# Stability-AI/stable-audio-tools

Hardware: AMD Instinct MI355X
Metric: train-step samples/sec (47s@44.1kHz) (higher is better)
Workload: dtype f32(bf16x3)

## Files before the change

### include/sat_amd.h

```cpp
#ifndef SAT_AMD_H
#define SAT_AMD_H

#ifdef __cplusplus
extern "C" {
#endif

int sat_abi_version(void);
int sat_is_simulator(void);
const char* sat_last_error(void);


int sat_conv1d(const float* x, const float* w_packed, const float* bias, const float* alpha, const float* beta,
               const float* res, float* y, const float* x2, const float* alpha2, const float* beta2,
               float* part_da, float* part_db, int B, int Cin, int Cout, int Tin, int Tout, int K, int stride,
               int dil, int pad, int tanh_out, void* stream);
int sat_conv1d_partial_rows(int B, int Tout);

int sat_conv1d_bf16x3(const float* x, const short* w_hi, const short* w_lo, const float* bias, const float* snake_a,
                      const float* snake_ib, const float* res, float* y, const float* x2, const float* alpha2,
                      const float* beta2, float* part_da, float* part_db, int B, int Cin, int Cout, int Tin, int Tout,
                      int K, int stride, int dil, int pad, int tanh_out, void* stream);
int sat_conv1d_bf16x3_emit(const float* x, const short* w_hi, const short* w_lo, const float* bias, const float* snake_a,
                      const float* snake_ib, const float* res, float* y, const float* x2, const float* alpha2,
                      const float* beta2, float* part_da, float* part_db, int B, int Cin, int Cout, int Tin, int Tout,
                      int K, int stride, int dil, int pad, int tanh_out, void* em_hi, void* em_lo,
                           const float* em_a, const float* em_ib, int em_rows, void* stream);
int sat_residual_unit_fwd(const short* xp_hi, const short* xp_lo, int rows, const short* w7_hi, const short* w7_lo,
                          const float* bias1, const float* a2, const float* ib2, const short* w1_hi, const short* w1_lo,
                          const float* bias2, const float* x, float* h, float* y, int B, int C, int T, int K, int dil, int pad,
                          void* em_hi, void* em_lo, const float* em_a, const float* em_ib, int em_rows, void* stream);
int sat_convtr1d_bf16x3(const float* x, const short* w_hi, const short* w_lo, const float* bias, const float* snake_a,
                        const float* snake_ib, const float* res, float* y, const float* x2, const float* alpha2,
                        const float* beta2, float* part_da, float* part_db, int B, int Cin, int Cout, int Tin, int Tout,
                        int K, int stride, int pad, int tanh_out, void* stream);
int sat_conv1d_bf16x3_partial_rows(int B, int Tout, int K, int stride);

int sat_rows_pack(const float* x, float* buf, int B, int C, int T, int W, int kh, int dil_t, int pad_t, int pad_w, int pitch, int lead,
                  void* stream);
int sat_rows_pack_bwd(const float* dbuf, float* dx, int B, int C, int T, int W, int kh, int dil_t, int pad_t, int pad_w, int pitch,
                      int lead, void* stream);
int sat_rows_unpack(const float* y, float* out, int B, int C, int T, int W, int pad_w, int pitch, float slope, void* stream);
int sat_rows_unpack_bwd(const float* dout, const float* out, float* dy, int B, int C, int T, int W, int pad_w, int pitch, float slope,
                        void* stream);

int sat_disc_geom(int frames, int W, int* P, int* L, int* lead, int* rows);
int sat_disc_planes(const float* src, const float* out, const signed char* fm_sign, const float* fm_coef, float* dst, void* hi, void* lo, int B,
                    int C, int frames, int W, int pitched, float slope, void* stream);
int sat_disc_l1_blocks(void);
int sat_disc_l1_sum(const float* a, const float* b, float* partial, signed char* sign, long long n, void* stream);
long long sat_disc_pack_size(int Cout, int Cin, int kh, int kw, int mode);
int sat_disc_pack_weights(const float* w, short* wq, int Cout, int Cin, int kh, int kw, int mode, void* stream);
int sat_disc_conv(const void* xp_hi, const void* xp_lo, const void* wq, const float* bias, float* y, void* em_hi,
                  void* em_lo, int B, int Cin, int Cout, int frames, int W, int kh, int kw, int dil_t, float slope, const float* lk_src,
                  float lk_slope, void* stream);
int sat_disc_wgrad_nsplit(int B, int M, int Cin, int kh, int frames, int W);
int sat_disc_wgrad(const float* dy, const float* x, float* partial, int B, int M, int Cin, int frames, int W, int kh, int kw, int dil_t,
                   void* stream);

int sat_conv1d_k7_plane_rows(int Tin, int Tout, int pad);
int sat_conv1d_k7_planes(const float* x, const float* snake_a, const float* snake_ib, short* xp_hi, short* xp_lo, int B, int Cin, int Tin,
                         int rows, void* stream);
long long sat_pack_weights_k7q_size(int D0, int D1, int K, int mode);
int sat_pack_weights_k7q(const float* w, short* hi, short* lo, int D0, int D1, int K, int mode, void* stream);
int sat_conv1d_bf16x3_planesq(const short* xp_hi, const short* xp_lo, int rows, const short* w_hi, const short* w_lo, const float* bias,
                             const float* res, float* y, const float* x2, const float* alpha2, const float* beta2, float* part_da,
                             float* part_db, int B, int Cin, int Cout, int Tin, int Tout, int K, int dil, int pad, int tanh_out,
                             int flags, void* stream);
int sat_convtr1d_bf16x3_partial_rows(int B, int Tout, int stride, int pad);
int sat_pack_weights_bf16x3(const float* w, short* hi, short* lo, int D0, int D1, int K, int stride, int mode, void* stream);
long long sat_pack_weights_bf16x3_size(int D0, int D1, int K, int stride, int mode);
int sat_snake_consts(const float* alpha, const float* beta, float* a, float* ib, int C, void* stream);

int sat_convtr1d(const float* x, const float* w_packed, const float* bias, const float* alpha, const float* beta,
                 const float* res, float* y, const float* x2, const float* alpha2, const float* beta2,
                 float* part_da, float* part_db, int B, int Cin, int Cout, int Tin, int Tout, int K, int stride,
                 int pad, int tanh_out, void* stream);
int sat_convtr1d_partial_rows(int B, int Tout, int stride, int pad);

int sat_conv_wgrad(const float* lo, const float* hi, const float* alpha, const float* beta, int snake_on,
                   float* partial, long long so_m, long long so_n, long long so_k, int B, int M, int N, int Tlo,
                   int Thi, int K, int stride, int dil, int pad, void* stream);
int sat_conv_wgrad_nsplit(int B, int M, int N, int Tlo, int K, int stride, int dil);

int sat_conv_wgrad7_bf16x3(const float* dy, const float* x, const float* alpha, const float* beta, float* partial,
                           long long so_m, long long so_n, long long so_k, int B, int M, int N, int T, int dil, int pad,
                           float* dy_rowsum, void* stream);
int sat_conv_wgrad7_bf16x3_nsplit(int B, int M, int N, int T);
int sat_conv_wgrad7_bf16x3_fuses_rowsum(int B, int M, int N, int T);

int sat_conv_wgrad_bf16x3(const float* lo, const float* hi, const float* alpha, const float* beta, int snake_on,
                          float* partial, long long so_m, long long so_n, long long so_k, int B, int M, int N, int Tlo,
                          int Thi, int K, int stride, int pad, float* lo_rowsum, void* stream);
int sat_conv_wgrad_bf16x3_nsplit(int B, int M, int N, int Tlo, int K, int stride);

int sat_ru_k1_bwd_nsplit(int B, int C, int T);
int sat_ru_k1_pack(const float* w, short* hi, short* lo, int C, void* stream);
int sat_ru_k1_bwd(const float* dy, const float* h, const short* wt_hi, const short* wt_lo, const float* alpha2, const float* beta2,
                  float* dh, short* em_hi, short* em_lo, int em_rows, float* dw_partial, float* part, int B, int C, int T,
                  void* stream);

int sat_reduce_splits(const float* partial, float* out, long long count, int nsplit, float scale, int accumulate,
                      void* stream);
int sat_rowsum(const float* x, float* partial, int B, int C, int T, void* stream);
int sat_rowsum_nsplit(int T);

int sat_wn_fold(const float* v, const float* g, float* w, float* norm, int D0, int R, void* stream);
int sat_wn_grad(const float* v, const float* g, const float* norm, const float* dw, float* dv, float* dg, int D0,
                int R, void* stream);
int sat_wn_grad_splits(const float* partial, int nsplit, long long count, long long so_m, long long so_n, long long so_k,
                       const float* v, const float* g, const float* norm, float* dv, float* dg, int D0, int N, int K,
                       const float* bias_partial, int bias_cols, float* dbias, void* stream);
int sat_edge_conv_ok(int cin, int cout, int k, int stride, int dil, int pad);
int sat_edge_conv_partial_rows(int B, int T);
int sat_edge_conv(const float* x, const float* w, const float* bias, const float* alpha, const float* beta, float* y, const float* x2,
                  const float* alpha2, const float* beta2, float* part_da, float* part_db, short* em_hi, short* em_lo,
                  const float* em_alpha, const float* em_beta, int em_rows, int B, int Cin, int Cout, int T, int K, int pad, int mode,
                  int tanh_out, void* stream);
int sat_edge_conv_wgrad_nsplit(int B, int M, int N, int T);
int sat_edge_conv_wgrad(const float* dy, const float* x, const float* alpha, const float* beta, float* partial, float* rowsum, int B,
                        int M, int N, int T, int K, int pad, void* stream);
int sat_pack_weights(const float* w, float* out, int D0, int D1, int K, int S, int mode, void* stream);

int sat_vae_nblocks(long long n);
int sat_vae_sample_fwd(const float* pre, const float* noise, float* z, float* kl_partial, int B, int C, int T,
                       void* stream);
int sat_vae_sample_bwd(const float* pre, const float* noise, const float* dz, const float* dkl, float* dpre, int B,
                       int C, int T, void* stream);

int sat_fir(const float* x, const float* taps, float* y, int N, int T, int ntaps, int adjoint, void* stream);
int sat_stft_tiles(int n_fft, int hop, int T);
int sat_stft_fwd(const float* x, const float* y, const float* views, float* partial, int NI, int C, int T, int NV,
                 int n_fft, int hop, void* stream);
int sat_stft_bwd(const float* x, const float* y, const float* views, const float* coef, float* dy, int NI, int C,
                 int T, int NV, int n_fft, int hop, int wrt_x, void* stream);

int sat_adamw_step(float* p, const float* g, float* m, float* v, long long n, float lr, float beta1, float beta2,
                   float eps, float weight_decay, int step, float grad_scale, float* ema, float ema_decay,
                   void* stream);
int sat_adamw_step_dev(float* p, const float* g, float* m, float* v, long long n, const float* hyper, float beta1, float beta2,
                       float eps, float weight_decay, float* ema, void* stream);

int sat_multi_copy(const void* entries, int nent, void* stream);

int sat_allreduce_available(void);
int sat_allreduce_unique_id(void* id128);
int sat_allreduce_init(const void* id128, int world, int rank, void** comm);
int sat_allreduce_bucket(void* comm, void* buf, long long count, int dtype, int mode, void* stream);
int sat_allreduce_finalize(void* comm);

int sat_attn_prepare(const void* src, long long sb, long long sh, long long sn, short* rm_hi, short* rm_lo,
                     short* tr_hi, short* tr_lo, int B, int H, int N, int Np, int dtype, void* stream);
int sat_attention_fwd(const short* q_hi, const short* q_lo, const short* k_hi, const short* k_lo, const short* vt_hi,
                      const short* vt_lo, void* o, float* lse, int B, int H, int Hkv, int Nq, int Nk, int Nqp, int Nkp,
                      int head_dim, float scale, int dtype, void* stream);
int sat_attention_rowdot(const void* dout, const void* out, float* dsum, int B, int H, int Nq, int dtype, void* stream);
int sat_attention_bwd(const short* const* planes, const float* lse, const float* dsum, void* dq, void* dk, void* dv,
                      int B, int H, int Hkv, int Nq, int Nk, int Nqp, int Nkp, int head_dim, float scale, int dtype,
                      void* stream);
int sat_attention_cross_ok(int H, int Hkv, int Nk, int head_dim, int dtype);
int sat_attention_cross_fwd(const short* q_rm, const short* k_rm, const short* v_tr, void* o, float* lse, int B, int H, int Hkv,
                            int Nq, int Nk, int Nqp, int Nkp, int head_dim, float scale, void* stream);
long long sat_attention_cross_bwd_ws(int B, int H, int Hkv, int Nq, int Nk);
int sat_attention_cross_bwd(const short* const* planes, const float* lse, const float* dsum, void* dq, void* dk, void* dv,
                            void* ws, long long ws_bytes, int B, int H, int Hkv, int Nq, int Nk, int Nqp, int Nkp, int head_dim,
                            float scale, void* stream);

int sat_layernorm_fwd(const void* x, const float* gamma, const float* beta, const void* scale, const void* shift,
                      long long mod_stride, void* y, float* mean, float* rstd, int rows, int D, int rows_per_batch,
                      float eps, int dtype, void* stream);
int sat_layernorm_fwd_fp8(const void* x, const float* gamma, const float* beta, const void* scale, const void* shift,
                          long long mod_stride, void* q, float* qscale, int rows, int D, int rows_per_batch, float eps,
                          int dtype, void* stream);
int sat_layernorm_bwd_nblocks(int rows, int rows_per_batch);
int sat_layernorm_bwd(const void* dy, const void* x, const float* gamma, const float* beta, const void* scale,
                      long long mod_stride, const float* mean, const float* rstd, void* dx, float* part, int rows, int D,
                      int rows_per_batch, int dtype, void* stream);
int sat_layernorm_bwd_res(const void* dy, const void* x, const float* gamma, const float* beta, const void* scale,
                          long long mod_stride, const float* mean, const float* rstd, const void* dres, void* dx, float* part,
                          int rows, int D, int rows_per_batch, int dtype, void* stream);

int sat_rope_tables(const float* inv_freq, float* cs, int N, int half, float pos_scale, void* stream);
int sat_rope_apply(void* t, const float* cs, long long sb, long long sn, long long sh, int B, int N, int H, int half,
                   int tab_off, int transpose, int dtype, void* stream);

int sat_swiglu(const void* xin, const void* dout, void* out, long long rows, int F, int backward, int dtype,
               void* stream);
int sat_gate_residual(const void* x, const void* gate, long long gstride, const void* res, void* y, int B, int N, int D,
                      int dtype, void* stream);
int sat_gate_residual_bwd_nchunks(int N);
int sat_gate_residual_bwd(const void* dy, const void* x, const void* gate, long long gstride, void* dx, float* part,
                          int B, int N, int D, int dtype, void* stream);

int sat_cfg_step(const void* out2, const void* x, void* y0, void* y1, int B, int C, int T, int ncond, float scale,
                 float phi, float c0x, float c0v, float c1x, float c1v, int dtype, void* stream);
int sat_sampler_step(const void* out2, const void* x, const void* prev, void* y0, void* y1, int B, int C, int T, int ncond,
                     float scale, float phi, const float* coef, int dtype, void* stream);
int sat_sampler_step_dev(const void* out2, const void* x, const void* prev, void* y0, void* y1, int B, int C, int T, int ncond,
                         float scale, float phi, const float* coef, int dtype, void* stream);
int sat_spec_frames(int n_fft, int hop, int T);
int sat_spec_fwd(const float* x, float* z, int NI, int C, int T, int n_fft, int hop, void* stream);
int sat_spec_bwd(const float* dz, float* dx, int NI, int C, int T, int n_fft, int hop, void* stream);


int sat_gemm_bf16(const void* A, long long lda, const void* B, long long ldb, void* C, long long ldc, const float* bias,
                  const void* res, long long ldr, const void* gate, long long ldg, int rows_per_gate, void* pre,
                  long long ldp, const void* zeros, int M, int N, int K, int epilogue, int out_f32, int splits, int tile,
                  void* stream);

int sat_gemm_qkv_bf16(const void* A, long long lda, const void* B, long long ldb, const float* rope_cs, int rope_off,
                      void* q_rm, void* k_rm, void* v_tr, const void* zeros, int nb, int ntok, int npad, int heads,
                      int K, int sec0, int nsec, int tile, void* stream);

int sat_splitk_epilogue(const float* slabs, int S, const float* bias, const void* res, long long ldr, void* out, long long ldo,
                        int M, int N, int out_f32, void* stream);

int sat_gemm_fp8(const void* A, long long lda, const void* B, long long ldb, void* C, long long ldc, const float* bias,
                 const void* res, long long ldr, const void* gate, long long ldg, int rows_per_gate, void* pre,
                 long long ldp, const void* zeros, const float* alpha, const float* row_alpha, const float* col_alpha, int M, int N,
                 int K, int epilogue, int out_f32, int tile, void* stream);
int sat_gemm_qkv_fp8(const void* A, long long lda, const void* B, long long ldb, const float* rope_cs, int rope_off,
                     void* q_rm, void* k_rm, void* v_tr, const void* zeros, const float* alpha, const float* row_alpha,
                     const float* col_alpha, int nb, int ntok, int npad, int heads, int K, int sec0, int nsec, int tile, void* stream);
int sat_absmax_scale_blocks(int R, int C);
int sat_absmax_scale(const void* src, long long lds, float* work, float* scales, int R, int C, int src_f32, void* stream);
int sat_quant_fp8(const void* src, long long lds, void* dst, long long ldd, const float* qscale, int R, int C, int src_f32,
                  void* stream);
int sat_quant_fp8_rows(const void* src, long long lds, void* dst, long long ldd, float* scale, int R, int C, int src_f32,
                       void* stream);

int sat_cast_bf16(const void* src, long long lds, void* dst, long long ldd, int R, int C, int Rpad, int src_f32,
                  int transpose, void* stream);
int sat_cast_bf16_tpair(const void* src_a, long long lds_a, void* dst_a, long long ldd_a, int Ra, int Ca, int Rpad_a, int a_f32,
                        const void* src_b, long long lds_b, void* dst_b, long long ldd_b, int Rb, int Cb, int Rpad_b, int b_f32,
                        void* stream);
int sat_cast_bf16_dual(const void* src, long long lds, void* dst, long long ldd, void* dst_t, long long ldd_t, int R, int C, int Rpad,
                       int src_f32, void* stream);

int sat_split_bf16x3(const float* src, long long lds, void* dst, long long ldd, int R, int C, int side, void* stream);

#ifdef __cplusplus
}
#endif
#endif
```

### stable_audio_tools_amd/_lib.py

```python
import ctypes
import os

_P = ctypes.c_void_p
_I = ctypes.c_int
_L = ctypes.c_longlong
_F = ctypes.c_float

SIGNATURES = {
    "sat_abi_version": (_I, []),
    "sat_is_simulator": (_I, []),
    "sat_last_error": (ctypes.c_char_p, []),
    "sat_conv1d": (_I, [_P] * 12 + [_I] * 10 + [_P]),
    "sat_conv1d_partial_rows": (_I, [_I, _I]),
    "sat_conv1d_bf16x3": (_I, [_P] * 13 + [_I] * 10 + [_P]),
    "sat_conv1d_bf16x3_emit": (_I, [_P] * 13 + [_I] * 10 + [_P] * 4 + [_I, _P]),
    "sat_convtr1d_bf16x3": (_I, [_P] * 13 + [_I] * 9 + [_P]),
    "sat_conv1d_bf16x3_partial_rows": (_I, [_I] * 4),
    "sat_rows_pack": (_I, [_P, _P] + [_I] * 10 + [_P]),
    "sat_rows_pack_bwd": (_I, [_P, _P] + [_I] * 10 + [_P]),
    "sat_rows_unpack": (_I, [_P, _P] + [_I] * 6 + [_F, _P]),
    "sat_rows_unpack_bwd": (_I, [_P, _P, _P] + [_I] * 6 + [_F, _P]),
    "sat_disc_geom": (_I, [_I, _I, _P, _P, _P, _P]),
    "sat_disc_planes": (_I, [_P] * 7 + [_I] * 5 + [_F, _P]),
    "sat_disc_l1_blocks": (_I, []),
    "sat_disc_l1_sum": (_I, [_P, _P, _P, _P, _L, _P]),
    "sat_disc_pack_size": (_L, [_I] * 5),
    "sat_disc_pack_weights": (_I, [_P] * 2 + [_I] * 5 + [_P]),
    "sat_disc_conv": (_I, [_P] * 7 + [_I] * 8 + [_F, _P, _F, _P]),
    "sat_disc_wgrad_nsplit": (_I, [_I] * 6),
    "sat_disc_wgrad": (_I, [_P] * 3 + [_I] * 8 + [_P]),
    "sat_conv1d_k7_plane_rows": (_I, [_I] * 3),
    "sat_conv1d_k7_planes": (_I, [_P] * 5 + [_I] * 4 + [_P]),
    "sat_conv1d_bf16x3_planesq": (_I, [_P, _P, _I] + [_P] * 10 + [_I] * 10 + [_P]),
    "sat_pack_weights_k7q": (_I, [_P, _P, _P, _I, _I, _I, _I, _P]),
    "sat_residual_unit_fwd": (_I, [_P, _P, _I] + [_P] * 11 + [_I] * 6 + [_P] * 4 + [_I, _P]),
    "sat_pack_weights_k7q_size": (_L, [_I, _I, _I, _I]),
    "sat_convtr1d_bf16x3_partial_rows": (_I, [_I] * 4),
    "sat_pack_weights_bf16x3": (_I, [_P, _P, _P, _I, _I, _I, _I, _I, _P]),
    "sat_pack_weights_bf16x3_size": (_L, [_I, _I, _I, _I, _I]),
    "sat_snake_consts": (_I, [_P, _P, _P, _P, _I, _P]),
    "sat_conv_wgrad7_bf16x3": (_I, [_P] * 5 + [_L] * 3 + [_I] * 6 + [_P, _P]),
    "sat_conv_wgrad7_bf16x3_nsplit": (_I, [_I] * 4),
    "sat_conv_wgrad7_bf16x3_fuses_rowsum": (_I, [_I] * 4),
    "sat_conv_wgrad_bf16x3": (_I, [_P] * 4 + [_I, _P] + [_L] * 3 + [_I] * 8 + [_P, _P]),
    "sat_conv_wgrad_bf16x3_nsplit": (_I, [_I] * 6),
    "sat_convtr1d": (_I, [_P] * 12 + [_I] * 9 + [_P]),
    "sat_convtr1d_partial_rows": (_I, [_I, _I, _I, _I]),
    "sat_conv_wgrad": (_I, [_P, _P, _P, _P, _I, _P, _L, _L, _L] + [_I] * 9 + [_P]),
    "sat_conv_wgrad_nsplit": (_I, [_I] * 7),
    "sat_reduce_splits": (_I, [_P, _P, _L, _I, _F, _I, _P]),
    "sat_ru_k1_bwd_nsplit": (_I, [_I] * 3),
    "sat_ru_k1_pack": (_I, [_P, _P, _P, _I, _P]),
    "sat_ru_k1_bwd": (_I, [_P] * 9 + [_I, _P, _P, _I, _I, _I, _P]),
    "sat_rowsum": (_I, [_P, _P, _I, _I, _I, _P]),
    "sat_rowsum_nsplit": (_I, [_I]),
    "sat_wn_fold": (_I, [_P, _P, _P, _P, _I, _I, _P]),
    "sat_wn_grad": (_I, [_P, _P, _P, _P, _P, _P, _I, _I, _P]),
    "sat_wn_grad_splits": (_I, [_P, _I, _L, _L, _L, _L, _P, _P, _P, _P, _P, _I, _I, _I, _P, _I, _P, _P]),
    "sat_pack_weights": (_I, [_P, _P, _I, _I, _I, _I, _I, _P]),
    "sat_vae_nblocks": (_I, [_L]),
    "sat_vae_sample_fwd": (_I, [_P, _P, _P, _P, _I, _I, _I, _P]),
    "sat_vae_sample_bwd": (_I, [_P, _P, _P, _P, _P, _I, _I, _I, _P]),
    "sat_multi_copy": (_I, [_P, _I, _P]),
    "sat_adamw_step": (_I, [_P, _P, _P, _P, _L, _F, _F, _F, _F, _F, _I, _F, _P, _F, _P]),
    "sat_adamw_step_dev": (_I, [_P, _P, _P, _P, _L, _P, _F, _F, _F, _F, _P, _P]),
    "sat_allreduce_available": (_I, []),
    "sat_allreduce_unique_id": (_I, [_P]),
    "sat_allreduce_init": (_I, [_P, _I, _I, _P]),
    "sat_allreduce_bucket": (_I, [_P, _P, _L, _I, _I, _P]),
    "sat_allreduce_finalize": (_I, [_P]),
    "sat_fir": (_I, [_P, _P, _P, _I, _I, _I, _I, _P]),
    "sat_stft_tiles": (_I, [_I, _I, _I]),
    "sat_stft_fwd": (_I, [_P, _P, _P, _P, _I, _I, _I, _I, _I, _I, _P]),
    "sat_stft_bwd": (_I, [_P, _P, _P, _P, _P, _I, _I, _I, _I, _I, _I, _I, _P]),
    "sat_spec_frames": (_I, [_I, _I, _I]),
    "sat_spec_fwd": (_I, [_P, _P, _I, _I, _I, _I, _I, _P]),
    "sat_spec_bwd": (_I, [_P, _P, _I, _I, _I, _I, _I, _P]),
    "sat_attn_prepare": (_I, [_P, _L, _L, _L, _P, _P, _P, _P, _I, _I, _I, _I, _I, _P]),
    "sat_attention_fwd": (_I, [_P] * 8 + [_I] * 8 + [_F, _I, _P]),
    "sat_attention_rowdot": (_I, [_P, _P, _P, _I, _I, _I, _I, _P]),
    "sat_attention_bwd": (_I, [_P] * 6 + [_I] * 8 + [_F, _I, _P]),
    "sat_edge_conv_ok": (_I, [_I] * 6),
    "sat_edge_conv_partial_rows": (_I, [_I] * 2),
    "sat_edge_conv": (_I, [_P] * 15 + [_I] * 9 + [_P]),
    "sat_edge_conv_wgrad_nsplit": (_I, [_I] * 4),
    "sat_edge_conv_wgrad": (_I, [_P] * 6 + [_I] * 6 + [_P]),
    "sat_attention_cross_ok": (_I, [_I] * 5),
    "sat_attention_cross_fwd": (_I, [_P] * 5 + [_I] * 8 + [_F, _P]),
    "sat_attention_cross_bwd_ws": (_L, [_I] * 5),
    "sat_attention_cross_bwd": (_I, [_P] * 7 + [_L] + [_I] * 8 + [_F, _P]),
    "sat_gemm_bf16": (_I, [_P, _L, _P, _L, _P, _L, _P, _P, _L, _P, _L, _I, _P, _L, _P] + [_I] * 7 + [_P]),
    "sat_gemm_qkv_bf16": (_I, [_P, _L, _P, _L, _P, _I, _P, _P, _P, _P] + [_I] * 8 + [_P]),
    "sat_gemm_fp8": (_I, [_P, _L, _P, _L, _P, _L, _P, _P, _L, _P, _L, _I, _P, _L, _P, _P, _P, _P] + [_I] * 6 + [_P]),
    "sat_gemm_qkv_fp8": (_I, [_P, _L, _P, _L, _P, _I, _P, _P, _P, _P, _P, _P, _P] + [_I] * 8 + [_P]),
    "sat_quant_fp8": (_I, [_P, _L, _P, _L, _P, _I, _I, _I, _P]),
    "sat_quant_fp8_rows": (_I, [_P, _L, _P, _L, _P, _I, _I, _I, _P]),
    "sat_absmax_scale": (_I, [_P, _L, _P, _P, _I, _I, _I, _P]),
    "sat_absmax_scale_blocks": (_I, [_I, _I]),
    "sat_splitk_epilogue": (_I, [_P, _I, _P, _P, _L, _P, _L, _I, _I, _I, _P]),
    "sat_cast_bf16": (_I, [_P, _L, _P, _L, _I, _I, _I, _I, _I, _P]),
    "sat_cast_bf16_tpair": (_I, [_P, _L, _P, _L, _I, _I, _I, _I, _P, _L, _P, _L, _I, _I, _I, _I, _P]),
    "sat_cast_bf16_dual": (_I, [_P, _L, _P, _L, _P, _L, _I, _I, _I, _I, _P]),
    "sat_split_bf16x3": (_I, [_P, _L, _P, _L, _I, _I, _I, _P]),
    "sat_layernorm_fwd": (_I, [_P] * 5 + [_L] + [_P] * 3 + [_I] * 3 + [_F, _I, _P]),
    "sat_layernorm_fwd_fp8": (_I, [_P] * 5 + [_L] + [_P] * 2 + [_I] * 3 + [_F, _I, _P]),
    "sat_layernorm_bwd_nblocks": (_I, [_I, _I]),
    "sat_layernorm_bwd": (_I, [_P] * 5 + [_L] + [_P] * 4 + [_I] * 4 + [_P]),
    "sat_layernorm_bwd_res": (_I, [_P] * 5 + [_L] + [_P] * 5 + [_I] * 4 + [_P]),
    "sat_rope_tables": (_I, [_P, _P, _I, _I, _F, _P]),
    "sat_rope_apply": (_I, [_P, _P, _L, _L, _L] + [_I] * 7 + [_P]),
    "sat_swiglu": (_I, [_P, _P, _P, _L, _I, _I, _I, _P]),
    "sat_gate_residual": (_I, [_P, _P, _L, _P, _P, _I, _I, _I, _I, _P]),
    "sat_gate_residual_bwd_nchunks": (_I, [_I]),
    "sat_cfg_step": (_I, [_P, _P, _P, _P, _I, _I, _I, _I, _F, _F, _F, _F, _F, _F, _I, _P]),
    "sat_sampler_step": (_I, [_P, _P, _P, _P, _P, _I, _I, _I, _I, _F, _F, _P, _I, _P]),
    "sat_sampler_step_dev": (_I, [_P, _P, _P, _P, _P, _I, _I, _I, _I, _F, _F, _P, _I, _P]),
    "sat_gate_residual_bwd": (_I, [_P, _P, _P, _L, _P, _P, _I, _I, _I, _I, _P]),
}

LIB_PATH = os.path.join(os.path.dirname(os.path.abspath(__file__)), "csrc", "libsat_amd.so")


def bind(cdll):
    for name, (res, args) in SIGNATURES.items():
        fn = getattr(cdll, name)
        fn.restype = res
        fn.argtypes = args
    return cdll


_lib = None


def load():
    global _lib
    if _lib is not None:
        return _lib
    if not os.path.exists(LIB_PATH):
        raise RuntimeError(
            f"stable_audio_tools_amd: HIP library not built: {LIB_PATH} is missing. "
            "Run `python -c 'import __graft_entry__ as g; g.build()'` (hipcc --offload-arch=gfx950). "
            "There is no CPU fallback.")
    try:
        cdll = ctypes.CDLL(LIB_PATH)
    except OSError as e:
        raise RuntimeError(f"stable_audio_tools_amd: cannot load {LIB_PATH}: {e}. There is no CPU fallback.") from e
    bind(cdll)
    if cdll.sat_is_simulator():
        raise RuntimeError("stable_audio_tools_amd: refusing to use a simulator build as the product library")
    _lib = cdll
    return _lib
```

### stable_audio_tools_amd/csrc/conv_wgrad_bf16x3.hip

```cpp
#include "conv_common.h"
#include <type_traits>

#define SAT_WB_TT 64
#define SAT_WB_LOROW (SAT_WB_TT + 8)
#define SAT_WB_HIROW 136

struct SatWgBfParams {
    const float* dy;
    const float* x;
    const float* alpha;
    const float* beta;
    float* out;
    long long so_split, so_m, so_n, so_k;
    int B, M, N, T, pad;
    int chunks_per_split, nchunks, nT;
    float* rowsum;
    int nsplit;
};

SAT_DEVICE unsigned sat_umulhi(unsigned a, unsigned b) { return (unsigned)(((unsigned long long)a * b) >> 32); }
SAT_DEVICE float sat_row16_sum(float4 q) {
    float s = (q.x + q.y) + (q.z + q.w);
#pragma unroll
    for (int m = 1; m <= 8; m <<= 1) s += __shfl_xor(s, m);
    return s;
}

#if defined(SAT_HIPEMU)
static inline unsigned sat_alignbit(unsigned hi, unsigned lo, unsigned s) {
    return (unsigned)((((unsigned long long)hi << 32) | lo) >> s);
}
#else
SAT_DEVICE unsigned sat_alignbit(unsigned hi, unsigned lo, unsigned s) { return __builtin_amdgcn_alignbit(hi, lo, s); }
#endif


template <int DIL>
__global__ void __launch_bounds__(256)
#if !defined(SAT_HIPEMU)
__attribute__((amdgpu_waves_per_eu(2, 2)))
#endif
sat_wgrad7_bf16x3_kernel(SatWgBfParams p) {
    constexpr int NCH = (6 * DIL + 7) / 8 + 1;
    __shared__ __attribute__((aligned(16))) short lo_lds[2][SAT_CO_T][SAT_WB_LOROW];
    __shared__ __attribute__((aligned(16))) short hi_lds[2][32][SAT_WB_HIROW];
    __shared__ float sn_a[32], sn_ib[32];

    const int tid = threadIdx.x, lane = tid & 63, wave = tid >> 6;
    const int l31 = lane & 31, hi = lane >> 5;
    int mn_tile, split;
    sat_xcd_tile(blockIdx.x + gridDim.x * (blockIdx.y + gridDim.y * blockIdx.z), gridDim.x * gridDim.y, gridDim.z, &mn_tile, &split);
    const int m0 = (mn_tile % (int)gridDim.x) * SAT_CO_T, n0 = (mn_tile / (int)gridDim.x) * 32;
    const int m_w = wave * 32;
    const bool wave_on = (m0 + m_w) < p.M;

    f32x16 acc[7];
#pragma unroll
    for (int k = 0; k < 7; ++k)
#pragma unroll
        for (int r = 0; r < 16; ++r) acc[k][r] = 0.0f;

    const bool want_rs = p.rowsum != nullptr && n0 == 0;
    float rs[8] = {0.f, 0.f, 0.f, 0.f, 0.f, 0.f, 0.f, 0.f};

    if (tid < 32) {
        const int c = n0 + tid;
        float sa = 1.f, sib = 0.f;
        if (p.alpha && c < p.N) {
            sa = expf(p.alpha[c]);
            sib = 1.0f / (expf(p.beta[c]) + 1e-9f);
        }
        sn_a[tid] = sa;
        sn_ib[tid] = sib;
    }
    for (int i = tid; i < 2 * 32 * SAT_WB_HIROW; i += 256) (&hi_lds[0][0][0])[i] = 0;
    __syncthreads();

    const int c_begin = split * p.chunks_per_split;
    int c_end = c_begin + p.chunks_per_split;
    if (c_end > p.nchunks) c_end = p.nchunks;
    constexpr int HSPAN = SAT_WB_TT + 6 * DIL;

    for (int ch = c_begin; ch < c_end; ++ch) {
        const int b = ch / p.nT;
        const int tt0 = (ch - b * p.nT) * SAT_WB_TT;
        {
            const float* src = p.dy + (size_t)b * p.M * p.T;
            for (int half = 0; half < 2; ++half) {
            float4 v[4];
#pragma unroll
            for (int u = 0; u < 4; ++u) {
                const int idx = tid + (half * 4 + u) * 256;
                const int row = idx >> 4, c4 = (idx & 15) * 4;
                const int m = m0 + row, t = tt0 + c4;
                float4 q = make_float4(0.f, 0.f, 0.f, 0.f);
                if (m < p.M) {
                    const float* s = src + (size_t)m * p.T + t;
                    if (t + 3 < p.T && ((p.T & 3) == 0)) {
                        q = *reinterpret_cast<const float4*>(s);
                    } else {
                        if (t + 0 < p.T) q.x = s[0];
                        if (t + 1 < p.T) q.y = s[1];
                        if (t + 2 < p.T) q.z = s[2];
                        if (t + 3 < p.T) q.w = s[3];
                    }
                }
                v[u] = q;
            }
#pragma unroll
            for (int u = 0; u < 4; ++u) {
                const int idx = tid + (half * 4 + u) * 256;
                const int row = idx >> 4, c4 = (idx & 15) * 4;
                if (want_rs) rs[half * 4 + u] += sat_row16_sum(v[u]);
                uint32_t h0, h1, l0, l1;
                sat_split2_pk(v[u].x, v[u].y, &h0, &l0);
                sat_split2_pk(v[u].z, v[u].w, &h1, &l1);
                typedef uint32_t u2 __attribute__((ext_vector_type(2)));
                *reinterpret_cast<u2*>(&lo_lds[0][row][c4]) = u2{h0, h1};
                *reinterpret_cast<u2*>(&lo_lds[1][row][c4]) = u2{l0, l1};
            }
            }
        }
        {
            const float* src = p.x + (size_t)b * p.N * p.T;
            const int th0 = tt0 - p.pad;
            constexpr int HP = HSPAN / 2;
            constexpr int TOTAL = 32 * HP;
            for (int base = tid; base < TOTAL; base += 8 * 256) {
                float v[8][2];
#pragma unroll
                for (int u = 0; u < 8; ++u) {
                    const int idx = base + u * 256;
                    const int row = idx / HP, col = (idx - row * HP) * 2;
                    const int n = n0 + row, t = th0 + col;
                    const bool ok = idx < TOTAL && n < p.N;
                    const float* s = src + (size_t)(ok ? n : 0) * p.T;
                    v[u][0] = (ok && t >= 0 && t < p.T) ? s[t] : 0.0f;
                    v[u][1] = (ok && t + 1 >= 0 && t + 1 < p.T) ? s[t + 1] : 0.0f;
                }
#pragma unroll
                for (int u = 0; u < 8; ++u) {
                    const int idx = base + u * 256;
                    if (idx < TOTAL) {
                        const int row = idx / HP, col = (idx - row * HP) * 2;
                        float o0 = v[u][0], o1 = v[u][1];
                        if (p.alpha) {
                            const float sa = sn_a[row], sib = sn_ib[row];
                            o0 = sat_snake(o0, sa, sib);
                            o1 = sat_snake(o1, sa, sib);
                        }
                        uint32_t h, l;
                        sat_split2_pk(o0, o1, &h, &l);
                        *reinterpret_cast<uint32_t*>(&hi_lds[0][row][col]) = h;
                        *reinterpret_cast<uint32_t*>(&hi_lds[1][row][col]) = l;
                    }
                }
            }
        }
        __syncthreads();
        if (wave_on) {
#pragma unroll
            for (int ks = 0; ks < SAT_WB_TT / 16; ++ks) {
                const int tb = 16 * ks + 8 * hi;
                bf16x8 af[2];
                af[0] = *reinterpret_cast<const bf16x8*>(&lo_lds[0][m_w + l31][tb]);
                af[1] = *reinterpret_cast<const bf16x8*>(&lo_lds[1][m_w + l31][tb]);
#pragma unroll
                for (int pl = 0; pl < 2; ++pl) {
                    u32x4 cw[NCH];
#if !defined(SAT_HIPEMU)
                    asm volatile("" ::: "memory");
#endif
#pragma unroll
                    for (int j = 0; j < NCH; ++j) cw[j] = *reinterpret_cast<const u32x4*>(&hi_lds[pl][l31][tb + 8 * j]);
#pragma unroll
                    for (int k = 0; k < 7; ++k) {
                        const int off = k * DIL;
                        const int wbase = (off >> 3) * 4 + ((off & 7) >> 1);
                        const bool odd = (off & 1) != 0;
                        u32x4 r;
#pragma unroll
                        for (int i = 0; i < 4; ++i) {
                            const int w0 = wbase + i, w1 = wbase + i + 1;
                            const unsigned a0 = cw[w0 >> 2][w0 & 3];
                            if (odd) {
                                const unsigned a1 = cw[w1 >> 2][w1 & 3];
                                r[i] = sat_alignbit(a1, a0, 16);
                            } else {
                                r[i] = a0;
                            }
                        }
                        const bf16x8 bf = __builtin_bit_cast(bf16x8, r);
                        acc[k] = sat_mfma_32x32x16_bf16(af[0], bf, acc[k]);
                        if (pl == 0) acc[k] = sat_mfma_32x32x16_bf16(af[1], bf, acc[k]);
                    }
                }
            }
        }
        __syncthreads();
    }

    if (want_rs && (tid & 15) == 0) {
#pragma unroll
        for (int i = 0; i < 8; ++i) {
            const int m = m0 + (tid >> 4) + 16 * i;
            if (m < p.M) p.rowsum[(size_t)m * p.nsplit + split] = rs[i];
        }
    }
    if (wave_on) {
        float* ob = p.out + (size_t)split * p.so_split;
        const int n = n0 + l31;
#pragma unroll
        for (int k = 0; k < 7; ++k)
#pragma unroll
            for (int r = 0; r < 16; ++r) {
                const int m = m0 + m_w + (r & 3) + 8 * (r >> 2) + 4 * hi;
                if (m < p.M && n < p.N) ob[(size_t)m * p.so_m + (size_t)n * p.so_n + (size_t)k * p.so_k] = acc[k][r];
            }
    }
}

#include "conv_wgrad7_bf16x3_pipe.h"

struct SatWgBfPlan { int nsplit, cps, nchunks, nT; bool pipe; };
static void sat_wgbf_plan(int B, int M, int N, int T, SatWgBfPlan* pl) {
    pl->nT = sat_cdiv(T, SAT_WB_TT);
    pl->nchunks = B * pl->nT;
    pl->pipe = N >= SAT_WP_NI && (T & 3) == 0;
    const int tiles = sat_cdiv(M, SAT_CO_T) * sat_cdiv(N, pl->pipe ? SAT_WP_NI : 32);
    int want = 512 / tiles;
    if (want > pl->nchunks) want = pl->nchunks;
    if (want < 1) want = 1;
    if (want > 512) want = 512;
    pl->cps = sat_cdiv(pl->nchunks, want);
    pl->nsplit = sat_cdiv(pl->nchunks, pl->cps);
}
extern "C" int sat_conv_wgrad7_bf16x3_nsplit(int B, int M, int N, int T) {
    SatWgBfPlan pl;
    sat_wgbf_plan(B, M, N, T, &pl);
    return pl.nsplit;
}
extern "C" int sat_conv_wgrad7_bf16x3_fuses_rowsum(int B, int M, int N, int T) {
    SatWgBfPlan pl;
    sat_wgbf_plan(B, M, N, T, &pl);
    return pl.pipe ? 0 : 1;
}
extern "C" int sat_conv_wgrad7_bf16x3(const float* dy, const float* x, const float* alpha, const float* beta, float* partial,
                                      long long so_m, long long so_n, long long so_k, int B, int M, int N, int T, int dil,
                                      int pad, float* dy_rowsum, void* stream) {
    if (B <= 0 || M <= 0 || N <= 0 || T <= 0) { sat_set_error("sat_conv_wgrad7_bf16x3: empty shape"); return 1; }
    if (dil != 1 && dil != 3 && dil != 9) { sat_set_error("sat_conv_wgrad7_bf16x3: dilation must be 1, 3 or 9 (the Oobleck ResidualUnits)"); return 1; }
    if ((alpha == nullptr) != (beta == nullptr)) { sat_set_error("sat_conv_wgrad7_bf16x3: alpha/beta must both be given"); return 1; }
    SatWgBfPlan pl;
    sat_wgbf_plan(B, M, N, T, &pl);
    SatWgBfParams p{dy, x, alpha, beta, partial, (long long)M * N * 7, so_m, so_n, so_k, B, M, N, T, pad, pl.cps, pl.nchunks, pl.nT,
                    dy_rowsum, pl.nsplit};
    if (pl.pipe) {
        dim3 grid(sat_cdiv(M, SAT_CO_T), sat_cdiv(N, SAT_WP_NI), pl.nsplit);
        if (dy_rowsum) { sat_set_error("sat_conv_wgrad7_bf16x3: this shape's kernel does not fuse the row sums (sat_conv_wgrad7_bf16x3_fuses_rowsum)"); return 1; }
        if (dil == 1) SAT_LAUNCH((sat_wgrad7_bf16x3_pipe_kernel<1>), grid, dim3(SAT_WP_NT), stream, p);
        else if (dil == 3) SAT_LAUNCH((sat_wgrad7_bf16x3_pipe_kernel<3>), grid, dim3(SAT_WP_NT), stream, p);
        else SAT_LAUNCH((sat_wgrad7_bf16x3_pipe_kernel<9>), grid, dim3(SAT_WP_NT), stream, p);
        return sat_check_launch("sat_conv_wgrad7_bf16x3");
    }
    dim3 grid(sat_cdiv(M, SAT_CO_T), sat_cdiv(N, 32), pl.nsplit);
    if (dil == 1) SAT_LAUNCH(sat_wgrad7_bf16x3_kernel<1>, grid, dim3(256), stream, p);
    else if (dil == 3) SAT_LAUNCH(sat_wgrad7_bf16x3_kernel<3>, grid, dim3(256), stream, p);
    else SAT_LAUNCH(sat_wgrad7_bf16x3_kernel<9>, grid, dim3(256), stream, p);
    return sat_check_launch("sat_conv_wgrad7_bf16x3");
}

#define SAT_WS_TT 64
#define SAT_WS_LOROW (SAT_WS_TT + 8)
#define SAT_WS_HIROW (SAT_WS_TT + 8)

struct SatWgSmallParams {
    const float* lo;
    const float* hi;
    const float* alpha;
    const float* beta;
    float* out;
    long long so_split, so_m, so_n, so_k;
    int B, M, N, Tlo, Thi, pad, snake_on, s_log2;
    int chunks_per_split, nchunks, nT;
    float* rowsum;
    int nsplit;
};

template <int NT>
__global__ void __launch_bounds__(256)
#if !defined(SAT_HIPEMU)
__attribute__((amdgpu_waves_per_eu(2, 2)))
#endif
sat_wgrad_small_bf16x3_kernel(SatWgSmallParams p) {
    constexpr int NCH = NT;
    __shared__ __attribute__((aligned(16))) short lo_lds[2][SAT_CO_T][SAT_WS_LOROW];
    __shared__ __attribute__((aligned(16))) short hi_lds[2][SAT_CO_T][SAT_WS_HIROW];
    __shared__ float sn_a[SAT_CO_T], sn_ib[SAT_CO_T];

    const int tid = threadIdx.x, lane = tid & 63, wave = tid >> 6;
    const int l31 = lane & 31, hi = lane >> 5;
    const int sl = p.s_log2, S = 1 << sl;
    int mn_tile, split;
    sat_xcd_tile(blockIdx.x + gridDim.x * (blockIdx.y + gridDim.y * blockIdx.z), gridDim.x * gridDim.y, gridDim.z, &mn_tile, &split);
    const int m0 = (mn_tile % (int)gridDim.x) * SAT_CO_T, v0 = (mn_tile / (int)gridDim.x) * SAT_CO_T;
    const int n_base = v0 >> sl, nc = SAT_CO_T >> sl;
    const int NV = p.N << sl;
    const int m_w = (wave >> 1) * 64, v_w = (wave & 1) * 64;
    const bool wave_on = (m0 + m_w) < p.M && (v0 + v_w) < NV;
    const bool snake_lo = p.alpha && p.snake_on == 1, snake_hi = p.alpha && p.snake_on == 2;

    f32x16 acc[2][2][NT];
#pragma unroll
    for (int i = 0; i < 2; ++i)
#pragma unroll
        for (int j = 0; j < 2; ++j)
#pragma unroll
            for (int k = 0; k < NT; ++k)
#pragma unroll
                for (int r = 0; r < 16; ++r) acc[i][j][k][r] = 0.0f;

    const bool want_rs = p.rowsum != nullptr && v0 == 0;
    float rsum[8] = {0.f, 0.f, 0.f, 0.f, 0.f, 0.f, 0.f, 0.f};

    if (tid < SAT_CO_T) {
        float sa = 1.f, sib = 0.f;
        const int c = snake_lo ? m0 + tid : n_base + tid;
        const bool ok = snake_lo ? c < p.M : (snake_hi && tid < nc && c < p.N);
        if (ok) {
            sa = expf(p.alpha[c]);
            sib = 1.0f / (expf(p.beta[c]) + 1e-9f);
        }
        sn_a[tid] = sa;
        sn_ib[tid] = sib;
    }
    __syncthreads();

    const int c_begin = split * p.chunks_per_split;
    int c_end = c_begin + p.chunks_per_split;
    if (c_end > p.nchunks) c_end = p.nchunks;
    const int rs = (SAT_WS_TT + NT - 1) << sl;
    const int up = rs >> 1;
    const int total_units = nc * up;

    auto mfma_stage = [&]() {
        if (wave_on) {
            SAT_MFMA_PRIO(1);
#pragma unroll
            for (int ks = 0; ks < SAT_WS_TT / 16; ++ks) {
                const int tb = 16 * ks + 8 * hi;
                bf16x8 af[2][2];
#pragma unroll
                for (int mi = 0; mi < 2; ++mi)
#pragma unroll
                    for (int pl = 0; pl < 2; ++pl)
                        af[mi][pl] = *reinterpret_cast<const bf16x8*>(&lo_lds[pl][m_w + mi * 32 + l31][tb]);
#pragma unroll
                for (int ni = 0; ni < 2; ++ni) {
#pragma unroll
                    for (int pl = 0; pl < 2; ++pl) {
                        u32x4 cw[NCH];
#pragma unroll
                        for (int j = 0; j < NCH; ++j) cw[j] = *reinterpret_cast<const u32x4*>(&hi_lds[pl][v_w + ni * 32 + l31][tb + 8 * j]);
#pragma unroll
                        for (int j = 0; j < NT; ++j) {
                            u32x4 r = cw[0];
                            if (j == 1) {
                                r[0] = sat_alignbit(cw[0][1], cw[0][0], 16);
                                r[1] = sat_alignbit(cw[0][2], cw[0][1], 16);
                                r[2] = sat_alignbit(cw[0][3], cw[0][2], 16);
                                r[3] = sat_alignbit(cw[NCH - 1][0], cw[0][3], 16);
                            }
                            const bf16x8 bf = __builtin_bit_cast(bf16x8, r);
#pragma unroll
                            for (int mi = 0; mi < 2; ++mi) {
                                acc[mi][ni][j] = sat_mfma_32x32x16_bf16(af[mi][0], bf, acc[mi][ni][j]);
                                if (pl == 0) acc[mi][ni][j] = sat_mfma_32x32x16_bf16(af[mi][1], bf, acc[mi][ni][j]);
                            }
                        }
                    }
                }
            }
            SAT_MFMA_PRIO(0);
        }
    };

    const bool fast1 = (NT == 1) && sl == 0 && p.pad == 0 && (p.Tlo & 3) == 0 && p.Thi == p.Tlo;
    if (fast1) {
        float4 vlo[8], vhi[8];
        const int row0 = tid >> 4, c4 = (tid & 15) * 4;
        auto issue = [&](int ch) {
            const int b = ch / p.nT;
            const int tt0 = (ch - b * p.nT) * SAT_WS_TT;
            const float* slo = p.lo + (size_t)b * p.M * p.Tlo;
            const float* shi = p.hi + (size_t)b * p.N * p.Thi;
            const bool t_ok = tt0 + c4 < p.Tlo;
#pragma unroll
            for (int u = 0; u < 8; ++u) {
                const int m = m0 + row0 + 16 * u, n = v0 + row0 + 16 * u;
                const bool okm = t_ok && m < p.M, okn = t_ok && n < p.N;
                const float4 a = *reinterpret_cast<const float4*>(slo + (size_t)(okm ? m : 0) * p.Tlo + (okm ? tt0 + c4 : 0));
                const float4 c = *reinterpret_cast<const float4*>(shi + (size_t)(okn ? n : 0) * p.Thi + (okn ? tt0 + c4 : 0));
                vlo[u] = okm ? a : make_float4(0.f, 0.f, 0.f, 0.f);
                vhi[u] = okn ? c : make_float4(0.f, 0.f, 0.f, 0.f);
            }
        };
        auto convert = [&]() {
            typedef uint32_t u2 __attribute__((ext_vector_type(2)));
#pragma unroll
            for (int u = 0; u < 8; ++u) {
                const int row = row0 + 16 * u;
                float4 q = vlo[u];
                if (want_rs) rsum[u] += sat_row16_sum(q);
                if (snake_lo) {
                    const float sa = sn_a[row], sib = sn_ib[row];
                    q.x = sat_snake(q.x, sa, sib); q.y = sat_snake(q.y, sa, sib);
                    q.z = sat_snake(q.z, sa, sib); q.w = sat_snake(q.w, sa, sib);
                }
                uint32_t h0, h1, l0, l1;
                sat_split2_pk(q.x, q.y, &h0, &l0);
                sat_split2_pk(q.z, q.w, &h1, &l1);
                *reinterpret_cast<u2*>(&lo_lds[0][row][c4]) = u2{h0, h1};
                *reinterpret_cast<u2*>(&lo_lds[1][row][c4]) = u2{l0, l1};
                q = vhi[u];
                if (snake_hi) {
                    const float sa = sn_a[row], sib = sn_ib[row];
                    q.x = sat_snake(q.x, sa, sib); q.y = sat_snake(q.y, sa, sib);
                    q.z = sat_snake(q.z, sa, sib); q.w = sat_snake(q.w, sa, sib);
                }
                sat_split2_pk(q.x, q.y, &h0, &l0);
                sat_split2_pk(q.z, q.w, &h1, &l1);
                *reinterpret_cast<u2*>(&hi_lds[0][row][c4]) = u2{h0, h1};
                *reinterpret_cast<u2*>(&hi_lds[1][row][c4]) = u2{l0, l1};
            }
        };
        issue(c_begin);
        for (int ch = c_begin; ch < c_end; ++ch) {
            convert();
            __syncthreads();
            if (ch + 1 < c_end) issue(ch + 1);
            mfma_stage();
            __syncthreads();
        }
    } else if ((NT == 2) && sl >= 1 && sl <= 3 && (p.Tlo & 3) == 0) {
        typedef float f4u __attribute__((ext_vector_type(4), aligned(4)));
        typedef uint32_t u2 __attribute__((ext_vector_type(2)));
        constexpr int NQ = 9;
        const int qpc = 33 << (sl - 1);
        const unsigned magic = 0xffffffffu / (unsigned)qpc + 1u;
        const int total_q = nc * qpc;
        const int qcl = sl >= 2 ? sl - 2 : 0, qc = 1 << qcl;
        auto load_quads = [&](int tv, const float* shi, int th0, bool interior, f4u* vq, auto ib, auto ie) {
            constexpr int IB = decltype(ib)::value, IE = decltype(ie)::value;
#pragma unroll
            for (int i = IB; i < IE; ++i) {
                f4u v = {0.f, 0.f, 0.f, 0.f};
                if (i < NQ - 1 || wave == 0) {
                    const int Q = tv + 256 * i;
                    const int cl = (int)sat_umulhi((unsigned)Q, magic), q = Q - cl * qpc;
                    const int n = n_base + cl, t = th0 + 4 * q;
                    const float* sp = shi + (size_t)(n < p.N ? n : p.N - 1) * p.Thi;
                    if (interior) {
                        v = *reinterpret_cast<const f4u*>(sp + t);
                    } else {
#pragma unroll
                        for (int e = 0; e < 4; ++e) {
                            const int te = t + e;
                            const int tc = te < 0 ? 0 : (te < p.Thi ? te : p.Thi - 1);
                            const float x = sp[tc];
                            v[e] = (te == tc) ? x : 0.0f;
                        }
                    }
                    if (n >= p.N) v = f4u{0.f, 0.f, 0.f, 0.f};
                }
                vq[i - IB] = v;
            }
        };
        auto store_quads = [&](int tv, const f4u* vq, auto ib, auto ie) {
            constexpr int IB = decltype(ib)::value, IE = decltype(ie)::value;
#pragma unroll
            for (int i = IB; i < IE; ++i) {
                const int Q = tv + 256 * i;
                if (i == NQ - 1 && Q >= total_q) break;
                const int cl = (int)sat_umulhi((unsigned)Q, magic), q = Q - cl * qpc;
                f4u o = vq[i - IB];
                if (snake_hi) {
                    const float sa = sn_a[cl], sib = sn_ib[cl];
#pragma unroll
                    for (int e = 0; e < 4; ++e) o[e] = sat_snake(o[e], sa, sib);
                }
                uint32_t h01, l01, h23, l23;
                sat_split2_pk(o[0], o[1], &h01, &l01);
                sat_split2_pk(o[2], o[3], &h23, &l23);
                int row, col;
                uint32_t wh0, wh1, wl0, wl1;
                if (sl == 1) {
                    row = cl << 1;
                    col = 2 * q;
                    wh0 = (h01 & 0xffffu) | (h23 << 16); wh1 = (h01 >> 16) | (h23 & 0xffff0000u);
                    wl0 = (l01 & 0xffffu) | (l23 << 16); wl1 = (l01 >> 16) | (l23 & 0xffff0000u);
                } else {
                    const int colq = q >> qcl, part = q & (qc - 1);
                    const bool odd = colq & 1;
                    const uint32_t rh = __shfl_xor(odd ? h01 : h23, qc), rl = __shfl_xor(odd ? l01 : l23, qc);
                    row = (cl << sl) + 4 * part + (odd ? 2 : 0);
                    col = colq & ~1;
                    if (!odd) {
                        wh0 = (h01 & 0xffffu) | (rh << 16); wh1 = (h01 >> 16) | (rh & 0xffff0000u);
                        wl0 = (l01 & 0xffffu) | (rl << 16); wl1 = (l01 >> 16) | (rl & 0xffff0000u);
                    } else {
                        wh0 = (rh & 0xffffu) | (h23 << 16); wh1 = (rh >> 16) | (h23 & 0xffff0000u);
                        wl0 = (rl & 0xffffu) | (l23 << 16); wl1 = (rl >> 16) | (l23 & 0xffff0000u);
                    }
                }
                *reinterpret_cast<uint32_t*>(&hi_lds[0][row][col]) = wh0;
                *reinterpret_cast<uint32_t*>(&hi_lds[0][row + 1][col]) = wh1;
                *reinterpret_cast<uint32_t*>(&hi_lds[1][row][col]) = wl0;
                *reinterpret_cast<uint32_t*>(&hi_lds[1][row + 1][col]) = wl1;
            }
        };
        using I0 = std::integral_constant<int, 0>; using IN = std::integral_constant<int, NQ>;
        f4u vq[NQ];
        auto issue_hi = [&](int ch) {
            const int b = ch / p.nT;
            const int tt0 = (ch - b * p.nT) * SAT_WS_TT;
            const int th0 = (tt0 << sl) - p.pad;
            const bool interior = th0 >= 0 && th0 + (66 << sl) <= p.Thi;
            int tv = tid;
#if !defined(SAT_HIPEMU)
            asm volatile("" : "+v"(tv));
#endif
            load_quads(tv, p.hi + (size_t)b * p.N * p.Thi, th0, interior, vq, I0{}, IN{});
        };
#if !defined(SAT_WGS_NOCARRY)
        issue_hi(c_begin);
#endif
        for (int ch = c_begin; ch < c_end; ++ch) {
            const int b = ch / p.nT;
            const int tt0 = (ch - b * p.nT) * SAT_WS_TT;
            const float* slo = p.lo + (size_t)b * p.M * p.Tlo;
            int tv = tid;
#if !defined(SAT_HIPEMU)
            asm volatile("" : "+v"(tv));
#endif
            const int row0 = tv >> 4, c4 = (tv & 15) * 4;
            float4 vlo[8];
#if defined(SAT_WGS_NOCARRY)
            issue_hi(ch);
#endif
            {
                const bool t_ok = tt0 + c4 < p.Tlo;
#pragma unroll
                for (int u = 0; u < 8; ++u) {
                    const int m = m0 + row0 + 16 * u;
                    const bool okm = t_ok && m < p.M;
                    const float4 a = *reinterpret_cast<const float4*>(slo + (size_t)(okm ? m : 0) * p.Tlo + (okm ? tt0 + c4 : 0));
                    vlo[u] = okm ? a : make_float4(0.f, 0.f, 0.f, 0.f);
                }
            }
            SAT_SCHED_FENCE();
            store_quads(tv, vq, I0{}, IN{});
            SAT_SCHED_FENCE();
#pragma unroll
            for (int u = 0; u < 8; ++u) {
                const int row = row0 + 16 * u;
                float4 q = vlo[u];
                if (want_rs) rsum[u] += sat_row16_sum(q);
                if (snake_lo) {
                    const float sa = sn_a[row], sib = sn_ib[row];
                    q.x = sat_snake(q.x, sa, sib); q.y = sat_snake(q.y, sa, sib);
                    q.z = sat_snake(q.z, sa, sib); q.w = sat_snake(q.w, sa, sib);
                }
// ... 181 lines not shown
```

### stable_audio_tools_amd/csrc/ru_k1_bwd.hip

```cpp
#include "conv_common.h"

typedef uint32_t sat_u32x2 __attribute__((ext_vector_type(2)));

#define SAT_RK_TT 32
#define SAT_RK_ROWN (SAT_RK_TT + 8)
#define SAT_RK_EROW (SAT_RK_TT + 4)
#define SAT_RK_LEAD 32

SAT_DEVICE f32x16 sat_rk_cat4(f32x4 v0, f32x4 v1, f32x4 v2, f32x4 v3) {
#if defined(SAT_HIPEMU)
    f32x16 o;
    for (int e = 0; e < 4; ++e) {
        o[e] = v0[e];
        o[4 + e] = v1[e];
        o[8 + e] = v2[e];
        o[12 + e] = v3[e];
    }
    return o;
#else
    typedef float sat_f8v __attribute__((ext_vector_type(8)));
    const sat_f8v lo = __builtin_shufflevector(v0, v1, 0, 1, 2, 3, 4, 5, 6, 7), hi = __builtin_shufflevector(v2, v3, 0, 1, 2, 3, 4, 5, 6, 7);
    return __builtin_shufflevector(lo, hi, 0, 1, 2, 3, 4, 5, 6, 7, 8, 9, 10, 11, 12, 13, 14, 15);
#endif
}
SAT_DEVICE bf16x8 sat_rk_frag(const f32x16& v, int g) {
    const f32x4 q = {v[4 * g], v[4 * g + 1], v[4 * g + 2], v[4 * g + 3]};
    return __builtin_bit_cast(bf16x8, q);
}

struct SatRuK1BwdParams {
    const float* dy;
    const float* h;
    const short* wt_hi;
    const short* wt_lo;
    const float* alpha2;
    const float* beta2;
    float* dh;
    short* em_hi;
    short* em_lo;
    float* dw_partial;
    float* part;
    int B, C, T, em_rows, nsplit, tiles_per_split, ntiles;
};

template <int C>
__global__ void __launch_bounds__(512) sat_ru_k1_bwd_kernel(SatRuK1BwdParams p) {
    static_assert(C == 128, "one 128-channel tile of h per workgroup, W2^T fragments in registers");
    constexpr int TT = SAT_RK_TT, ROWN = SAT_RK_ROWN, ROWT = C + 8, EROW = SAT_RK_EROW;
    constexpr int NJ = C / 64;
    constexpr int DYT = 2 * TT * ROWT;
    constexpr int DYN = 2 * C * ROWN;
    constexpr int AN = 2 * C * ROWN;
    constexpr int RAW = 2 * C * TT;
    static_assert(C * EROW * 4 <= AN * 2, "the epilogue tile aliases the snake2(h) image");
    static_assert(TT * 4 == 128, "a raw row is eight 16-byte DMA lanes");
    __shared__ __attribute__((aligned(16))) char smem[(DYT + DYN + AN) * 2 + 2 * RAW * 4];
    short* dyT = reinterpret_cast<short*>(smem);
    short* dyN = dyT + DYT;
    short* aN = dyN + DYN;
    float* etile = reinterpret_cast<float*>(aN);
    short* dhT = dyT;
    float* raw = reinterpret_cast<float*>(smem + (DYT + DYN + AN) * 2);

    const int tid = threadIdx.x, lane = tid & 63;
    const int wave = SAT_UNIFORM((int)(threadIdx.x >> 6));
    const int l31 = lane & 31, hi = lane >> 5;
    const int split = blockIdx.x;
    const int tiles_per_b = p.T / TT;
    const int tile_begin = split * p.tiles_per_split;
    int tile_end = tile_begin + p.tiles_per_split;
    if (tile_end > p.ntiles) tile_end = p.ntiles;
    const bool dgrad_wave = wave < 4;
    const int wq = wave & 3, wm = wq >> 1, wn = wq & 1;

    const int srow = tid >> 3, st4 = (tid & 7) * 4;
    const int swz_w = ((st4 >> 3) & 3) << 3;
    const int swz_f = ((l31 >> 3) & 3) << 3;
    float sa[NJ], sb[NJ], sib[NJ];
#pragma unroll
    for (int j = 0; j < NJ; ++j) {
        const int ci = srow + 64 * j;
        sa[j] = expf(p.alpha2[ci]);
        sb[j] = expf(p.beta2[ci]);
        sib[j] = 1.0f / (sb[j] + 1e-9f);
    }
    float sum_da[NJ], sum_db[NJ], sum_dh[NJ], sum_dy[NJ];
#pragma unroll
    for (int j = 0; j < NJ; ++j) sum_da[j] = sum_db[j] = sum_dh[j] = sum_dy[j] = 0.0f;

    f32x16 big[4];
    if (dgrad_wave) {
        const short* wrow_hi = p.wt_hi + (size_t)(32 * wq + l31) * C + 8 * hi;
        const short* wrow_lo = p.wt_lo + (size_t)(32 * wq + l31) * C + 8 * hi;
#pragma unroll
        for (int q = 0; q < 2; ++q) {
            big[q] = sat_rk_cat4(*reinterpret_cast<const f32x4*>(wrow_hi + 64 * q), *reinterpret_cast<const f32x4*>(wrow_hi + 64 * q + 16),
                                 *reinterpret_cast<const f32x4*>(wrow_hi + 64 * q + 32), *reinterpret_cast<const f32x4*>(wrow_hi + 64 * q + 48));
            big[2 + q] = sat_rk_cat4(*reinterpret_cast<const f32x4*>(wrow_lo + 64 * q), *reinterpret_cast<const f32x4*>(wrow_lo + 64 * q + 16),
                                     *reinterpret_cast<const f32x4*>(wrow_lo + 64 * q + 32), *reinterpret_cast<const f32x4*>(wrow_lo + 64 * q + 48));
        }
#if !defined(SAT_HIPEMU)
        asm volatile("" : "+v"(big[0]), "+v"(big[1]), "+v"(big[2]), "+v"(big[3]));
#endif
    } else {
#pragma unroll
        for (int i = 0; i < 4; ++i)
#pragma unroll
            for (int r = 0; r < 16; ++r) big[i][r] = 0.0f;
    }

    const size_t lane_off = (size_t)(lane >> 3) * p.T + (lane & 7) * 4;
    auto dma_tile = [&](int tile) __attribute__((always_inline)) {
        const int b = tile / tiles_per_b, t0 = (tile - b * tiles_per_b) * TT;
        char* slot = reinterpret_cast<char*>(raw) + (tile & 1) * (RAW * 4);
        const size_t base = (size_t)b * C * p.T + t0 + lane_off;
#pragma unroll
        for (int q = 0; q < 4; ++q) {
            const int piece = wave + 8 * q;
            const float* src = (q < 2 ? p.dy : p.h) + base + (size_t)(8 * (piece & 15)) * p.T;
            sat_glds16(src, slot + piece * 1024);
        }
    };
    if (tile_begin < tile_end) dma_tile(tile_begin);

    for (int tile = tile_begin; tile < tile_end; ++tile) {
        const int b = tile / tiles_per_b, t0 = (tile - b * tiles_per_b) * TT;
        const float* rt = raw + (tile & 1) * RAW;
        const bool more = tile + 1 < tile_end;
        if (more) { dma_tile(tile + 1); SAT_WAIT_VMCNT(4); } else { SAT_WAIT_VMCNT(0); }
        SAT_RAW_BARRIER();
        f32x4 hv[NJ];
#pragma unroll
        for (int j = 0; j < NJ; ++j) {
            const int ch = srow + 64 * j;
            const f32x4 dyv = *reinterpret_cast<const f32x4*>(rt + ch * TT + st4);
            hv[j] = *reinterpret_cast<const f32x4*>(rt + (C + ch) * TT + st4);
            uint32_t h0, l0, h1, l1;
            sat_split2_pk(dyv[0], dyv[1], &h0, &l0);
            sat_split2_pk(dyv[2], dyv[3], &h1, &l1);
            *reinterpret_cast<sat_u32x2*>(dyN + ch * ROWN + st4) = sat_u32x2{h0, h1};
            *reinterpret_cast<sat_u32x2*>(dyN + C * ROWN + ch * ROWN + st4) = sat_u32x2{l0, l1};
            const int cs = ch ^ swz_w;
            dyT[(st4 + 0) * ROWT + cs] = (short)(h0 & 0xffffu);
            dyT[(st4 + 1) * ROWT + cs] = (short)(h0 >> 16);
            dyT[(st4 + 2) * ROWT + cs] = (short)(h1 & 0xffffu);
            dyT[(st4 + 3) * ROWT + cs] = (short)(h1 >> 16);
            dyT[TT * ROWT + (st4 + 0) * ROWT + cs] = (short)(l0 & 0xffffu);
            dyT[TT * ROWT + (st4 + 1) * ROWT + cs] = (short)(l0 >> 16);
            dyT[TT * ROWT + (st4 + 2) * ROWT + cs] = (short)(l1 & 0xffffu);
            dyT[TT * ROWT + (st4 + 3) * ROWT + cs] = (short)(l1 >> 16);
            sum_dy[j] += (dyv[0] + dyv[1]) + (dyv[2] + dyv[3]);
            float v[4];
#pragma unroll
            for (int e = 0; e < 4; ++e) v[e] = sat_snake(hv[j][e], sa[j], sib[j]);
            sat_split2_pk(v[0], v[1], &h0, &l0);
            sat_split2_pk(v[2], v[3], &h1, &l1);
            *reinterpret_cast<sat_u32x2*>(aN + ch * ROWN + st4) = sat_u32x2{h0, h1};
            *reinterpret_cast<sat_u32x2*>(aN + C * ROWN + ch * ROWN + st4) = sat_u32x2{l0, l1};
        }
        SAT_WAIT_LGKM0();
        SAT_RAW_BARRIER();

        if (dgrad_wave) {
            f32x16 accd;
#pragma unroll
            for (int r = 0; r < 16; ++r) accd[r] = 0.0f;
            const short* brow = dyT + l31 * ROWT;
#pragma unroll
            for (int s = 0; s < C / 16; ++s) {
                const int col = (16 * s + 8 * hi) ^ swz_f;
                const bf16x8 bh = *reinterpret_cast<const bf16x8*>(brow + col);
                const bf16x8 bl = *reinterpret_cast<const bf16x8*>(brow + TT * ROWT + col);
                const bf16x8 wh = sat_rk_frag(big[s >> 2], s & 3), wl = sat_rk_frag(big[2 + (s >> 2)], s & 3);
                accd = sat_mfma_32x32x16_bf16(wh, bh, accd);
                accd = sat_mfma_32x32x16_bf16(wh, bl, accd);
                accd = sat_mfma_32x32x16_bf16(wl, bh, accd);
            }
            SAT_WAIT_LGKM0();
            SAT_RAW_BARRIER();
#pragma unroll
            for (int r = 0; r < 16; ++r) etile[(32 * wq + (r & 3) + 8 * (r >> 2) + 4 * hi) * EROW + l31] = accd[r];
        } else {
#pragma unroll
            for (int s = 0; s < TT / 16; ++s) {
                bf16x8 bh[2], bl[2];
#pragma unroll
                for (int nb = 0; nb < 2; ++nb) {
                    const short* br = aN + (wn * 64 + 32 * nb + l31) * ROWN + 16 * s + 8 * hi;
                    bh[nb] = *reinterpret_cast<const bf16x8*>(br);
                    bl[nb] = *reinterpret_cast<const bf16x8*>(br + C * ROWN);
                }
#pragma unroll
                for (int mb = 0; mb < 2; ++mb) {
                    const short* ar = dyN + (wm * 64 + 32 * mb + l31) * ROWN + 16 * s + 8 * hi;
                    const bf16x8 ah = *reinterpret_cast<const bf16x8*>(ar);
                    const bf16x8 al = *reinterpret_cast<const bf16x8*>(ar + C * ROWN);
#pragma unroll
                    for (int nb = 0; nb < 2; ++nb) {
                        big[2 * mb + nb] = sat_mfma_32x32x16_bf16(ah, bh[nb], big[2 * mb + nb]);
                        big[2 * mb + nb] = sat_mfma_32x32x16_bf16(ah, bl[nb], big[2 * mb + nb]);
                        big[2 * mb + nb] = sat_mfma_32x32x16_bf16(al, bh[nb], big[2 * mb + nb]);
                    }
                }
            }
            SAT_WAIT_LGKM0();
            SAT_RAW_BARRIER();
        }
        SAT_WAIT_LGKM0();
        SAT_RAW_BARRIER();

#pragma unroll
        for (int j = 0; j < NJ; ++j) {
            const int ch = srow + 64 * j;
            const f32x4 pre = *reinterpret_cast<const f32x4*>(etile + ch * EROW + st4);
            f32x4 out;
#pragma unroll
            for (int e = 0; e < 4; ++e) {
                const SatSnakeGrad g = sat_snake_grad(hv[j][e], sa[j], sb[j]);
                sum_da[j] += pre[e] * g.dla;
                sum_db[j] += pre[e] * g.dlb;
                out[e] = pre[e] * g.dx;
                sum_dh[j] += out[e];
            }
            *reinterpret_cast<f32x4*>(p.dh + ((size_t)b * C + ch) * p.T + t0 + st4) = out;
            if (p.em_hi) {
                uint32_t h0, l0, h1, l1;
                sat_split2_pk(out[0], out[1], &h0, &l0);
                sat_split2_pk(out[2], out[3], &h1, &l1);
                const int cs = ch ^ swz_w;
                dhT[(st4 + 0) * ROWT + cs] = (short)(h0 & 0xffffu);
                dhT[(st4 + 1) * ROWT + cs] = (short)(h0 >> 16);
                dhT[(st4 + 2) * ROWT + cs] = (short)(h1 & 0xffffu);
                dhT[(st4 + 3) * ROWT + cs] = (short)(h1 >> 16);
                dhT[TT * ROWT + (st4 + 0) * ROWT + cs] = (short)(l0 & 0xffffu);
                dhT[TT * ROWT + (st4 + 1) * ROWT + cs] = (short)(l0 >> 16);
                dhT[TT * ROWT + (st4 + 2) * ROWT + cs] = (short)(l1 & 0xffffu);
                dhT[TT * ROWT + (st4 + 3) * ROWT + cs] = (short)(l1 >> 16);
            }
        }
        SAT_WAIT_LGKM0();
        SAT_RAW_BARRIER();

        if (p.em_hi) {
            const int t = tid & 31, g = tid >> 5;
            const size_t o = (((size_t)b * (C / 8) + g) * p.em_rows + SAT_RK_LEAD + t0 + t) * 8;
            const int gs = (8 * g) ^ (((t >> 3) & 3) << 3);
            *reinterpret_cast<u32x4*>(p.em_hi + o) = *reinterpret_cast<const u32x4*>(dhT + t * ROWT + gs);
            *reinterpret_cast<u32x4*>(p.em_lo + o) = *reinterpret_cast<const u32x4*>(dhT + TT * ROWT + t * ROWT + gs);
            SAT_WAIT_LGKM0();
            SAT_RAW_BARRIER();
        }
    }

    if (!dgrad_wave) {
        float* slab = p.dw_partial + (size_t)split * C * C;
#pragma unroll
        for (int mb = 0; mb < 2; ++mb)
#pragma unroll
            for (int nb = 0; nb < 2; ++nb)
#pragma unroll
                for (int r = 0; r < 16; ++r) {
                    const int co = wm * 64 + 32 * mb + (r & 3) + 8 * (r >> 2) + 4 * hi;
                    const int ci = wn * 64 + 32 * nb + l31;
                    slab[(size_t)co * C + ci] = big[2 * mb + nb][r];
                }
    }
    const size_t ps = (size_t)C * p.nsplit;
#pragma unroll
    for (int j = 0; j < NJ; ++j) {
        float va = sum_da[j], vb = sum_db[j], vh = sum_dh[j], vy = sum_dy[j];
#pragma unroll
        for (int m = 1; m <= 4; m <<= 1) {
            va += __shfl_xor(va, m);
            vb += __shfl_xor(vb, m);
            vh += __shfl_xor(vh, m);
            vy += __shfl_xor(vy, m);
        }
        if ((tid & 7) == 0) {
            const size_t o = (size_t)(srow + 64 * j) * p.nsplit + split;
            p.part[o] = va;
            p.part[ps + o] = vb;
            p.part[2 * ps + o] = vh;
            p.part[3 * ps + o] = vy;
        }
    }
}

static int sat_ru_k1_plan(int B, int C, int T, int* nsplit, int* tiles_per_split, int* ntiles) {
    if (B <= 0 || T <= 0 || C != 128 || (T % SAT_RK_TT) != 0) return 1;
    const long long nt = (long long)B * (T / SAT_RK_TT);
    if (nt > 0x7fffffff) return 1;
    int want = sat_cu_count();
    if (want > nt) want = (int)nt;
    const int per = (int)((nt + want - 1) / want);
    *tiles_per_split = per;
    *nsplit = (int)((nt + per - 1) / per);
    *ntiles = (int)nt;
    return 0;
}

extern "C" int sat_ru_k1_bwd_nsplit(int B, int C, int T) {
    int ns, per, nt;
    if (sat_ru_k1_plan(B, C, T, &ns, &per, &nt)) return -1;
    return ns;
}

extern "C" int sat_ru_k1_bwd(const float* dy, const float* h, const short* wt_hi, const short* wt_lo, const float* alpha2,
                             const float* beta2, float* dh, short* em_hi, short* em_lo, int em_rows, float* dw_partial, float* part,
                             int B, int C, int T, void* stream) {
    SatRuK1BwdParams p{dy, h, wt_hi, wt_lo, alpha2, beta2, dh, em_hi, em_lo, dw_partial, part, B, C, T, em_rows, 0, 0, 0};
    if (sat_ru_k1_plan(B, C, T, &p.nsplit, &p.tiles_per_split, &p.ntiles)) {
        sat_set_error("sat_ru_k1_bwd: needs C == 128 and T % 32 == 0 (sat_ru_k1_bwd_nsplit)");
        return 1;
    }
    if (!dy || !h || !wt_hi || !wt_lo || !alpha2 || !beta2 || !dh || !dw_partial || !part) { sat_set_error("sat_ru_k1_bwd: missing buffer"); return 1; }
    if ((em_hi == nullptr) != (em_lo == nullptr) || (em_hi && em_rows < SAT_RK_LEAD + T)) { sat_set_error("sat_ru_k1_bwd: bad emission planes"); return 1; }
    if ((((uintptr_t)dy | (uintptr_t)h | (uintptr_t)dh | (uintptr_t)em_hi | (uintptr_t)em_lo | (uintptr_t)wt_hi | (uintptr_t)wt_lo) & 15) != 0) {
        sat_set_error("sat_ru_k1_bwd: buffers must be 16-byte aligned");
        return 1;
    }
    SAT_LAUNCH(sat_ru_k1_bwd_kernel<128>, dim3(p.nsplit), dim3(512), stream, p);
    return sat_check_launch("sat_ru_k1_bwd");
}

struct SatRuK1PackParams {
    const float* w;
    short* hi;
    short* lo;
    int C;
};
__global__ void __launch_bounds__(256) sat_ru_k1_pack_kernel(SatRuK1PackParams p) {
    const int i = blockIdx.x * 256 + threadIdx.x;
    if (i >= p.C * p.C) return;
    const int ci = i / p.C, co = i - ci * p.C;
    const float v = p.w[(size_t)co * p.C + ci];
    const short hb = sat_f32_to_bf16(v);
    p.hi[i] = hb;
    p.lo[i] = sat_f32_to_bf16(v - sat_bf16_to_f32(hb));
}
extern "C" int sat_ru_k1_pack(const float* w, short* hi, short* lo, int C, void* stream) {
    if (C <= 0 || !w || !hi || !lo) { sat_set_error("sat_ru_k1_pack: bad arguments"); return 1; }
    SatRuK1PackParams p{w, hi, lo, C};
    SAT_LAUNCH(sat_ru_k1_pack_kernel, dim3(sat_cdiv(C * C, 256)), dim3(256), stream, p);
    return sat_check_launch("sat_ru_k1_pack");
}
```

### stable_audio_tools_amd/csrc/sat_device.h

```cpp
#pragma once

#if defined(SAT_HIPEMU)
#include "hipemu.h"
#define SAT_DEVICE static inline
#else
#include <hip/hip_runtime.h>
#define SAT_DEVICE __device__ __forceinline__
#endif

#include <stdint.h>

typedef float f32x4 __attribute__((ext_vector_type(4)));
typedef float f32x16 __attribute__((ext_vector_type(16)));
typedef short bf16x8 __attribute__((ext_vector_type(8)));
typedef uint32_t u32x4 __attribute__((ext_vector_type(4)));
typedef int i32x8 __attribute__((ext_vector_type(8)));

#define SAT_WAVE 64

#if defined(SAT_HIPEMU)
static inline float hipemu_bf16_to_f32(short s) {
    uint32_t u = ((uint32_t)(uint16_t)s) << 16;
    float f;
    memcpy(&f, &u, 4);
    return f;
}
static inline f32x16 sat_mfma_32x32x2_f32(float a, float b, f32x16 c) {
    struct { float a, b; } mine = {a, b};
    const char* all = hipemu::wave_exchange(&mine, sizeof(mine));
    const int l = hipemu::lane_id();
    const int col = l & 31, hi = l >> 5;
    f32x16 d = c;
    for (int r = 0; r < 16; ++r) {
        const int row = (r & 3) + 8 * (r >> 2) + 4 * hi;
        float acc = c[r];
        for (int k = 0; k < 2; ++k) {
            float av, bv;
            memcpy(&av, all + (size_t)(row + 32 * k) * hipemu::kSlotBytes, 4);
            memcpy(&bv, all + (size_t)(col + 32 * k) * hipemu::kSlotBytes + 4, 4);
            acc = fmaf(av, bv, acc);
        }
        d[r] = acc;
    }
    return d;
}
static inline f32x16 sat_mfma_32x32x16_bf16(bf16x8 a, bf16x8 b, f32x16 c) {
    struct { bf16x8 a, b; } mine = {a, b};
    const char* all = hipemu::wave_exchange(&mine, sizeof(mine));
    const int l = hipemu::lane_id();
    const int col = l & 31, hi = l >> 5;
    f32x16 d = c;
    for (int r = 0; r < 16; ++r) {
        const int row = (r & 3) + 8 * (r >> 2) + 4 * hi;
        float acc = c[r];
        for (int g = 0; g < 2; ++g) {
            bf16x8 av, bv;
            memcpy(&av, all + (size_t)(row + 32 * g) * hipemu::kSlotBytes, 16);
            memcpy(&bv, all + (size_t)(col + 32 * g) * hipemu::kSlotBytes + 16, 16);
            for (int e = 0; e < 8; ++e) acc += hipemu_bf16_to_f32(av[e]) * hipemu_bf16_to_f32(bv[e]);
        }
        d[r] = acc;
    }
    return d;
}
static inline f32x4 sat_mfma_16x16x32_bf16(bf16x8 a, bf16x8 b, f32x4 c) {
    struct { bf16x8 a, b; } mine = {a, b};
    const char* all = hipemu::wave_exchange(&mine, sizeof(mine));
    const int l = hipemu::lane_id();
    const int col = l & 15, grp = l >> 4;
    f32x4 d = c;
    for (int r = 0; r < 4; ++r) {
        const int row = 4 * grp + r;
        float acc = c[r];
        for (int g = 0; g < 4; ++g) {
            bf16x8 av, bv;
            memcpy(&av, all + (size_t)(row + 16 * g) * hipemu::kSlotBytes, 16);
            memcpy(&bv, all + (size_t)(col + 16 * g) * hipemu::kSlotBytes + 16, 16);
            for (int e = 0; e < 8; ++e) acc += hipemu_bf16_to_f32(av[e]) * hipemu_bf16_to_f32(bv[e]);
        }
        d[r] = acc;
    }
    return d;
}
static inline float hipemu_e4m3_to_f32(uint8_t v) {
    const int s = v >> 7, e = (v >> 3) & 15, m = v & 7;
    float f;
    if (e == 15 && m == 7) f = NAN;
    else if (e == 0) f = ldexpf((float)m, -9);
    else f = ldexpf((float)(8 + m), e - 10);
    return s ? -f : f;
}
static inline f32x16 sat_mfma_32x32x64_fp8(i32x8 a, i32x8 b, f32x16 c) {
    struct { i32x8 a, b; } mine = {a, b};
    const char* all = hipemu::wave_exchange(&mine, sizeof(mine));
    const int l = hipemu::lane_id();
    const int col = l & 31, hi = l >> 5;
    f32x16 d = c;
    for (int r = 0; r < 16; ++r) {
        const int row = (r & 3) + 8 * (r >> 2) + 4 * hi;
        float acc = c[r];
        for (int g = 0; g < 2; ++g) {
            uint8_t av[32], bv[32];
            memcpy(av, all + (size_t)(row + 32 * g) * hipemu::kSlotBytes, 32);
            memcpy(bv, all + (size_t)(col + 32 * g) * hipemu::kSlotBytes + 32, 32);
            for (int e = 0; e < 32; ++e) acc += hipemu_e4m3_to_f32(av[e]) * hipemu_e4m3_to_f32(bv[e]);
        }
        d[r] = acc;
    }
    return d;
}
#else
SAT_DEVICE f32x16 sat_mfma_32x32x64_fp8(i32x8 a, i32x8 b, f32x16 c) {
    return __builtin_amdgcn_mfma_scale_f32_32x32x64_f8f6f4(a, b, c, 0, 0, 0, 127, 0, 127);
}
SAT_DEVICE f32x16 sat_mfma_32x32x2_f32(float a, float b, f32x16 c) {
    return __builtin_amdgcn_mfma_f32_32x32x2f32(a, b, c, 0, 0, 0);
}
SAT_DEVICE f32x16 sat_mfma_32x32x16_bf16(bf16x8 a, bf16x8 b, f32x16 c) {
    typedef __bf16 bf16x8_t __attribute__((ext_vector_type(8)));
    return __builtin_amdgcn_mfma_f32_32x32x16_bf16(__builtin_bit_cast(bf16x8_t, a), __builtin_bit_cast(bf16x8_t, b), c, 0, 0, 0);
}
SAT_DEVICE f32x4 sat_mfma_16x16x32_bf16(bf16x8 a, bf16x8 b, f32x4 c) {
    typedef __bf16 bf16x8_t __attribute__((ext_vector_type(8)));
    return __builtin_amdgcn_mfma_f32_16x16x32_bf16(__builtin_bit_cast(bf16x8_t, a), __builtin_bit_cast(bf16x8_t, b), c, 0, 0, 0);
}
#endif

SAT_DEVICE uint32_t sat_f32x4_to_fp8(float a, float b, float c, float d) {
#if defined(SAT_HIPEMU)
    auto enc = [](float x) -> uint32_t {
        if (x != x) return 0x7fu;
        const uint32_t sign = x < 0.f ? 0x80u : 0u;
        float ax = fabsf(x);
        if (ax > 448.f) ax = 448.f;
        if (ax < ldexpf(1.0f, -10)) return sign;
        int e;
        frexpf(ax, &e);
        int ue = e - 1;
        if (ue < -6) ue = -6;
        const float q = ldexpf(1.0f, ue - 3);
        float m = nearbyintf(ax / q);
        float v = m * q;
        if (v > 448.f) v = 448.f;
        if (v == 0.f) return sign;
        frexpf(v, &e);
        ue = e - 1;
        uint32_t bits;
        if (ue < -6) bits = (uint32_t)nearbyintf(v / ldexpf(1.0f, -9));
        else bits = ((uint32_t)(ue + 7) << 3) | ((uint32_t)nearbyintf(v / ldexpf(1.0f, ue - 3)) - 8u);
        return sign | bits;
    };
    return enc(a) | (enc(b) << 8) | (enc(c) << 16) | (enc(d) << 24);
#else
    const float lim = 448.0f;
    a = fminf(fmaxf(a, -lim), lim); b = fminf(fmaxf(b, -lim), lim); c = fminf(fmaxf(c, -lim), lim); d = fminf(fmaxf(d, -lim), lim);
    int w = 0;
    w = __builtin_amdgcn_cvt_pk_fp8_f32(a, b, w, false);
    w = __builtin_amdgcn_cvt_pk_fp8_f32(c, d, w, true);
    return (uint32_t)w;
#endif
}

SAT_DEVICE short sat_f32_to_bf16(float f) {
    uint32_t u;
    memcpy(&u, &f, 4);
    if ((u & 0x7fffffffu) > 0x7f800000u) return (short)0x7fc0;
    u += 0x7fffu + ((u >> 16) & 1u);
    return (short)(u >> 16);
}
SAT_DEVICE float sat_bf16_to_f32(short s) {
    uint32_t u = ((uint32_t)(uint16_t)s) << 16;
    float f;
    memcpy(&f, &u, 4);
    return f;
}

SAT_DEVICE void sat_split2_pk(float a, float b, uint32_t* hi, uint32_t* lo) {
#if defined(SAT_HIPEMU)
    const short ha = sat_f32_to_bf16(a), hb = sat_f32_to_bf16(b);
    const short la = sat_f32_to_bf16(a - sat_bf16_to_f32(ha)), lb = sat_f32_to_bf16(b - sat_bf16_to_f32(hb));
    *hi = ((uint32_t)(uint16_t)hb << 16) | (uint16_t)ha;
    *lo = ((uint32_t)(uint16_t)lb << 16) | (uint16_t)la;
#else
    typedef __bf16 sat_bf2 __attribute__((ext_vector_type(2)));
    typedef float sat_f2 __attribute__((ext_vector_type(2)));
    const sat_f2 v = {a, b};
    const sat_bf2 h = __builtin_convertvector(v, sat_bf2);
    const sat_f2 d = v - __builtin_convertvector(h, sat_f2);
    const sat_bf2 l = __builtin_convertvector(d, sat_bf2);
    *hi = __builtin_bit_cast(uint32_t, h);
    *lo = __builtin_bit_cast(uint32_t, l);
#endif
}

SAT_DEVICE uint32_t sat_cvt2_pk(float a, float b) {
#if defined(SAT_HIPEMU)
    return ((uint32_t)(uint16_t)sat_f32_to_bf16(b) << 16) | (uint16_t)sat_f32_to_bf16(a);
#else
    typedef __bf16 sat_bf2 __attribute__((ext_vector_type(2)));
    typedef float sat_f2 __attribute__((ext_vector_type(2)));
    const sat_f2 v = {a, b};
    return __builtin_bit_cast(uint32_t, __builtin_convertvector(v, sat_bf2));
#endif
}

#if defined(SAT_HIPEMU)
#define SAT_UNIFORM(x) (x)
#else
#define SAT_UNIFORM(x) __builtin_amdgcn_readfirstlane(x)
#endif

SAT_DEVICE void sat_xcd_tile(int L, int nshare, int nouter, int* share_idx, int* outer_idx) {
    const int ngroups = nouter >> 3;
    const int per_group = 8 * nshare;
    if (L < ngroups * per_group) {
        const int grp = L / per_group, rem = L - grp * per_group;
        *share_idx = rem >> 3;
        *outer_idx = grp * 8 + (rem & 7);
    } else {
        const int R = L - ngroups * per_group;
        *share_idx = R % nshare;
        *outer_idx = ngroups * 8 + R / nshare;
    }
}

template <int B, class T>
SAT_DEVICE T& sat_pick(T& a, T& b) {
    if constexpr (B == 0) return a;
    else return b;
}

SAT_DEVICE float sat_wave_sum(float v) {
    for (int m = 32; m >= 1; m >>= 1) v += __shfl_xor(v, m);
    return v;
}
SAT_DEVICE float sat_half_sum(float v) {
    for (int m = 16; m >= 1; m >>= 1) v += __shfl_xor(v, m);
    return v;
}

SAT_DEVICE void sat_sincos2(float y, float* s2y, float* c2y) {
    const float hi = y * 0.31830987334251404f;
    float lo = fmaf(y, 0.31830987334251404f, -hi);
    lo = fmaf(y, 1.2841276486e-08f, lo);
#if defined(SAT_HIPEMU)
    const float f = (hi - floorf(hi)) + lo;
    *s2y = sinf(6.283185307179586f * f);
    *c2y = cosf(6.283185307179586f * f);
#else
    const float f = __builtin_amdgcn_fractf(hi) + lo;
    *s2y = __builtin_amdgcn_sinf(f);
    *c2y = __builtin_amdgcn_cosf(f);
#endif
}
SAT_DEVICE float sat_sin2(float y) {
    float s, c;
    sat_sincos2(y, &s, &c);
    return fmaf(-0.5f, c, 0.5f);
}

SAT_DEVICE float sat_snake(float x, float a, float ib) {
    return fmaf(ib, sat_sin2(x * a), x);
}

#if defined(SAT_HIPEMU)
static inline void sat_glds16(const void* g, void* lds_wave_base) { memcpy((char*)lds_wave_base + 16 * hipemu::lane_id(), g, 16); }
static inline void sat_glds4(const void* g, void* lds_wave_base) { memcpy((char*)lds_wave_base + 4 * hipemu::lane_id(), g, 4); }
#define SAT_WAIT_VMCNT(n)
#define SAT_RAW_BARRIER() hipemu::block_barrier()
#define SAT_WAIT_LGKM0()
#define SAT_SCHED_FENCE()
static inline void sat_wave_sync() { int z = 0; (void)hipemu::wave_exchange(&z, sizeof(z)); }
#define SAT_SETPRIO(x)
#define SAT_SCHED_GROUP(mask, n)
static inline bool sat_wave_any(bool v) {
    int x = v ? 1 : 0;
    for (int m = 32; m >= 1; m >>= 1) x |= __shfl_xor(x, m);
    return x != 0;
}
#else
SAT_DEVICE void sat_glds16(const void* g, void* lds_wave_base) {
    __builtin_amdgcn_global_load_lds((const __attribute__((address_space(1))) void*)g,
                                     (__attribute__((address_space(3))) void*)lds_wave_base, 16, 0, 0);
}
SAT_DEVICE void sat_glds4(const void* g, void* lds_wave_base) {
    __builtin_amdgcn_global_load_lds((const __attribute__((address_space(1))) void*)g,
                                     (__attribute__((address_space(3))) void*)lds_wave_base, 4, 0, 0);
}
#define SAT_WAIT_VMCNT(n) asm volatile("s_waitcnt vmcnt(%0)" ::"n"(n) : "memory")
#define SAT_RAW_BARRIER() __builtin_amdgcn_s_barrier()
#define SAT_WAIT_LGKM0() asm volatile("s_waitcnt lgkmcnt(0)" ::: "memory")
#define SAT_SCHED_FENCE() __builtin_amdgcn_sched_barrier(0)
SAT_DEVICE void sat_wave_sync() { __builtin_amdgcn_wave_barrier(); }
#define SAT_SETPRIO(x) __builtin_amdgcn_s_setprio(x)
#define SAT_SCHED_GROUP(mask, n) __builtin_amdgcn_sched_group_barrier(mask, n, 0)
SAT_DEVICE bool sat_wave_any(bool v) { return __builtin_amdgcn_ballot_w64(v) != 0; }
#endif

#if defined(SAT_WITH_MFMA_PRIO)
#define SAT_MFMA_PRIO(x) SAT_SETPRIO(x)
#else
#define SAT_MFMA_PRIO(x)
#endif

void sat_set_error(const char* msg);
int sat_check_launch(const char* what);
int sat_cu_count();

#if defined(SAT_HIPEMU)
#define SAT_LAUNCH(kernel, grid, block, stream, params) \
    hipemu::launch((grid), (block), [=]() { kernel(params); })
#else
#define SAT_LAUNCH(kernel, grid, block, stream, params) \
    hipLaunchKernelGGL(kernel, (grid), (block), 0, (hipStream_t)(stream), params)
#endif

static inline int sat_cdiv(int a, int b) { return (a + b - 1) / b; }
static inline long long sat_cdivll(long long a, long long b) { return (a + b - 1) / b; }
```

### stable_audio_tools_amd/functional.py

```python
import torch

from . import ops as _ops_mod
from .ops import PACK_CONV_DGRAD, PACK_CONV_FWD, PACK_POLYPHASE


def _ops(ops):
    return ops if ops is not None else _ops_mod.get_ops()


class SumAllFn(torch.autograd.Function):

    @staticmethod
    def forward(ctx, x, ops=None):
        ctx.in_shape, ctx.in_dtype = x.shape, x.dtype
        return _ops(ops).sum_all(x.detach())

    @staticmethod
    def backward(ctx, g):
        return g.to(ctx.in_dtype).expand(ctx.in_shape), None


def sum_all(x, ops=None):
    return SumAllFn.apply(x, ops)


def mean_all(x, ops=None):
    return SumAllFn.apply(x, ops) / x.numel()


class DerivedCache:

    def __init__(self):
        self.items = {}

    def get(self, name, sources, make):
        from . import _caches
        if not _caches.trackable(*sources):
            return make()
        key = tuple((t.data_ptr(), _caches.version_of(t), t.device) for t in sources if t is not None) + _caches.epoch_of(*sources)
        hit = self.items.get(name)
        if hit is None or hit[0] != key:
            hit = (key, make())
            self.items[name] = hit
        return hit[1]


def _cached(cache, name, sources, make):
    return make() if cache is None else cache.get(name, sources, make)


class WeightNormFn(torch.autograd.Function):
    @staticmethod
    def forward(ctx, v, g, ops=None):
        ops = _ops(ops)
        v = v.contiguous()
        gf = g.contiguous().view(-1)
        w, norm = ops.wn_fold(v, gf)
        ctx.save_for_backward(v, gf, norm)
        ctx.ops = ops
        ctx.g_shape = g.shape
        return w

    @staticmethod
    def backward(ctx, dw):
        v, gf, norm = ctx.saved_tensors
        dv, dg = ctx.ops.wn_grad(v, gf, norm, dw.contiguous())
        return dv, dg.view(ctx.g_shape), None


def _conv_dgrad(ops, dy, w, k, stride, dil, pad, cin, tin, dsnake, res=None, out=None, emit=None):
    if stride == 1:
        if (res is None and out is None and emit is None and ops.edge_ok(w.shape[0], cin, k, 1, dil, (k - 1) * dil - pad) and tin == dy.shape[2]
                and (dsnake is None or w.shape[0] <= 2)):
            return ops.edge_conv(dy, w, (k - 1) * dil - pad, mode=1, dsnake=dsnake)
        if ops.bf16x3_ok(k, 1, dil):
            q = ops.k7q_applicable(w.shape[0], k, 1, dil, (k - 1) * dil - pad, cin)
            return ops.conv1d_bf16x3(dy, ops.pack_bf16x3(w, mode=1, q=q), cin, k, 1, dil, (k - 1) * dil - pad, tout=tin,
                                     dsnake=dsnake, res=res, out=out, emit=emit)
        wpb = ops.pack(w, PACK_CONV_DGRAD)
        return ops.conv1d(dy, wpb, cin, k, 1, dil, (k - 1) * dil - pad, tout=tin, dsnake=dsnake, res=res, out=out)
    if out is not None:
        raise NotImplementedError("_conv_dgrad(out=...) is only plumbed through the stride-1 kernels")
    if ops.bf16x3_ok(k, stride, dil, transposed=True):
        return ops.convtr1d_bf16x3(dy, ops.pack_bf16x3(w, mode=2, stride=stride), cin, k, stride, pad, tout=tin,
                                   dsnake=dsnake, res=res)
    wpb = ops.pack(w, PACK_POLYPHASE, stride)
    return ops.convtr1d(dy, wpb, cin, k, stride, pad, tout=tin, dsnake=dsnake, res=res)


def _conv_wgrad(ops, dy, x, k, stride, dil, pad, snake, bias_grad=False, raw=False):
    if ops.edge_ok(x.shape[1], dy.shape[1], k, stride, dil, pad) and dy.shape[2] == x.shape[2] and (snake is None or dy.shape[1] <= 2):
        return ops.edge_conv_wgrad(dy, x, k, pad, snake=snake, dy_rowsum=bias_grad, raw=raw)
    if ops.wgrad7_bf16x3_ok(x.shape[1], k, stride, dil):
        return ops.conv_wgrad7_bf16x3(dy, x, dil, pad, snake=snake, dy_rowsum=bias_grad, raw=raw)
    return ops.conv_wgrad(dy, x, k, stride, dil, pad, snake=snake, snake_on=2, lo_rowsum=bias_grad, raw=raw)


def _wn_forward(ops, v, g):
    v = v.contiguous()
    gf = g.contiguous().view(-1)
    w, norm = ops.wn_fold(v, gf)
    return w, (v, gf, norm)


def _wn_backward(ops, slabs, saved, g_shape, bias_partial=None):
    v, gf, norm = saved
    out = ops.wn_grad_splits(slabs, v, gf, norm, bias_partial=bias_partial)
    return (out[0], out[1].view(g_shape)) + tuple(out[2:])


def _conv_fwd(ops, x, w, stride, dil, pad, bias=None, snake=None, res=None, tanh_out=False, dsnake=None, tout=None, cache=None, emit=None):
    cout, cin, k = w.shape
    if (res is None and ops.edge_ok(cin, cout, k, stride, dil, pad) and (tout is None or tout == x.shape[2])
            and (snake is None or cout <= 2) and (dsnake is None or cin <= 2) and (emit is None or cin <= 2)):
        return ops.edge_conv(x, w, pad, bias=bias, snake=snake, tanh_out=tanh_out, dsnake=dsnake, emit=emit)
    if ops.bf16x3_ok(k, stride, dil):
        q = ops.k7q_applicable(cin, k, stride, dil, pad, cout)
        planes = _cached(cache, "pack_fwd_q" if q else "pack_fwd", (w,), lambda: ops.pack_bf16x3(w, stride=stride, q=q))
        sconsts = _cached(cache, "snake", snake, lambda: ops.snake_consts(snake[0], snake[1])) if snake is not None else None
        return ops.conv1d_bf16x3(x, planes, cout, k, stride, dil, pad, tout=tout, bias=bias,
                                 snake=snake, res=res, tanh_out=tanh_out, dsnake=dsnake, sconsts=sconsts, emit=emit)
    return ops.conv1d(x, _cached(cache, "pack_fwd32", (w,), lambda: ops.pack(w, PACK_CONV_FWD)), cout, k, stride, dil, pad, tout=tout,
                      bias=bias, snake=snake, res=res, tanh_out=tanh_out, dsnake=dsnake)


def _convtr_fwd(ops, x, w, stride, pad, bias=None, snake=None, cache=None):
    cin, cout, k = w.shape
    if ops.bf16x3_ok(k, stride, 1, transposed=True):
        planes = _cached(cache, "pack_tr", (w,), lambda: ops.pack_bf16x3(w, mode=2, stride=stride))
        sconsts = _cached(cache, "snake", snake, lambda: ops.snake_consts(snake[0], snake[1])) if snake is not None else None
        return ops.convtr1d_bf16x3(x, planes, cout, k, stride, pad, bias=bias, snake=snake, sconsts=sconsts)
    return ops.convtr1d(x, _cached(cache, "pack_tr32", (w,), lambda: ops.pack(w, PACK_POLYPHASE, stride)), cout, k, stride, pad,
                        bias=bias, snake=snake)


class SnakeConv1dFn(torch.autograd.Function):

    @staticmethod
    def forward(ctx, x, alpha, beta, w, bias, res, stride, dil, pad, tanh_out, ops=None, cache=None, next_snake=None, g=None):
        ops = _ops(ops)
        x = x.contiguous()
        wn = ()
        if g is not None:
            w, wn = _wn_forward(ops, w, g)
        w = w.contiguous()
        cout, cin, k = w.shape
        snake = (alpha.contiguous(), beta.contiguous()) if alpha is not None else None
        emit = None
        if next_snake is not None and not tanh_out:
            tout_ = (x.shape[2] + 2 * pad - dil * (k - 1) - 1) // stride + 1
            if ((ops.emit_ok(cout, k, stride, tout_, next_snake[2]) and ops.bf16x3_ok(k, stride, dil))
                    or (res is None and snake is None and ops.edge_emit_ok(cin, cout, k, stride, dil, pad, next_snake[2]))):
                emit = {"snake": (next_snake[0].detach(), next_snake[1].detach())}
        y = _conv_fwd(ops, x, w, stride, dil, pad, bias=bias, snake=snake,
                      res=res.contiguous() if res is not None else None, tanh_out=tanh_out, cache=cache, emit=emit)
        ctx.ops = ops
        ctx.cfg = (stride, dil, pad, tanh_out, bias is not None, res is not None, alpha is not None)
        ctx.g_shape = g.shape if g is not None else None
        ctx.save_for_backward(x, alpha, beta, w, y if tanh_out else None, *wn)
        return y

    @staticmethod
    def backward(ctx, dy):
        ops = ctx.ops
        stride, dil, pad, tanh_out, has_bias, has_res, has_snake = ctx.cfg
        x, alpha, beta, w, y = ctx.saved_tensors[:5]
        wn = ctx.saved_tensors[5:]
        cout, cin, k = w.shape
        dy = dy.contiguous()
        if tanh_out:
            dy = dy * (1.0 - y * y)
        snake = (alpha, beta) if has_snake else None
        dres = dy if has_res else None
        dw = dbias = dg = None
        if ctx.needs_input_grad[3] or (wn and ctx.needs_input_grad[13]):
            dw = _conv_wgrad(ops, dy, x, k, stride, dil, pad, snake, bias_grad=has_bias, raw=bool(wn))
            if has_bias:
                dw, dbias = dw
            if wn:
                dw, dg, *rest = _wn_backward(ops, dw, wn, ctx.g_shape, bias_partial=dbias)
                if has_bias:
                    dbias = rest[0]
        elif has_bias:
            dbias = ops.rowsum(dy)
        dx = da = db = None
        if has_snake:
            dx, da, db = _conv_dgrad(ops, dy, w, k, stride, dil, pad, cin, x.shape[2], (x, alpha, beta))
        elif ctx.needs_input_grad[0]:
            dx = _conv_dgrad(ops, dy, w, k, stride, dil, pad, cin, x.shape[2], None)
        return dx, da, db, dw, dbias, dres, None, None, None, None, None, None, None, dg


class SnakeConvTr1dFn(torch.autograd.Function):

    @staticmethod
    def forward(ctx, x, alpha, beta, w, bias, stride, pad, ops=None, cache=None, g=None):
        ops = _ops(ops)
        x = x.contiguous()
        wn = ()
        if g is not None:
            w, wn = _wn_forward(ops, w, g)
        w = w.contiguous()
        cin, cout, k = w.shape
        snake = (alpha.contiguous(), beta.contiguous()) if alpha is not None else None
        y = _convtr_fwd(ops, x, w, stride, pad, bias=bias, snake=snake, cache=cache)
        ctx.ops = ops
        ctx.cfg = (stride, pad, bias is not None, alpha is not None)
        ctx.g_shape = g.shape if g is not None else None
        ctx.save_for_backward(x, alpha, beta, w, *wn)
        return y

    @staticmethod
    def backward(ctx, dy):
        ops = ctx.ops
        stride, pad, has_bias, has_snake = ctx.cfg
        x, alpha, beta, w = ctx.saved_tensors[:4]
        wn = ctx.saved_tensors[4:]
        cin, cout, k = w.shape
        dy = dy.contiguous()
        snake = (alpha, beta) if has_snake else None
        dbias = ops.rowsum(dy) if has_bias else None
        dw = ops.conv_wgrad(x, dy, k, stride, 1, pad, snake=snake, snake_on=1, raw=bool(wn))
        dg = None
        if wn:
            dw, dg = _wn_backward(ops, dw, wn, ctx.g_shape)
        dx = da = db = None
        if has_snake:
            dx, da, db = _conv_fwd(ops, dy, w, stride, 1, pad, dsnake=(x, alpha, beta), tout=x.shape[2])
        elif ctx.needs_input_grad[0]:
            dx = _conv_fwd(ops, dy, w, stride, 1, pad, tout=x.shape[2])
        return dx, da, db, dw, dbias, None, None, None, None, dg


class ResidualUnitFn(torch.autograd.Function):

    @staticmethod
    def forward(ctx, x, a1, b1, w1, bias1, a2, b2, w2, bias2, dil, ops=None, recompute=False, caches=None, next_snake=None, fuse=False,
                g1=None, g2=None):
        ops = _ops(ops)
        x = x.contiguous()
        wn1 = wn2 = ()
        if g1 is not None:
            w1, wn1 = _wn_forward(ops, w1, g1)
        if g2 is not None:
            w2, wn2 = _wn_forward(ops, w2, g2)
        w1 = w1.contiguous()
        w2 = w2.contiguous()
        c = x.shape[1]
        k1 = w1.shape[2]
        pad = dil * (k1 - 1) // 2
        c1, c2 = caches if caches is not None else (None, None)
        emit = None
        if next_snake is not None and ops.emit_ok(c, w2.shape[2], 1, x.shape[2], next_snake[2]):
            emit = {"snake": (next_snake[0].detach(), next_snake[1].detach())}
        if fuse and w2.shape[2] == 1 and w1.shape[0] == c and ops.ru_fused_ok(c, k1, dil, x.shape[2]):
            w7q = _cached(c1, "pack_q7", (w1,), lambda: ops.pack_k7q(w1))
            w1q = _cached(c2, "pack_q1", (w2,), lambda: ops.pack_k7q(w2))
            sc = None
            if c1 is not None and c2 is not None:
                sc = (_cached(c1, "snake", (a1, b1), lambda: ops.snake_consts(a1, b1)), _cached(c2, "snake", (a2, b2), lambda: ops.snake_consts(a2, b2)))
            h, y = ops.residual_unit_fwd(x, (a1, b1), w7q, bias1, (a2, b2), w1q, bias2, k1, dil, keep_h=ctx is not None and not recompute and fuse != "nokeep",
                                         emit=emit, sconsts=sc)
        else:
            h = _conv_fwd(ops, x, w1, 1, dil, pad, bias=bias1, snake=(a1, b1), cache=c1)
            y = _conv_fwd(ops, h, w2, 1, 1, 0, bias=bias2, snake=(a2, b2), res=x, cache=c2, emit=emit)
        ctx.ops = ops
        ctx.dil = dil
        ctx.recompute = bool(recompute)
        ctx.g_shapes = (g1.shape if g1 is not None else None, g2.shape if g2 is not None else None)
        ctx.save_for_backward(x, None if recompute else h, a1, b1, w1, a2, b2, w2, bias1 if recompute else None, *wn1, *wn2)
        return y

    @staticmethod
    def backward(ctx, dy):
        ops = ctx.ops
        x, h, a1, b1, w1, a2, b2, w2, bias1 = ctx.saved_tensors[:9]
        gs1, gs2 = ctx.g_shapes
        rest = ctx.saved_tensors[9:]
        wn1 = rest[:3] if gs1 is not None else ()
        wn2 = rest[len(wn1):] if gs2 is not None else ()
        dil = ctx.dil
        c = x.shape[1]
        k1, k2 = w1.shape[2], w2.shape[2]
        pad1 = dil * (k1 - 1) // 2
        t = x.shape[2]
        dy = dy.contiguous()
        if ctx.recompute:
            h = _conv_fwd(ops, x, w1, 1, dil, pad1, bias=bias1, snake=(a1, b1))
        want_emit = ops.emit_ok(w1.shape[0], k2, 1, t, dil) and ops.k7q_applicable(w1.shape[0], k1, 1, dil, pad1, c)
        if k2 == 1 and w2.shape[0] == c and w1.shape[0] == c and ops.ru_k1_bwd_ok(dy.shape[0], c, t):
            dh, da2, db2, dw2, dbias2, dbias1 = ops.ru_k1_bwd(dy, h, w2, (a2, b2), emit=want_emit, raw=bool(wn2))
            dw1 = _conv_wgrad(ops, dh, x, k1, 1, dil, pad1, (a1, b1), bias_grad=False, raw=bool(wn1))
        else:
            dw2, dbias2 = ops.conv_wgrad(dy, h, k2, 1, 1, 0, snake=(a2, b2), snake_on=2, lo_rowsum=True, raw=bool(wn2))
            dh, da2, db2 = _conv_dgrad(ops, dy, w2, k2, 1, 1, 0, c, t, (h, a2, b2), emit={"snake": None} if want_emit else None)
            dw1, dbias1 = _conv_wgrad(ops, dh, x, k1, 1, dil, pad1, (a1, b1), bias_grad=True, raw=bool(wn1))
        dg1 = dg2 = None
        if wn1:
            if dbias1.dim() == 2:
                dw1, dg1, dbias1 = _wn_backward(ops, dw1, wn1, gs1, bias_partial=dbias1)
            else:
                dw1, dg1 = _wn_backward(ops, dw1, wn1, gs1)
        if wn2:
            if dbias2.dim() == 2:
                dw2, dg2, dbias2 = _wn_backward(ops, dw2, wn2, gs2, bias_partial=dbias2)
            else:
                dw2, dg2 = _wn_backward(ops, dw2, wn2, gs2)
        dx, da1, db1 = _conv_dgrad(ops, dh, w1, k1, 1, dil, pad1, c, t, (x, a1, b1), res=dy)
        return dx, da1, db1, dw1, dbias1, da2, db2, dw2, dbias2, None, None, None, None, None, None, dg1, dg2


class VaeSampleFn(torch.autograd.Function):

    @staticmethod
    def forward(ctx, pre, noise, ops=None):
        ops = _ops(ops)
        pre = pre.contiguous()
        noise = noise.contiguous()
        z, kl = ops.vae_sample_fwd(pre, noise)
        ctx.ops = ops
        ctx.save_for_backward(pre, noise)
        return z, kl

    @staticmethod
    def backward(ctx, dz, dkl):
        pre, noise = ctx.saved_tensors
        dpre = ctx.ops.vae_sample_bwd(pre, noise, dz.contiguous() if dz is not None else None,
                                      dkl.contiguous() if dkl is not None else None)
        return dpre, None, None
```

### stable_audio_tools_amd/ops.py

```python
import ctypes

import torch

from . import _caches, _lib

PACK_CONV_FWD = 0
PACK_CONV_DGRAD = 1
PACK_POLYPHASE = 2


def _ptr(t):
    if t is None:
        return None
    return ctypes.c_void_p(t.data_ptr())


def _keep_zeros(shape, dtype, device):
    with torch.inference_mode(False):
        return torch.zeros(shape, dtype=dtype, device=device)


def _keep_empty(shape, dtype, device):
    with torch.inference_mode(False):
        return torch.empty(shape, dtype=dtype, device=device)


class WgradSlabs:
    __slots__ = ("partial", "nsplit", "dims", "strides")

    def __init__(self, partial, nsplit, dims, strides):
        self.partial, self.nsplit, self.dims, self.strides = partial, int(nsplit), tuple(int(d) for d in dims), tuple(int(x) for x in strides)

    @property
    def count(self):
        return self.partial.shape[1]

    def reduce(self, ops):
        m, n, k = self.dims
        part = self.partial if self.count == m * n * k else self.partial[:, :m * n * k].contiguous()
        flat = ops._reduce_rows(part, self.nsplit, m * n * k)
        if self.strides == (n * k, k, 1):
            return flat.view(m, n, k)
        if self.strides == (n, 1, m * n):
            return flat.view(k, m, n).permute(1, 2, 0).contiguous()
        raise ValueError("WgradSlabs.reduce: unknown slab layout %s" % (self.strides,))


class SatOps:
    def __init__(self, cdll):
        self.lib = cdll
        self.simulator = bool(cdll.sat_is_simulator())

    def _stream(self, t):
        if self.simulator:
            return None
        return ctypes.c_void_p(torch.cuda.current_stream(t.device).cuda_stream)

    def _chk(self, status):
        if status != 0:
            raise RuntimeError(self.lib.sat_last_error().decode())

    def _f32(self, *tensors):
        for t in tensors:
            if t is None:
                continue
            if t.dtype != torch.float32:
                raise TypeError(f"expected float32 tensor, got {t.dtype}")
            if not t.is_contiguous():
                raise ValueError("expected contiguous tensor")
            if not self.simulator and not t.is_cuda:
                raise RuntimeError("stable_audio_tools_amd kernels need CUDA(HIP) tensors; there is no CPU path")

    def wn_fold(self, v, g):
        self._f32(v, g)
        d0 = v.shape[0]
        r = v.numel() // d0
        w = torch.empty_like(v)
        norm = torch.empty(d0, dtype=torch.float32, device=v.device)
        self._chk(self.lib.sat_wn_fold(_ptr(v), _ptr(g), _ptr(w), _ptr(norm), d0, r, self._stream(v)))
        return w, norm

    def wn_grad(self, v, g, norm, dw):
        self._f32(v, g, norm, dw)
        d0 = v.shape[0]
        r = v.numel() // d0
        dv = torch.empty_like(v)
        dg = torch.empty_like(g)
        self._chk(self.lib.sat_wn_grad(_ptr(v), _ptr(g), _ptr(norm), _ptr(dw), _ptr(dv), _ptr(dg), d0, r, self._stream(v)))
        return dv, dg

    wn_fused = True

    def wn_grad_splits(self, slabs, v, g, norm, bias_partial=None):
        self._f32(v, g, norm, slabs.partial, bias_partial)
        m, n, k = slabs.dims
        if tuple(v.shape) != (m, n, k):
            raise ValueError("wn_grad_splits: slabs of a %s weight gradient for a %s weight" % ((m, n, k), tuple(v.shape)))
        dv = torch.empty_like(v)
        dg = torch.empty_like(g)
        dbias, cols = None, 0
        if bias_partial is not None:
            if bias_partial.dim() != 2 or bias_partial.shape[0] != m:
                raise ValueError("wn_grad_splits: bias_partial must be (D0, R)")
            cols = bias_partial.shape[1]
            dbias = torch.empty(m, dtype=torch.float32, device=v.device)
        so_m, so_n, so_k = slabs.strides
        self._chk(self.lib.sat_wn_grad_splits(_ptr(slabs.partial), slabs.nsplit, slabs.count, so_m, so_n, so_k, _ptr(v), _ptr(g), _ptr(norm),
                                              _ptr(dv), _ptr(dg), m, n, k, _ptr(bias_partial), cols, _ptr(dbias), self._stream(v)))
        return (dv, dg) if bias_partial is None else (dv, dg, dbias)

    def pack(self, w, mode, stride=1):
        self._f32(w)
        d0, d1, k = w.shape
        out = torch.empty(w.numel(), dtype=torch.float32, device=w.device)
        self._chk(self.lib.sat_pack_weights(_ptr(w), _ptr(out), d0, d1, k, stride, mode, self._stream(w)))
        return out

    def _reduce_rows(self, partial, rows, count, scale=1.0):
        out = torch.empty(count, dtype=torch.float32, device=partial.device)
        self._chk(self.lib.sat_reduce_splits(_ptr(partial), _ptr(out), count, rows, scale, 0, self._stream(partial)))
        return out

    def _sum_pair(self, pda, pdb):
        c, r = pda.shape
        both = self.rowsum(pda._base.view(1, 2 * c, r) if pda._base is not None else torch.stack([pda, pdb]).view(1, 2 * c, r))
        return both[:c], both[c:]

    def _sum_last(self, partial):
        c, r = partial.shape
        return self.rowsum(partial.view(1, c, r))

    def conv1d(self, x, w_packed, cout, k, stride=1, dil=1, pad=0, tout=None, bias=None, snake=None, res=None,
               tanh_out=False, dsnake=None, out=None):
        b, cin, tin = x.shape
        if tout is None:
            tout = (tin + 2 * pad - dil * (k - 1) - 1) // stride + 1
        alpha, beta = snake if snake is not None else (None, None)
        self._f32(x, w_packed, bias, alpha, beta, res)
        y = self._conv_out(out, b, cout, tout, x.device)
        x2 = a2 = b2 = pda = pdb = None
        rows = 0
        if dsnake is not None:
            x2, a2, b2 = dsnake
            self._f32(x2, a2, b2)
            rows = self.lib.sat_conv1d_partial_rows(b, tout)
            pda, pdb = torch.empty(2, cout, rows, dtype=torch.float32, device=x.device).unbind(0)
        self._chk(self.lib.sat_conv1d(_ptr(x), _ptr(w_packed), _ptr(bias), _ptr(alpha), _ptr(beta), _ptr(res), _ptr(y),
                                      _ptr(x2), _ptr(a2), _ptr(b2), _ptr(pda), _ptr(pdb),
                                      b, cin, cout, tin, tout, k, stride, dil, pad, int(tanh_out), self._stream(x)))
        if dsnake is not None:
            return (y, *self._sum_pair(pda, pdb))
        return y

    use_bf16x3 = True

    edge_convs = True

    def edge_ok(self, cin, cout, k, stride, dil, pad):
        return bool(self.edge_convs) and bool(self.lib.sat_edge_conv_ok(cin, cout, k, stride, dil, pad))

    def edge_conv(self, x, w, pad, mode=0, bias=None, snake=None, tanh_out=False, dsnake=None, emit=None):
        b, cin, t = x.shape
        k = w.shape[2]
        cout = w.shape[0] if mode == 0 else w.shape[1]
        alpha, beta = snake if snake is not None else (None, None)
        self._f32(x, w, bias, alpha, beta)
        y = torch.empty(b, cout, t, dtype=torch.float32, device=x.device)
        x2 = a2 = b2 = pda = pdb = None
        if dsnake is not None:
            x2, a2, b2 = dsnake
            self._f32(x2, a2, b2)
            rows = self.lib.sat_edge_conv_partial_rows(b, t)
            pda, pdb = torch.empty(2, cout, rows, dtype=torch.float32, device=x.device).unbind(0)
        ehi = elo = ela = elb = None
        erows = 0
        if emit is not None:
            esnake = emit.get("snake")
            if esnake is not None:
                ela, elb = esnake
                self._f32(ela, elb)
            ehi, elo, erows = self._emit_planes(b, cout, t, x.device, self._stream(x))
        self._chk(self.lib.sat_edge_conv(_ptr(x), _ptr(w), _ptr(bias), _ptr(alpha), _ptr(beta), _ptr(y), _ptr(x2), _ptr(a2), _ptr(b2),
                                         _ptr(pda), _ptr(pdb), _ptr(ehi), _ptr(elo), _ptr(ela), _ptr(elb), erows, b, cin, cout, t, k, pad, mode,
                                         int(tanh_out), self._stream(x)))
        if emit is not None:
            self._note_emitted(y, emit.get("snake"), ehi, elo, erows)
        if dsnake is not None:
            return (y, *self._sum_pair(pda, pdb))
        return y

    def edge_conv_wgrad(self, dy, x, k, pad, snake=None, dy_rowsum=False, raw=False):
        b, m, t = dy.shape
        n = x.shape[1]
        alpha, beta = snake if snake is not None else (None, None)
        self._f32(dy, x, alpha, beta)
        nsplit = self.lib.sat_edge_conv_wgrad_nsplit(b, m, n, t)
        partial = torch.empty(nsplit, m * n * k, dtype=torch.float32, device=dy.device)
        fused = dy_rowsum and n <= 2
        rs = torch.empty(m, nsplit, dtype=torch.float32, device=dy.device) if fused else None
        self._chk(self.lib.sat_edge_conv_wgrad(_ptr(dy), _ptr(x), _ptr(alpha), _ptr(beta), _ptr(partial), _ptr(rs), b, m, n, t, k, pad,
                                               self._stream(dy)))
        slabs = WgradSlabs(partial, nsplit, (m, n, k), (n * k, k, 1))
        dw = slabs if raw else slabs.reduce(self)
        if not dy_rowsum:
            return dw
        if raw:
            return dw, (rs if fused else self.rowsum(dy, partial=True))
        return dw, (self._sum_last(rs) if fused else self.rowsum(dy))

    def bf16x3_ok(self, k, stride, dil, transposed=False):
        if not self.use_bf16x3:
            return False
        if transposed or stride > 1:
            return k == 2 * stride and stride & (stride - 1) == 0 and dil == 1
        return k == 1 or (2 <= k <= 4 and dil == 1) or (5 <= k <= 8 and (k - 1) * dil <= 62)

    k7q = True
    k7q_persist = True
    k7q_dma_in_mfma = True
    k7q_min_cin = 64
    k7q_min_cout = 128
    k7q_wide_cin = 512

    def k7q_applicable(self, cin, k, stride, dil, pad, cout=None):
        return (self.k7q and self.use_bf16x3 and stride == 1 and 5 <= k <= 7 and 0 <= pad <= 32
                and (k - 1) * dil <= 62 and cin >= self.k7q_min_cin
                and (cout is None or cout >= self.k7q_min_cout or cin >= self.k7q_wide_cin))

    def pack_bf16x3(self, w, mode=0, stride=1, q=False):
        self._f32(w)
        d0, d1, k = w.shape
        if q:
            n = self.lib.sat_pack_weights_k7q_size(d0, d1, k, mode)
            if n <= 0 or stride != 1:
                raise RuntimeError("sat_pack_weights_k7q: unsupported shape")
            hi = torch.empty(n, dtype=torch.int16, device=w.device)
            lo = torch.empty(n, dtype=torch.int16, device=w.device)
            self._chk(self.lib.sat_pack_weights_k7q(_ptr(w), _ptr(hi), _ptr(lo), d0, d1, k, mode, self._stream(w)))
            return hi, lo, "q"
        n = self.lib.sat_pack_weights_bf16x3_size(d0, d1, k, stride, mode)
        if n <= 0:
            raise RuntimeError("sat_pack_weights_bf16x3: unsupported shape")
        hi = torch.empty(n, dtype=torch.int16, device=w.device)
        lo = torch.empty(n, dtype=torch.int16, device=w.device)
        self._chk(self.lib.sat_pack_weights_bf16x3(_ptr(w), _ptr(hi), _ptr(lo), d0, d1, k, stride, mode, self._stream(w)))
        return hi, lo

    def snake_consts(self, alpha, beta):
        self._f32(alpha, beta)
        a = torch.empty_like(alpha)
        ib = torch.empty_like(beta)
        self._chk(self.lib.sat_snake_consts(_ptr(alpha), _ptr(beta), _ptr(a), _ptr(ib), alpha.numel(), self._stream(alpha)))
        return a, ib

    def _conv_out(self, out, b, cout, tout, device):
        if out is None:
            return torch.empty(b, cout, tout, dtype=torch.float32, device=device)
        if tuple(out.shape) != (b, cout, tout) or not out.is_contiguous():
            raise ValueError("conv out= must be a dense (B, Cout, Tout) tensor")
        self._f32(out)
        return out

    def _bf16x3_call(self, fn, rows, x, w_planes, cout, tout, dims, bias, snake, res, tanh_out, dsnake, out=None, sconsts=None, emit=None):
        b, cin, tin = x.shape
        self._f32(x, bias, res)
        sa = sib = None
        if snake is not None:
            sa, sib = sconsts if sconsts is not None else self.snake_consts(snake[0], snake[1])
        y = self._conv_out(out, b, cout, tout, x.device)
        x2 = a2 = b2 = pda = pdb = None
        if dsnake is not None:
            x2, a2, b2 = dsnake
            self._f32(x2, a2, b2)
            pda, pdb = torch.empty(2, cout, rows, dtype=torch.float32, device=x.device).unbind(0)
        if emit is not None:
            esnake = emit.get("snake")
            ea = eib = None
            if esnake is not None:
                ea, eib = self.snake_consts(esnake[0], esnake[1])
            ehi, elo, erows = self._emit_planes(b, cout, tout, x.device, self._stream(x))
            self._chk(self.lib.sat_conv1d_bf16x3_emit(_ptr(x), _ptr(w_planes[0]), _ptr(w_planes[1]), _ptr(bias), _ptr(sa), _ptr(sib),
                                                      _ptr(res), _ptr(y), _ptr(x2), _ptr(a2), _ptr(b2), _ptr(pda), _ptr(pdb),
                                                      b, cin, cout, tin, tout, *dims, int(tanh_out), _ptr(ehi), _ptr(elo), _ptr(ea), _ptr(eib),
                                                      erows, self._stream(x)))
            self._note_emitted(y, esnake, ehi, elo, erows)
            if dsnake is not None:
                return (y, *self._sum_pair(pda, pdb))
            return y
        self._chk(fn(_ptr(x), _ptr(w_planes[0]), _ptr(w_planes[1]), _ptr(bias), _ptr(sa), _ptr(sib),
                     _ptr(res), _ptr(y), _ptr(x2), _ptr(a2), _ptr(b2), _ptr(pda), _ptr(pdb),
                     b, cin, cout, tin, tout, *dims, int(tanh_out), self._stream(x)))
        if dsnake is not None:
            return (y, *self._sum_pair(pda, pdb))
        return y

    ru_fused = True

    def ru_fused_ok(self, c, k, dil, t):
        return (self.ru_fused and self.use_bf16x3 and self.k7q and self.k7q_min_cin <= c <= 128
                and 5 <= k <= 7 and (k - 1) * dil <= 62 and (k - 1) * dil % 2 == 0 and (k - 1) * dil // 2 <= 32 and t % 4 == 0)

    def pack_k7q(self, w, mode=0):
        self._f32(w)
        d0, d1, k = w.shape
        n = self.lib.sat_pack_weights_k7q_size(d0, d1, k, mode)
        if n <= 0:
            raise RuntimeError("sat_pack_weights_k7q: unsupported shape")
        hi = torch.empty(n, dtype=torch.int16, device=w.device)
        lo = torch.empty(n, dtype=torch.int16, device=w.device)
        self._chk(self.lib.sat_pack_weights_k7q(_ptr(w), _ptr(hi), _ptr(lo), d0, d1, k, mode, self._stream(w)))
        return hi, lo

    def residual_unit_fwd(self, x, snake1, w7q, bias1, snake2, w1q, bias2, k, dil, keep_h=True, emit=None, sconsts=None):
        b, c, t = x.shape
        self._f32(x, bias1, bias2)
        pad = (k - 1) * dil // 2
        st = self._stream(x)
        sa1, sib1 = sconsts[0] if sconsts is not None else self.snake_consts(snake1[0], snake1[1])
        sa2, sib2 = sconsts[1] if sconsts is not None else self.snake_consts(snake2[0], snake2[1])
        em = self._take_emitted(x, snake1)
        if em is not None:
            hi, lo, rows = em["hi"], em["lo"], em["rows"]
        else:
            rows = self.lib.sat_conv1d_k7_plane_rows(t, t, pad)
            c8 = (c + 7) // 8
            need = 2 * b * c8 * rows * 8
            wkey = ("k7p", x.device, st.value if st is not None else 0)
            ws = self.__dict__.setdefault("_planes", {}).get(wkey)
            if ws is None or ws.numel() < need:
                ws = _keep_empty(need, torch.int16, x.device)
                self._planes[wkey] = ws
            hi, lo = ws[:need // 2], ws[need // 2:need]
            self._chk(self.lib.sat_conv1d_k7_planes(_ptr(x), _ptr(sa1), _ptr(sib1), _ptr(hi), _ptr(lo), b, c, t, rows, st))
        h = torch.empty_like(x) if keep_h else None
        y = torch.empty_like(x)
        ehi = elo = ea = eib = None
        erows = 0
        if emit is not None:
            esnake = emit.get("snake")
            if esnake is not None:
                ea, eib = self.snake_consts(esnake[0], esnake[1])
            ehi, elo, erows = self._emit_planes(b, c, t, x.device, st)
            if ehi.data_ptr() == hi.data_ptr():
                ehi, elo, erows = self._emit_planes(b, c, t, x.device, st, alt=True)
        self._chk(self.lib.sat_residual_unit_fwd(_ptr(hi), _ptr(lo), rows, _ptr(w7q[0]), _ptr(w7q[1]), _ptr(bias1), _ptr(sa2), _ptr(sib2),
                                                 _ptr(w1q[0]), _ptr(w1q[1]), _ptr(bias2), _ptr(x), _ptr(h), _ptr(y), b, c, t, k, dil, pad,
                                                 _ptr(ehi), _ptr(elo), _ptr(ea), _ptr(eib), erows, st))
        if emit is not None:
            self._note_emitted(y, emit.get("snake"), ehi, elo, erows)
        return h, y

    k7_emit = True

    @staticmethod
    def _snake_key(snake):
        return None if snake is None else (snake[0].data_ptr(), snake[1].data_ptr(), _caches.version_of(snake[0]), _caches.version_of(snake[1]))

    def _note_emitted(self, y, snake, hi, lo, rows):
        if not _caches.trackable(y, *(snake or ())):
            self._emitted = None
            return
        self._emitted = {"ptr": y.data_ptr(), "shape": tuple(y.shape), "ver": _caches.version_of(y), "snake": self._snake_key(snake),
                         "hi": hi, "lo": lo, "rows": rows}

    def emit_ok(self, cout, k, stride, tout, consumer_dil):
        if not (self.k7_emit and self.use_bf16x3 and self.k7q_applicable(cout, 7, 1, consumer_dil, 3 * consumer_dil, cout)):
            return False
        generic = (stride == 1 and k <= 4) or stride > 1
        return generic and tout % 4 == 0

    def edge_emit_ok(self, cin, cout, k, stride, dil, pad, consumer_dil):
        return (self.k7_emit and self.use_bf16x3 and cin <= 2 and self.edge_ok(cin, cout, k, stride, dil, pad)
                and self.k7q_applicable(cout, 7, 1, consumer_dil, 3 * consumer_dil, cout))

    def _emit_planes(self, b, c, t, device, st, alt=False):
        rows = self.lib.sat_conv1d_k7_plane_rows(t, t, 0)
        key = ("emit", b, c, t, device, st.value if st is not None else 0, alt)
        cache = self.__dict__.setdefault("_planes", {})
        pl = cache.get(key)
        if pl is None:
            n = b * ((c + 7) // 8) * rows * 8
            pl = (_keep_zeros(n, torch.int16, device), _keep_zeros(n, torch.int16, device), rows)
            cache[key] = pl
        return pl

    def _take_emitted(self, x, snake):
        e = self.__dict__.get("_emitted")
        if e is None:
            return None
        self._emitted = None
        if (e["ptr"] == x.data_ptr() and e["shape"] == tuple(x.shape) and _caches.trackable(x) and e["ver"] == _caches.version_of(x)
                and e["snake"] == self._snake_key(snake)):
            return e
        return None

    def conv1d_bf16x3(self, x, w_planes, cout, k, stride=1, dil=1, pad=0, tout=None, bias=None, snake=None, res=None,
                      tanh_out=False, dsnake=None, out=None, sconsts=None, emit=None):
        b, cin, tin = x.shape
        if tout is None:
            tout = (tin + 2 * pad - dil * (k - 1) - 1) // stride + 1
        rows = self.lib.sat_conv1d_bf16x3_partial_rows(b, tout, k, stride)
        if len(w_planes) == 3:
            if not (stride == 1 and 5 <= k <= 7 and 0 <= pad <= 32 and (k - 1) * dil <= 62):
                raise ValueError("conv1d_bf16x3: q-packed weights need stride 1, 5 <= K <= 7, pad <= 32, (K-1)*dil <= 62")
            return self._k7_planes_call(rows, x, w_planes, cout, tout, k, dil, pad, bias, snake, res, tanh_out, dsnake, out, sconsts)
        return self._bf16x3_call(self.lib.sat_conv1d_bf16x3, rows, x, w_planes, cout, tout, (k, stride, dil, pad),
                                 bias, snake, res, tanh_out, dsnake, out, sconsts, emit)

    def _k7_planes_call(self, prows, x, w_planes, cout, tout, k, dil, pad, bias, snake, res, tanh_out, dsnake, out=None, sconsts=None):
        b, cin, tin = x.shape
        self._f32(x, bias, res)
        sa = sib = None
        if snake is not None:
            sa, sib = sconsts if sconsts is not None else self.snake_consts(snake[0], snake[1])
        st = self._stream(x)
        em = self._take_emitted(x, snake)
        if em is not None:
            hi, lo, rows = em["hi"], em["lo"], em["rows"]
        else:
            rows = self.lib.sat_conv1d_k7_plane_rows(tin, tout, pad)
            c8 = (cin + 7) // 8
            need = 2 * b * c8 * rows * 8
            wkey = ("k7p", x.device, st.value if st is not None else 0)
            ws = self.__dict__.setdefault("_planes", {}).get(wkey)
            if ws is None or ws.numel() < need:
                ws = _keep_empty(need, torch.int16, x.device)
                self._planes[wkey] = ws
            hi, lo = ws[:need // 2], ws[need // 2:need]
            self._chk(self.lib.sat_conv1d_k7_planes(_ptr(x), _ptr(sa), _ptr(sib), _ptr(hi), _ptr(lo), b, cin, tin, rows, st))
        y = self._conv_out(out, b, cout, tout, x.device)
        x2 = a2 = b2 = pda = pdb = None
        if dsnake is not None:
            x2, a2, b2 = dsnake
            self._f32(x2, a2, b2)
            pda, pdb = torch.empty(2, cout, prows, dtype=torch.float32, device=x.device).unbind(0)
        self._chk(self.lib.sat_conv1d_bf16x3_planesq(_ptr(hi), _ptr(lo), rows, _ptr(w_planes[0]), _ptr(w_planes[1]), _ptr(bias), _ptr(res),
                                                     _ptr(y), _ptr(x2), _ptr(a2), _ptr(b2), _ptr(pda), _ptr(pdb), b, cin, cout, tin, tout,
                                                     k, dil, pad, int(tanh_out), {True: 0, False: 1, "force": 2}[self.k7q_persist] | (4 if self.k7q_dma_in_mfma else 0), st))
        if dsnake is not None:
            return (y, *self._sum_pair(pda, pdb))
        return y

    def convtr1d_bf16x3(self, x, w_planes, cout, k, stride, pad, tout=None, bias=None, snake=None, res=None,
                        tanh_out=False, dsnake=None, sconsts=None):
        b, cin, tin = x.shape
        if tout is None:
            tout = (tin - 1) * stride - 2 * pad + k
        rows = self.lib.sat_convtr1d_bf16x3_partial_rows(b, tout, stride, pad)
        return self._bf16x3_call(self.lib.sat_convtr1d_bf16x3, rows, x, w_planes, cout, tout, (k, stride, pad),
                                 bias, snake, res, tanh_out, dsnake, None, sconsts)

    def convtr1d(self, x, w_packed, cout, k, stride, pad, tout=None, bias=None, snake=None, res=None,
                 tanh_out=False, dsnake=None):
        b, cin, tin = x.shape
        if tout is None:
            tout = (tin - 1) * stride - 2 * pad + k
        alpha, beta = snake if snake is not None else (None, None)
        self._f32(x, w_packed, bias, alpha, beta, res)
        y = torch.empty(b, cout, tout, dtype=torch.float32, device=x.device)
        x2 = a2 = b2 = pda = pdb = None
        rows = 0
        if dsnake is not None:
            x2, a2, b2 = dsnake
            self._f32(x2, a2, b2)
            rows = self.lib.sat_convtr1d_partial_rows(b, tout, stride, pad)
            if rows < 0:
                raise RuntimeError("sat_convtr1d: unsupported stride")
            pda, pdb = torch.empty(2, cout, rows, dtype=torch.float32, device=x.device).unbind(0)
        self._chk(self.lib.sat_convtr1d(_ptr(x), _ptr(w_packed), _ptr(bias), _ptr(alpha), _ptr(beta), _ptr(res), _ptr(y),
                                        _ptr(x2), _ptr(a2), _ptr(b2), _ptr(pda), _ptr(pdb),
                                        b, cin, cout, tin, tout, k, stride, pad, int(tanh_out), self._stream(x)))
        if dsnake is not None:
            return (y, *self._sum_pair(pda, pdb))
        return y

    def conv_wgrad(self, lo, hi, k, stride=1, dil=1, pad=0, snake=None, snake_on=0, lo_rowsum=False, raw=False):
        bsz, m, tlo = lo.shape
        _, n, thi = hi.shape
        alpha, beta = snake if snake is not None else (None, None)
        self._f32(lo, hi, alpha, beta)
        x3 = self.use_bf16x3 and dil == 1 and self.lib.sat_conv_wgrad_bf16x3_nsplit(bsz, m, n, tlo, k, stride) > 0
        if x3:
            nsplit = self.lib.sat_conv_wgrad_bf16x3_nsplit(bsz, m, n, tlo, k, stride)
        else:
            nsplit = self.lib.sat_conv_wgrad_nsplit(bsz, m, n, tlo, k, stride, dil)
        if nsplit < 0:
            raise RuntimeError("sat_conv_wgrad: receptive field too large")
        partial = torch.empty(nsplit, m * n * k, dtype=torch.float32, device=lo.device)
        so_m, so_n, so_k = n * k, k, 1
        rs = None
        if x3:
            fused = lo_rowsum and not (snake is not None and snake_on == 1)
            rs = torch.empty(m, nsplit, dtype=torch.float32, device=lo.device) if fused else None
            self._chk(self.lib.sat_conv_wgrad_bf16x3(_ptr(lo), _ptr(hi), _ptr(alpha), _ptr(beta),
                                                     snake_on if snake is not None else 0, _ptr(partial), so_m, so_n, so_k,
                                                     bsz, m, n, tlo, thi, k, stride, pad, _ptr(rs), self._stream(lo)))
        else:
            self._chk(self.lib.sat_conv_wgrad(_ptr(lo), _ptr(hi), _ptr(alpha), _ptr(beta), snake_on if snake is not None else 0,
                                              _ptr(partial), so_m, so_n, so_k, bsz, m, n, tlo, thi, k, stride, dil, pad,
                                              self._stream(lo)))
        slabs = WgradSlabs(partial, nsplit, (m, n, k), (so_m, so_n, so_k))
        dw = slabs if raw else slabs.reduce(self)
        if not lo_rowsum:
            return dw
        if raw:
            return dw, (rs if rs is not None else self.rowsum(lo, partial=True))
        return dw, (self._sum_last(rs) if rs is not None else self.rowsum(lo))

    ru_k1_fused = True

    def ru_k1_bwd_ok(self, b, c, t):
        return self.ru_k1_fused and self.use_bf16x3 and self.lib.sat_ru_k1_bwd_nsplit(b, c, t) > 0

    def ru_k1_pack(self, w2):
        self._f32(w2)
        c = w2.shape[0]
        planes = torch.empty(2, c * c, dtype=torch.int16, device=w2.device)
        self._chk(self.lib.sat_ru_k1_pack(_ptr(w2), _ptr(planes[0]), _ptr(planes[1]), c, self._stream(w2)))
        return planes[0], planes[1]

    def ru_k1_bwd(self, dy, h, w2, snake2, emit=False, wt=None, raw=False):
        b, c, t = dy.shape
        a2, b2 = snake2
        self._f32(dy, h, w2, a2, b2)
        ns = self.lib.sat_ru_k1_bwd_nsplit(b, c, t)
        if ns <= 0:
            raise RuntimeError("ru_k1_bwd: shape not served by the fused kernel (ru_k1_bwd_ok)")
        st = self._stream(dy)
        wt_hi, wt_lo = wt if wt is not None else self.ru_k1_pack(w2)
        dh = torch.empty_like(dy)
        slabs = torch.empty(ns, c * c, dtype=torch.float32, device=dy.device)
        part = torch.empty(4 * c, ns, dtype=torch.float32, device=dy.device)
        ehi = elo = None
        erows = 0
        if emit:
            ehi, elo, erows = self._emit_planes(b, c, t, dy.device, st)
        self._chk(self.lib.sat_ru_k1_bwd(_ptr(dy), _ptr(h), _ptr(wt_hi), _ptr(wt_lo), _ptr(a2), _ptr(b2), _ptr(dh), _ptr(ehi), _ptr(elo), erows,
                                         _ptr(slabs), _ptr(part), b, c, t, st))
        if emit:
            self._note_emitted(dh, None, ehi, elo, erows)
        dw2 = WgradSlabs(slabs, ns, (c, c, 1), (c, 1, 1))
        if not raw:
            dw2 = dw2.reduce(self)
        sums = self._sum_last(part)
        return dh, sums[:c], sums[c:2 * c], dw2, sums[3 * c:], sums[2 * c:3 * c]

    def wgrad7_bf16x3_ok(self, n_in, k, stride, dil):
        return self.use_bf16x3 and stride == 1 and k == 7 and dil in (1, 3, 9)

    def conv_wgrad7_bf16x3(self, dy, x, dil, pad, snake=None, dy_rowsum=False, raw=False):
        b, m, t = dy.shape
        n = x.shape[1]
        alpha, beta = snake if snake is not None else (None, None)
        self._f32(dy, x, alpha, beta)
        nsplit = self.lib.sat_conv_wgrad7_bf16x3_nsplit(b, m, n, t)
        partial = torch.empty(nsplit, m * n * 7, dtype=torch.float32, device=dy.device)
        fused = dy_rowsum and self.lib.sat_conv_wgrad7_bf16x3_fuses_rowsum(b, m, n, t) == 1
        rs = torch.empty(m, nsplit, dtype=torch.float32, device=dy.device) if fused else None
        self._chk(self.lib.sat_conv_wgrad7_bf16x3(_ptr(dy), _ptr(x), _ptr(alpha), _ptr(beta), _ptr(partial), n, 1, m * n,
                                                  b, m, n, t, dil, pad, _ptr(rs), self._stream(dy)))
        slabs = WgradSlabs(partial, nsplit, (m, n, 7), (n, 1, m * n))
        dw = slabs if raw else slabs.reduce(self)
        if not dy_rowsum:
            return dw
        if raw:
            return dw, (rs if fused else self.rowsum(dy, partial=True))
        return dw, (self._sum_last(rs) if fused else self.rowsum(dy))

    def rowsum(self, x, partial=False):
        self._f32(x)
        b, c, t = x.shape
        while True:
            ns = self.lib.sat_rowsum_nsplit(t)
            part = torch.empty(c, ns, dtype=torch.float32, device=x.device)
            self._chk(self.lib.sat_rowsum(_ptr(x), _ptr(part), b, c, t, self._stream(x)))
            if partial:
                return part
            if ns == 1:
                return part.view(c)
            x, b, t = part, 1, ns

    def sum_all(self, x):
        x = x.contiguous()
        if x.dtype != torch.float32:
            x = x.float()
        n = x.numel()
        if n == 0:
            return torch.zeros((), dtype=torch.float32, device=x.device)
        if n > 1 << 29:
            flat = x.view(-1)
            return torch.stack([self.sum_all(piece) for piece in flat.split(1 << 29)]).sum()
        if x.data_ptr() % 16:
            x = x.clone()
        return self.rowsum(x.view(1, 1, n)).view(())

    def vae_sample_fwd(self, pre, noise):
        self._f32(pre, noise)
        b, c2, t = pre.shape
        c = c2 // 2
        z = torch.empty(b, c, t, dtype=torch.float32, device=pre.device)
        nb = self.lib.sat_vae_nblocks(b * c * t)
        klp = torch.empty(nb, dtype=torch.float32, device=pre.device)
        self._chk(self.lib.sat_vae_sample_fwd(_ptr(pre), _ptr(noise), _ptr(z), _ptr(klp), b, c, t, self._stream(pre)))
        kl = (self._sum_last(klp.view(1, nb)) * (1.0 / (b * t))).view(())
        return z, kl

    def vae_sample_bwd(self, pre, noise, dz, dkl):
        self._f32(pre, noise, dz, dkl)
        b, c2, t = pre.shape
        c = c2 // 2
        dpre = torch.empty_like(pre)
        self._chk(self.lib.sat_vae_sample_bwd(_ptr(pre), _ptr(noise), _ptr(dz), _ptr(dkl), _ptr(dpre), b, c, t,
                                              self._stream(pre)))
        return dpre

    def fir(self, x, taps, adjoint=False):
        self._f32(x, taps)
        n, t = x.shape
        y = torch.empty_like(x)
        self._chk(self.lib.sat_fir(_ptr(x), _ptr(taps), _ptr(y), n, t, taps.numel(), int(adjoint), self._stream(x)))
        return y

    def stft_sums(self, x, y, views, n_fft, hop):
        self._f32(x, y, views)
        ni, c, t = x.shape
        nv = views.shape[0]
        tiles = self.lib.sat_stft_tiles(n_fft, hop, t)
        if tiles < 0:
            raise RuntimeError(f"sat_stft: unsupported n_fft={n_fft} hop={hop} T={t}")
        partial = torch.empty(ni * nv * 3, tiles, dtype=torch.float32, device=x.device)
        self._chk(self.lib.sat_stft_fwd(_ptr(x), _ptr(y), _ptr(views), _ptr(partial), ni, c, t, nv, n_fft, hop, self._stream(x)))
        return self._sum_last(partial).view(ni, nv, 3)

    def stft_backward(self, x, y, views, coef, planes, n_fft, hop, wrt_x=False):
        self._f32(x, y, views, coef, planes)
        ni, c, t = x.shape
        nv = views.shape[0]
        if tuple(planes.shape) != (4, ni, c, t):
            raise ValueError("stft_backward: planes must be (4, NI, C, T)")
        self._chk(self.lib.sat_stft_bwd(_ptr(x), _ptr(y), _ptr(views), _ptr(coef), _ptr(planes), ni, c, t, nv, n_fft, hop,
                                        int(wrt_x), self._stream(x)))

    def rows_pack(self, x, kh, dil_t, pad_t, pad_w, pitch, lead):
        self._f32(x)
        b, c, t, w = x.shape
        buf = torch.empty(2 * lead + b * c * kh * t * pitch, dtype=torch.float32, device=x.device)
        self._chk(self.lib.sat_rows_pack(_ptr(x), _ptr(buf), b, c, t, w, kh, dil_t, pad_t, pad_w, pitch, lead, self._stream(x)))
        return buf

    def rows_pack_bwd(self, dbuf, shape, kh, dil_t, pad_t, pad_w, pitch, lead):
        self._f32(dbuf)
        b, c, t, w = shape
        dx = torch.empty(shape, dtype=torch.float32, device=dbuf.device)
        self._chk(self.lib.sat_rows_pack_bwd(_ptr(dbuf), _ptr(dx), b, c, t, w, kh, dil_t, pad_t, pad_w, pitch, lead, self._stream(dbuf)))
        return dx

    def release_workspaces(self):
        for name in ("_planes", "_disc_pool", "_disc_gen", "_disc_geoms"):
            d = self.__dict__.get(name)
            if d is not None:
                d.clear()
        self._emitted = None
        self._disc_emitted = None

    def disc_geom(self, frames, w):
        key = ("disc_geom", frames, w)
        cache = self.__dict__.setdefault("_disc_geoms", {})
        g = cache.get(key)
        if g is None:
            out = [ctypes.c_int() for _ in range(4)]
            self._chk(self.lib.sat_disc_geom(frames, w, *[ctypes.byref(o) for o in out]))
            g = cache[key] = tuple(o.value for o in out)
        return g

    def _disc_plane_buf(self, b, c, frames, w, device, slot):
        P, L, lead, rows = self.disc_geom(frames, w)
        c8 = (c + 7) // 8
        n = b * c8 * rows * 8
        key = (device, 0 if c8 == 1 else 1, slot)
        gen = self.__dict__.setdefault("_disc_gen", {})
        gen[key] = gen.get(key, 0) + 1
        pool = self.__dict__.setdefault("_disc_pool", {})
        e = pool.get(key)
        if e is None or e["cap"] < n:
            e = pool[key] = {"hi": _keep_zeros(n, torch.int16, device), "lo": _keep_zeros(n, torch.int16, device),
                             "cap": n, "geom": (b, c8, frames, w)}
        elif e["geom"] != (b, c8, frames, w):
            for t in (e["hi"], e["lo"]):
                v = t[:n].view(b * c8, rows, 8)
                v[:, :lead].zero_()
                v[:, lead + L:].zero_()
            e["geom"] = (b, c8, frames, w)
        return e["hi"][:n], e["lo"][:n]

    def disc_register(self, t, planes, c, frames, w, slot):
        key = (t.device, 0 if (c + 7) // 8 == 1 else 1, slot)
        if not _caches.trackable(t):
            self._disc_emitted = None
            return
        self._disc_emitted = {"ptr": t.data_ptr(), "ver": _caches.version_of(t), "key": key, "gen": self.__dict__.get("_disc_gen", {}).get(key, 0),
                              "geom": (t.shape[0], (c + 7) // 8, frames, w), "planes": planes, "slot": slot}

    def disc_take(self, h, c, frames, w):
        e = self.__dict__.get("_disc_emitted")
        self._disc_emitted = None
        if (e is not None and e["ptr"] == h.data_ptr() and _caches.trackable(h) and e["ver"] == _caches.version_of(h) and e["geom"] == (h.shape[0], (c + 7) // 8, frames, w)
                and self.__dict__.get("_disc_gen", {}).get(e["key"], 0) == e["gen"]):
            return e["planes"], e["slot"]
        return self.disc_planes(h, frames, w, slot=0)[1], 0

    def disc_planes(self, src, frames, w, out=None, slope=1.0, want_dst=False, want_planes=True, slot=0, fm_sign=None, fm_coef=None):
        self._f32(src, out, fm_coef)
        if fm_sign is not None and (fm_sign.dtype != torch.int8 or not fm_sign.is_contiguous() or fm_sign.numel() != src.numel()):
            raise ValueError("disc_planes: fm_sign must be a contiguous int8 tensor of src's size")
        b, c = src.shape[0], src.shape[1]
        P, L, lead, rows = self.disc_geom(frames, w)
        pitched = src.dim() == 3
        if pitched and src.shape[2] != L or not pitched and tuple(src.shape[2:]) != (frames, w):
            raise ValueError("disc_planes: shape does not match (frames, w)")
        dst = torch.empty(b, c, L, dtype=torch.float32, device=src.device) if want_dst else None
        pl = self._disc_plane_buf(b, c, frames, w, src.device, slot) if want_planes else None
        self._chk(self.lib.sat_disc_planes(_ptr(src), _ptr(out), _ptr(fm_sign), _ptr(fm_coef), _ptr(dst), _ptr(pl[0]) if pl else None,
                                           _ptr(pl[1]) if pl else None, b, c, frames, w, 1 if pitched else 0, float(slope), self._stream(src)))
        return dst, pl

    def disc_l1_sum(self, a, b, want_sign=False):
        self._f32(a, b)
        partial = torch.empty(self.lib.sat_disc_l1_blocks(), dtype=torch.float32, device=a.device)
        sign = torch.empty(a.shape, dtype=torch.int8, device=a.device) if want_sign else None
        self._chk(self.lib.sat_disc_l1_sum(_ptr(a), _ptr(b), _ptr(partial), _ptr(sign), a.numel(), self._stream(a)))
        return (partial.sum(), sign) if want_sign else partial.sum()

    def disc_pack(self, w4, mode):
        self._f32(w4)
        cout, cin, kh, kw = w4.shape
        n = self.lib.sat_disc_pack_size(cout, cin, kh, kw, mode)
        if n < 0:
            raise ValueError("disc_pack: unsupported kernel shape")
        wq = torch.empty(n, dtype=torch.int16, device=w4.device)
        self._chk(self.lib.sat_disc_pack_weights(_ptr(w4), _ptr(wq), cout, cin, kh, kw, mode, self._stream(w4)))
        return wq

    def disc_conv(self, planes, wq, bias, b, cin, cout, frames, w, kh, kw, dil_t, slope, emit_slot=None, lk_src=None, lk_slope=1.0):
        self._f32(bias, lk_src)
        L = self.disc_geom(frames, w)[1]
        y = torch.empty(b, cout, L, dtype=torch.float32, device=planes[0].device)
        em = self._disc_plane_buf(b, cout, frames, w, y.device, emit_slot) if emit_slot is not None else None
        self._chk(self.lib.sat_disc_conv(_ptr(planes[0]), _ptr(planes[1]), _ptr(wq), _ptr(bias), _ptr(y),
                                         _ptr(em[0]) if em else None, _ptr(em[1]) if em else None, b, cin, cout, frames, w, kh, kw, dil_t,
                                         float(slope), _ptr(lk_src), float(lk_slope), self._stream(y)))
        return y, em

    def disc_wgrad(self, dy, x, frames, w, kh, kw, dil_t):
        self._f32(dy, x)
        b, m, _ = dy.shape
        cin = x.shape[1]
        nsplit = self.lib.sat_disc_wgrad_nsplit(b, m, cin, kh, frames, w)
        mp, npad = (m + 63) // 64 * 64, (kh * cin + 63) // 64 * 64
        partial = torch.empty(nsplit, kw * mp * npad, dtype=torch.float32, device=dy.device)
        self._chk(self.lib.sat_disc_wgrad(_ptr(dy), _ptr(x), _ptr(partial), b, m, cin, frames, w, kh, kw, dil_t, self._stream(dy)))
        dw = self._reduce_rows(partial, nsplit, kw * mp * npad).view(kw, mp, npad)[:, :m, :kh * cin]
        return dw.reshape(kw, m, kh, cin).permute(1, 3, 2, 0).contiguous()

    def rows_unpack(self, y, t, w, pad_w, pitch, slope):
        self._f32(y)
        b, c = y.shape[0], y.shape[1]
        out = torch.empty(b, c, t, w, dtype=torch.float32, device=y.device)
        self._chk(self.lib.sat_rows_unpack(_ptr(y), _ptr(out), b, c, t, w, pad_w, pitch, float(slope), self._stream(y)))
        return out

    def rows_unpack_bwd(self, dout, out, pad_w, pitch, slope):
        self._f32(dout, out)
        b, c, t, w = dout.shape
        dy = torch.empty(b, c, t * pitch, dtype=torch.float32, device=dout.device)
        self._chk(self.lib.sat_rows_unpack_bwd(_ptr(dout), _ptr(out), _ptr(dy), b, c, t, w, pad_w, pitch, float(slope), self._stream(dout)))
        return dy

    def spec_fwd(self, x, n_fft, hop):
        self._f32(x)
        ni, c, t = x.shape
        frames = self.lib.sat_spec_frames(n_fft, hop, t)
        if frames < 0:
            raise RuntimeError(f"sat_spec: unsupported n_fft={n_fft} hop={hop} T={t}")
        z = torch.empty(ni, 2 * c, frames, n_fft // 2 + 1, dtype=torch.float32, device=x.device)
        self._chk(self.lib.sat_spec_fwd(_ptr(x), _ptr(z), ni, c, t, n_fft, hop, self._stream(x)))
        return z

    def spec_bwd(self, dz, c, t, n_fft, hop):
        self._f32(dz)
        ni = dz.shape[0]
        planes = torch.zeros(2, ni, c, t, dtype=torch.float32, device=dz.device)
        self._chk(self.lib.sat_spec_bwd(_ptr(dz), _ptr(planes), ni, c, t, n_fft, hop, self._stream(dz)))
        return planes[0] + planes[1]

    def _dt(self, *tensors):
        dt = None
        for t in tensors:
            if t is None:
                continue
            if t.dtype not in (torch.float32, torch.bfloat16):
                raise TypeError(f"DiT kernels take float32 or bfloat16 tensors, got {t.dtype}")
            if dt is not None and t.dtype != dt:
                raise TypeError("mixed dtypes")
            dt = t.dtype
            if not self.simulator and not t.is_cuda:
                raise RuntimeError("stable_audio_tools_amd kernels need CUDA(HIP) tensors; there is no CPU path")
        return 0 if dt == torch.float32 else 1

    def attn_planes(self, t, row_major=True, transposed=False):
        dt = self._dt(t)
        if t.stride(3) != 1:
            raise ValueError("head dim must be contiguous")
        b, h, n, d = t.shape
        npad = (n + 63) // 64 * 64
        split = dt == 0

        def alloc(shape, want):
            return torch.empty(shape, dtype=torch.int16, device=t.device) if want else None
        rm_hi, rm_lo = alloc((b, h, npad, d), row_major), alloc((b, h, npad, d), row_major and split)
        tr_hi, tr_lo = alloc((b, h, d, npad), transposed), alloc((b, h, d, npad), transposed and split)
        self._chk(self.lib.sat_attn_prepare(_ptr(t), t.stride(0), t.stride(1), t.stride(2), _ptr(rm_hi), _ptr(rm_lo),
                                            _ptr(tr_hi), _ptr(tr_lo), b, h, n, npad, dt, self._stream(t)))
        return {"rm": (rm_hi, rm_lo), "tr": (tr_hi, tr_lo), "n": n, "np": npad, "dt": dt}

    def attention(self, q, k, v, scale, need_lse=False, return_planes=False):
        dt = self._dt(q, k, v)
        b, h, nq, d = q.shape
        _, hk, nk, _ = k.shape
        qp = self.attn_planes(q, row_major=True, transposed=return_planes)
        kp = self.attn_planes(k, row_major=True, transposed=return_planes)
        vp = self.attn_planes(v, row_major=return_planes, transposed=True)
        o = torch.empty(b, nq, h * d, dtype=q.dtype, device=q.device)
        lse = torch.empty(b, h, nq, dtype=torch.float32, device=q.device) if (need_lse or return_planes) else None
        if self.cross_ok(h, hk, nk, d, dt):
            self._chk(self.lib.sat_attention_cross_fwd(_ptr(qp["rm"][0]), _ptr(kp["rm"][0]), _ptr(vp["tr"][0]), _ptr(o), _ptr(lse), b, h, hk,
                                                       nq, nk, qp["np"], kp["np"], d, float(scale), self._stream(q)))
        else:
            self._chk(self.lib.sat_attention_fwd(_ptr(qp["rm"][0]), _ptr(qp["rm"][1]), _ptr(kp["rm"][0]), _ptr(kp["rm"][1]),
                                                 _ptr(vp["tr"][0]), _ptr(vp["tr"][1]), _ptr(o), _ptr(lse), b, h, hk, nq, nk,
                                                 qp["np"], kp["np"], d, float(scale), self._fwd_dtype(dt), self._stream(q)))
        out = (o,)
        if need_lse or return_planes:
            out += (lse,)
        if return_planes:
            out += ({"q": qp, "k": kp, "v": vp},)
        return out[0] if len(out) == 1 else out

    def attention_bwd(self, planes, o, do, lse, scale, hkv, nk, out=None):
        dt = self._dt(o, do)
        b, nq, hd = o.shape
        h = hd // 64
        do = do.contiguous()
        dsum = torch.empty(b, h, nq, dtype=torch.float32, device=o.device)
        self._chk(self.lib.sat_attention_rowdot(_ptr(do), _ptr(o), _ptr(dsum), b, h, nq, dt, self._stream(o)))
        gp = self.attn_planes(do.view(b, nq, h, 64).permute(0, 2, 1, 3), row_major=True, transposed=True)
        qp, kp, vp = planes["q"], planes["k"], planes["v"]
        ptrs = [qp["rm"], kp["rm"], vp["rm"], kp["tr"], qp["tr"], gp["rm"], gp["tr"], (None, None)]
        arr = (ctypes.c_void_p * 16)(*[(x.data_ptr() if x is not None else None) for pair in ptrs for x in pair])
        if out is not None:
            dq, dk, dv = out
            if (tuple(dq.shape), tuple(dk.shape), tuple(dv.shape)) != ((b, h, nq, 64), (b, hkv, nk, 64), (b, hkv, nk, 64)) \
                    or not (dq.is_contiguous() and dk.is_contiguous() and dv.is_contiguous()) or {dq.dtype, dk.dtype, dv.dtype} != {o.dtype}:
                raise ValueError("attention_bwd: out must be contiguous (B,H,Nq,64) / (B,Hkv,Nk,64) x 2 tensors in the dtype of o")
        else:
            dq = torch.empty(b, h, nq, 64, dtype=o.dtype, device=o.device)
            dk = torch.empty(b, hkv, nk, 64, dtype=o.dtype, device=o.device)
            dv = torch.empty(b, hkv, nk, 64, dtype=o.dtype, device=o.device)
        if self.cross_ok(h, hkv, nk, 64, dt):
            nbytes = int(self.lib.sat_attention_cross_bwd_ws(b, h, hkv, nq, nk))
            ws = torch.empty(nbytes // 4, dtype=torch.float32, device=o.device)
            self._chk(self.lib.sat_attention_cross_bwd(arr, _ptr(lse), _ptr(dsum), _ptr(dq), _ptr(dk), _ptr(dv), _ptr(ws), nbytes, b, h, hkv,
                                                       nq, nk, qp["np"], kp["np"], 64, float(scale), self._stream(o)))
        else:
            self._chk(self.lib.sat_attention_bwd(arr, _ptr(lse), _ptr(dsum), _ptr(dq), _ptr(dk), _ptr(dv), b, h, hkv, nq, nk,
                                                 qp["np"], kp["np"], 64, float(scale), dt, self._stream(o)))
        return dq, dk, dv

    cross_kernels = True
    train_fused_nodes = True
    ln_residual = True
    cast_pair = True
    attn_q64 = None

    def _fwd_dtype(self, dt):
        if dt != 1 or self.attn_q64 is None:
            return dt
        return 3 if self.attn_q64 else 2

    def cross_ok(self, h, hkv, nk, d, dt):
        return bool(self.cross_kernels) and bool(self.lib.sat_attention_cross_ok(h, hkv, nk, d, dt))

    def layernorm(self, x, gamma, beta=None, scale=None, shift=None, eps=1e-5, save_stats=False):
        dt = self._dt(x, scale, shift)
        self._f32(gamma, beta)
        if not x.is_contiguous():
            raise ValueError("expected contiguous x")
        b, n, d = x.shape
        y = torch.empty_like(x)
        mean = rstd = None
        if save_stats:
            mean = torch.empty(b * n, dtype=torch.float32, device=x.device)
            rstd = torch.empty(b * n, dtype=torch.float32, device=x.device)
        ms = scale.stride(0) if scale is not None else 0
        self._chk(self.lib.sat_layernorm_fwd(_ptr(x), _ptr(gamma), _ptr(beta), _ptr(scale), _ptr(shift), ms, _ptr(y),
                                             _ptr(mean), _ptr(rstd), b * n, d, n, eps, dt, self._stream(x)))
        return (y, mean, rstd) if save_stats else y

    def layernorm_fp8(self, x, gamma, beta=None, scale=None, shift=None, eps=1e-5):
        dt = self._dt(x, scale, shift)
        self._f32(gamma, beta)
        if not x.is_contiguous():
            raise ValueError("expected contiguous x")
        b, n, d = x.shape
        q = torch.empty(b * n, d, dtype=torch.uint8, device=x.device)
        rs = torch.empty(b * n, dtype=torch.float32, device=x.device)
        ms = scale.stride(0) if scale is not None else 0
        rc = self.lib.sat_layernorm_fwd_fp8(_ptr(x), _ptr(gamma), _ptr(beta), _ptr(scale), _ptr(shift), ms, _ptr(q), _ptr(rs),
                                            b * n, d, n, eps, dt, self._stream(x))
        if rc == 2:
            return None
        self._chk(rc)
        return q, rs

    def layernorm_bwd(self, dy, x, gamma, beta, scale, mean, rstd, dres=None):
        dt = self._dt(dy, x, scale, dres)
        if dres is not None and (dres.shape != x.shape or not dres.is_contiguous()):
            raise ValueError("layernorm_bwd: dres must be contiguous with the shape of x")
        b, n, d = x.shape
        dx = torch.empty_like(x)
        nby = self.lib.sat_layernorm_bwd_nblocks(b * n, n)
        part = torch.empty(3, nby, d, dtype=torch.float32, device=x.device)
        ms = scale.stride(0) if scale is not None else 0
        self._chk(self.lib.sat_layernorm_bwd_res(_ptr(dy), _ptr(x), _ptr(gamma), _ptr(beta), _ptr(scale), ms, _ptr(mean),
                                                 _ptr(rstd), _ptr(dres), _ptr(dx), _ptr(part), b * n, d, n, dt, self._stream(x)))
        per_b = nby // b
        dgamma = self._reduce_rows(part[0].contiguous(), nby, d)
        if scale is None:
            return dx, dgamma, None, None
        dscale = torch.stack([self._reduce_rows(part[1, i * per_b:(i + 1) * per_b].contiguous(), per_b, d) for i in range(b)])
        dshift = torch.stack([self._reduce_rows(part[2, i * per_b:(i + 1) * per_b].contiguous(), per_b, d) for i in range(b)])
        return dx, dgamma, dscale, dshift

    def rope_tables(self, inv_freq, n, pos_scale=1.0):
        self._f32(inv_freq)
        half = inv_freq.numel()
        cs = torch.empty(n, half, 2, dtype=torch.float32, device=inv_freq.device)
        self._chk(self.lib.sat_rope_tables(_ptr(inv_freq), _ptr(cs), n, half, float(pos_scale), self._stream(inv_freq)))
        return cs

    def rope_apply_(self, t, cs, transpose=False):
        dt = self._dt(t)
        b, n, h, dh = t.shape
        half = cs.shape[1]
        if t.stride(3) != 1 or 2 * half > dh:
            raise ValueError("bad rotary layout")
        self._chk(self.lib.sat_rope_apply(_ptr(t), _ptr(cs), t.stride(0), t.stride(1), t.stride(2), b, n, h, half,
                                          cs.shape[0] - n, int(transpose), dt, self._stream(t)))
        return t

    def swiglu(self, xin):
        dt = self._dt(xin)
# ... 385 lines not shown
```

Before: 7.771.

## Add planes-based wgrad7 kernel reusing emitted bf16 hi/lo planes and skip dh writes

Adds a new K=7 weight-gradient kernel that reads pre-split bf16 hi/lo planes of dy and the snake-activated input directly via global-to-LDS loads and transposing LDS reads, feeding 32x32x16 MFMAs. The forward conv can keep its activation planes alive for backward, and the k1 residual backward can skip writing dh in f32 when its planes are emitted. The aim is to remove redundant f32 reads, snake recomputation and bf16 splitting in backward. In exchange it adds plane-ownership bookkeeping, a memory budget and runtime checks against using an unwritten dh.

```diff
diff --git a/include/sat_amd.h b/include/sat_amd.h
--- a/include/sat_amd.h
+++ b/include/sat_amd.h
@@ -88,6 +88,13 @@
 int sat_conv_wgrad7_bf16x3_nsplit(int B, int M, int N, int T);
 int sat_conv_wgrad7_bf16x3_fuses_rowsum(int B, int M, int N, int T);
 
+int sat_conv_wgrad7_planes_ok(int B, int M, int N, int T, int dil, int pad, int rows_dy, int rows_act);
+int sat_conv_wgrad7_planes_nsplit(int B, int M, int N, int T);
+int sat_conv_wgrad7_planes(const short* dy_hi, const short* dy_lo, int rows_dy, const short* act_hi, const short* act_lo, int rows_act,
+                           float* partial, long long so_m, long long so_n, long long so_k, int B, int M, int N, int T, int dil, int pad,
+                           void* stream);
+int sat_lds_read_tr16_probe(const short* image, const int* lane_off, short* out, void* stream);
+
 int sat_conv_wgrad_bf16x3(const float* lo, const float* hi, const float* alpha, const float* beta, int snake_on,
                           float* partial, long long so_m, long long so_n, long long so_k, int B, int M, int N, int Tlo,
                           int Thi, int K, int stride, int pad, float* lo_rowsum, void* stream);
diff --git a/stable_audio_tools_amd/_lib.py b/stable_audio_tools_amd/_lib.py
--- a/stable_audio_tools_amd/_lib.py
+++ b/stable_audio_tools_amd/_lib.py
@@ -42,6 +42,10 @@
     "sat_conv_wgrad7_bf16x3": (_I, [_P] * 5 + [_L] * 3 + [_I] * 6 + [_P, _P]),
     "sat_conv_wgrad7_bf16x3_nsplit": (_I, [_I] * 4),
     "sat_conv_wgrad7_bf16x3_fuses_rowsum": (_I, [_I] * 4),
+    "sat_conv_wgrad7_planes_ok": (_I, [_I] * 8),
+    "sat_conv_wgrad7_planes_nsplit": (_I, [_I] * 4),
+    "sat_conv_wgrad7_planes": (_I, [_P, _P, _I, _P, _P, _I, _P] + [_L] * 3 + [_I] * 6 + [_P]),
+    "sat_lds_read_tr16_probe": (_I, [_P] * 4),
     "sat_conv_wgrad_bf16x3": (_I, [_P] * 4 + [_I, _P] + [_L] * 3 + [_I] * 8 + [_P, _P]),
     "sat_conv_wgrad_bf16x3_nsplit": (_I, [_I] * 6),
     "sat_convtr1d": (_I, [_P] * 12 + [_I] * 9 + [_P]),
diff --git a/stable_audio_tools_amd/csrc/conv_wgrad7_planes.h b/stable_audio_tools_amd/csrc/conv_wgrad7_planes.h
--- /dev/null
+++ b/stable_audio_tools_amd/csrc/conv_wgrad7_planes.h
@@ -0,0 +1,118 @@
+#pragma once
+
+#define SAT_WQ_NT 512
+#define SAT_WQ_NI 64
+#define SAT_WQ_LEAD 32
+#define SAT_WQ_DY_CH (64 * 16 + 64)
+#define SAT_WQ_ACT_CH (128 * 16 + 64)
+#define SAT_WQ_DY_PLANE (16 * SAT_WQ_DY_CH)
+#define SAT_WQ_ACT_PLANE (8 * SAT_WQ_ACT_CH)
+#define SAT_WQ_ACT_OFF (2 * SAT_WQ_DY_PLANE)
+#define SAT_WQ_STAGE (SAT_WQ_ACT_OFF + 2 * SAT_WQ_ACT_PLANE)
+
+struct SatWgPlParams {
+    const short* dy_hi;
+    const short* dy_lo;
+    const short* act_hi;
+    const short* act_lo;
+    float* out;
+    long long so_split, so_m, so_n, so_k;
+    int B, M, N, T, pad, rows_dy, rows_act, c8_dy, c8_act;
+    int chunks_per_split, nchunks, nT;
+};
+
+template <int DIL>
+__global__ void __launch_bounds__(SAT_WQ_NT) sat_wgrad7_planes_kernel(SatWgPlParams p) {
+    static_assert(64 + 6 * DIL <= 128, "a stage's activation rows fit two pieces");
+    __shared__ __attribute__((aligned(1024))) char lds[2 * SAT_WQ_STAGE];
+
+    const int tid = threadIdx.x, lane = tid & 63, wave = SAT_UNIFORM(tid >> 6);
+    const int l31 = lane & 31, hi = lane >> 5;
+    int mn_tile, split;
+    sat_xcd_tile(blockIdx.x + gridDim.x * (blockIdx.y + gridDim.y * blockIdx.z), gridDim.x * gridDim.y, gridDim.z, &mn_tile, &split);
+    const int m0 = (mn_tile % (int)gridDim.x) * SAT_CO_T, n0 = (mn_tile / (int)gridDim.x) * SAT_WQ_NI;
+    const int m_w = (wave & 3) * 32, n_w = (wave >> 2) * 32;
+
+    f32x16 acc[7];
+#pragma unroll
+    for (int k = 0; k < 7; ++k)
+#pragma unroll
+        for (int r = 0; r < 16; ++r) acc[k][r] = 0.0f;
+
+    const int c_begin = split * p.chunks_per_split;
+    int c_end = c_begin + p.chunks_per_split;
+    if (c_end > p.nchunks) c_end = p.nchunks;
+    const int nst = c_end - c_begin;
+
+    const unsigned lane8 = (unsigned)lane * 8u;
+    auto issue = [&](int c, int st) {
+        const int ch = c_begin + c;
+        const int b = ch / p.nT;
+        const int tt0 = (ch - b * p.nT) * SAT_WB_TT;
+        char* sb = lds + st * SAT_WQ_STAGE;
+#pragma unroll
+        for (int i = 0; i < 4; ++i) {
+            const int d = wave + 8 * i, pl = d >> 4, g = d & 15;
+            int c8 = (m0 >> 3) + g;
+            c8 = c8 < p.c8_dy ? c8 : p.c8_dy - 1;
+            const short* src = (pl ? p.dy_lo : p.dy_hi) + (((size_t)b * p.c8_dy + c8) * p.rows_dy + SAT_WQ_LEAD + tt0) * 8;
+            sat_glds16_raw(src + lane8, sb + pl * SAT_WQ_DY_PLANE + g * SAT_WQ_DY_CH);
+        }
+#pragma unroll
+        for (int i = 0; i < 4; ++i) {
+            const int a = wave + 8 * i, pl = a >> 4, g = (a >> 1) & 7, part = a & 1;
+            int c8 = (n0 >> 3) + g;
+            c8 = c8 < p.c8_act ? c8 : p.c8_act - 1;
+            const short* src = (pl ? p.act_lo : p.act_hi) +
+                               (((size_t)b * p.c8_act + c8) * p.rows_act + SAT_WQ_LEAD + tt0 - p.pad + part * 64) * 8;
+            sat_glds16_raw(src + lane8, sb + SAT_WQ_ACT_OFF + pl * SAT_WQ_ACT_PLANE + g * SAT_WQ_ACT_CH + part * 1024);
+        }
+    };
+
+    const int gq = lane >> 4, q = (lane >> 2) & 3, pp = lane & 3;
+    const unsigned row_off = (unsigned)((8 * hi + q) * 16 + 8 * (pp & 1));
+    const unsigned a_off = (unsigned)(((m_w >> 3) + 2 * (gq & 1) + (pp >> 1)) * SAT_WQ_DY_CH) + row_off;
+    const unsigned b_off = (unsigned)(SAT_WQ_ACT_OFF + ((n_w >> 3) + 2 * (gq & 1) + (pp >> 1)) * SAT_WQ_ACT_CH) + row_off;
+    auto frag = [&](const char* at) {
+        const bf16x4 v0 = sat_lds_read_tr16_b64(at), v1 = sat_lds_read_tr16_b64(at + 64);
+        return bf16x8{v0[0], v0[1], v0[2], v0[3], v1[0], v1[1], v1[2], v1[3]};
+    };
+    auto compute = [&](int st) {
+        const char* pa = lds + st * SAT_WQ_STAGE + a_off;
+        const char* pb = lds + st * SAT_WQ_STAGE + b_off;
+        SAT_MFMA_PRIO(1);
+#pragma unroll
+        for (int ks = 0; ks < SAT_WB_TT / 16; ++ks) {
+            const bf16x8 a_hi = frag(pa + ks * 256), a_lo = frag(pa + SAT_WQ_DY_PLANE + ks * 256);
+#pragma unroll
+            for (int k = 0; k < 7; ++k) {
+                const bf16x8 b_hi = frag(pb + ks * 256 + k * DIL * 16), b_lo = frag(pb + SAT_WQ_ACT_PLANE + ks * 256 + k * DIL * 16);
+                acc[k] = sat_mfma_32x32x16_bf16(a_hi, b_hi, acc[k]);
+                acc[k] = sat_mfma_32x32x16_bf16(a_lo, b_hi, acc[k]);
+                acc[k] = sat_mfma_32x32x16_bf16(a_hi, b_lo, acc[k]);
+            }
+        }
+        SAT_MFMA_PRIO(0);
+    };
+
+    issue(0, 0);
+    for (int c = 0; c < nst; ++c) {
+        SAT_WAIT_VMCNT(0);
+        SAT_RAW_BARRIER();
+        SAT_SCHED_FENCE();
+        if (c + 1 < nst) issue(c + 1, (c + 1) & 1);
+        compute(c & 1);
+    }
+
+    if (m0 + m_w < p.M) {
+        float* ob = p.out + (size_t)split * p.so_split;
+        const int n = n0 + n_w + l31;
+#pragma unroll
+        for (int k = 0; k < 7; ++k)
+#pragma unroll
+            for (int r = 0; r < 16; ++r) {
+                const int m = m0 + m_w + (r & 3) + 8 * (r >> 2) + 4 * hi;
+                if (m < p.M && n < p.N) ob[(size_t)m * p.so_m + (size_t)n * p.so_n + (size_t)k * p.so_k] = acc[k][r];
+            }
+    }
+}
diff --git a/stable_audio_tools_amd/csrc/conv_wgrad_bf16x3.hip b/stable_audio_tools_amd/csrc/conv_wgrad_bf16x3.hip
--- a/stable_audio_tools_amd/csrc/conv_wgrad_bf16x3.hip
+++ b/stable_audio_tools_amd/csrc/conv_wgrad_bf16x3.hip
@@ -268,6 +268,71 @@
     else if (dil == 3) SAT_LAUNCH(sat_wgrad7_bf16x3_kernel<3>, grid, dim3(256), stream, p);
     else SAT_LAUNCH(sat_wgrad7_bf16x3_kernel<9>, grid, dim3(256), stream, p);
     return sat_check_launch("sat_conv_wgrad7_bf16x3");
+}
+
+#include "conv_wgrad7_planes.h"
+
+struct SatTrProbeParams { const short* image; const int* lane_off; short* out; };
+__global__ void __launch_bounds__(64) sat_lds_read_tr16_probe_kernel(SatTrProbeParams p) {
+    __shared__ __attribute__((aligned(16))) short img[1024];
+    const int lane = threadIdx.x;
+    for (int i = lane; i < 1024; i += 64) img[i] = p.image[i];
+    __syncthreads();
+    const bf16x4 v = sat_lds_read_tr16_b64(reinterpret_cast<const char*>(img) + p.lane_off[lane]);
+#pragma unroll
+    for (int e = 0; e < 4; ++e) p.out[4 * lane + e] = v[e];
+}
+extern "C" int sat_lds_read_tr16_probe(const short* image, const int* lane_off, short* out, void* stream) {
+    if (!image || !lane_off || !out) { sat_set_error("sat_lds_read_tr16_probe: missing buffer"); return 1; }
+    SatTrProbeParams p{image, lane_off, out};
+    SAT_LAUNCH(sat_lds_read_tr16_probe_kernel, dim3(1), dim3(64), stream, p);
+    return sat_check_launch("sat_lds_read_tr16_probe");
+}
+
+extern "C" int sat_conv_wgrad7_planes_ok(int B, int M, int N, int T, int dil, int pad, int rows_dy, int rows_act) {
+    if (B <= 0 || M <= 0 || N < SAT_WQ_NI || T <= 0) return 0;
+    if ((dil != 1 && dil != 3 && dil != 9) || pad < 0 || pad > SAT_WQ_LEAD) return 0;
+    const int nT = sat_cdiv(T, SAT_WB_TT);
+    if (rows_dy < SAT_WQ_LEAD + nT * SAT_WB_TT) return 0;
+    if (rows_act < SAT_WQ_LEAD + (nT - 1) * SAT_WB_TT - pad + 128) return 0;
+    if (rows_act < SAT_WQ_LEAD + T + 6 * dil - pad) return 0;
+    return 1;
+}
+static void sat_wgpl_plan(int B, int M, int N, int T, SatWgBfPlan* pl) {
+    pl->nT = sat_cdiv(T, SAT_WB_TT);
+    pl->nchunks = B * pl->nT;
+    pl->pipe = true;
+    const int tiles = sat_cdiv(M, SAT_CO_T) * sat_cdiv(N, SAT_WQ_NI);
+    int want = 512 / tiles;
+    if (want > pl->nchunks) want = pl->nchunks;
+    if (want < 1) want = 1;
+    pl->cps = sat_cdiv(pl->nchunks, want);
+    pl->nsplit = sat_cdiv(pl->nchunks, pl->cps);
+}
+extern "C" int sat_conv_wgrad7_planes_nsplit(int B, int M, int N, int T) {
+    if (B <= 0 || M <= 0 || N <= 0 || T <= 0) return -1;
+    SatWgBfPlan pl;
+    sat_wgpl_plan(B, M, N, T, &pl);
+    return pl.nsplit;
+}
+extern "C" int sat_conv_wgrad7_planes(const short* dy_hi, const short* dy_lo, int rows_dy, const short* act_hi, const short* act_lo,
+                                      int rows_act, float* partial, long long so_m, long long so_n, long long so_k, int B, int M, int N,
+                                      int T, int dil, int pad, void* stream) {
+    if (!dy_hi || !dy_lo || !act_hi || !act_lo || !partial) { sat_set_error("sat_conv_wgrad7_planes: missing buffer"); return 1; }
+    if (!sat_conv_wgrad7_planes_ok(B, M, N, T, dil, pad, rows_dy, rows_act)) {
+        sat_set_error("sat_conv_wgrad7_planes: shape outside the kernel's contract (sat_conv_wgrad7_planes_ok)");
+        return 1;
+    }
+    if ((((uintptr_t)dy_hi | (uintptr_t)dy_lo | (uintptr_t)act_hi | (uintptr_t)act_lo) & 15) != 0) { sat_set_error("sat_conv_wgrad7_planes: planes must be 16-byte aligned"); return 1; }
+    SatWgBfPlan pl;
+    sat_wgpl_plan(B, M, N, T, &pl);
+    SatWgPlParams p{dy_hi, dy_lo, act_hi, act_lo, partial, (long long)M * N * 7, so_m, so_n, so_k, B, M, N, T, pad, rows_dy, rows_act,
+                    sat_cdiv(M, 8), sat_cdiv(N, 8), pl.cps, pl.nchunks, pl.nT};
+    dim3 grid(sat_cdiv(M, SAT_CO_T), sat_cdiv(N, SAT_WQ_NI), pl.nsplit);
+    if (dil == 1) SAT_LAUNCH((sat_wgrad7_planes_kernel<1>), grid, dim3(SAT_WQ_NT), stream, p);
+    else if (dil == 3) SAT_LAUNCH((sat_wgrad7_planes_kernel<3>), grid, dim3(SAT_WQ_NT), stream, p);
+    else SAT_LAUNCH((sat_wgrad7_planes_kernel<9>), grid, dim3(SAT_WQ_NT), stream, p);
+    return sat_check_launch("sat_conv_wgrad7_planes");
 }
 
 #define SAT_WS_TT 64
diff --git a/stable_audio_tools_amd/csrc/ru_k1_bwd.hip b/stable_audio_tools_amd/csrc/ru_k1_bwd.hip
--- a/stable_audio_tools_amd/csrc/ru_k1_bwd.hip
+++ b/stable_audio_tools_amd/csrc/ru_k1_bwd.hip
@@ -222,7 +222,7 @@
                 out[e] = pre[e] * g.dx;
                 sum_dh[j] += out[e];
             }
-            *reinterpret_cast<f32x4*>(p.dh + ((size_t)b * C + ch) * p.T + t0 + st4) = out;
+            if (p.dh) *reinterpret_cast<f32x4*>(p.dh + ((size_t)b * C + ch) * p.T + t0 + st4) = out;
             if (p.em_hi) {
                 uint32_t h0, l0, h1, l1;
                 sat_split2_pk(out[0], out[1], &h0, &l0);
@@ -313,7 +313,8 @@
         sat_set_error("sat_ru_k1_bwd: needs C == 128 and T % 32 == 0 (sat_ru_k1_bwd_nsplit)");
         return 1;
     }
-    if (!dy || !h || !wt_hi || !wt_lo || !alpha2 || !beta2 || !dh || !dw_partial || !part) { sat_set_error("sat_ru_k1_bwd: missing buffer"); return 1; }
+    if (!dy || !h || !wt_hi || !wt_lo || !alpha2 || !beta2 || !dw_partial || !part) { sat_set_error("sat_ru_k1_bwd: missing buffer"); return 1; }
+    if (!dh && !em_hi) { sat_set_error("sat_ru_k1_bwd: dh may only be NULL when its planes are emitted"); return 1; }
     if ((em_hi == nullptr) != (em_lo == nullptr) || (em_hi && em_rows < SAT_RK_LEAD + T)) { sat_set_error("sat_ru_k1_bwd: bad emission planes"); return 1; }
     if ((((uintptr_t)dy | (uintptr_t)h | (uintptr_t)dh | (uintptr_t)em_hi | (uintptr_t)em_lo | (uintptr_t)wt_hi | (uintptr_t)wt_lo) & 15) != 0) {
         sat_set_error("sat_ru_k1_bwd: buffers must be 16-byte aligned");
diff --git a/stable_audio_tools_amd/csrc/sat_device.h b/stable_audio_tools_amd/csrc/sat_device.h
--- a/stable_audio_tools_amd/csrc/sat_device.h
+++ b/stable_audio_tools_amd/csrc/sat_device.h
@@ -266,6 +266,7 @@
 #if defined(SAT_HIPEMU)
 static inline void sat_glds16(const void* g, void* lds_wave_base) { memcpy((char*)lds_wave_base + 16 * hipemu::lane_id(), g, 16); }
 static inline void sat_glds4(const void* g, void* lds_wave_base) { memcpy((char*)lds_wave_base + 4 * hipemu::lane_id(), g, 4); }
+static inline void sat_glds16_raw(const void* g, void* lds_wave_base) { sat_glds16(g, lds_wave_base); }
 #define SAT_WAIT_VMCNT(n)
 #define SAT_RAW_BARRIER() hipemu::block_barrier()
 #define SAT_WAIT_LGKM0()
@@ -287,6 +288,11 @@
     __builtin_amdgcn_global_load_lds((const __attribute__((address_space(1))) void*)g,
                                      (__attribute__((address_space(3))) void*)lds_wave_base, 4, 0, 0);
 }
+SAT_DEVICE void sat_glds16_raw(const void* g, void* lds_wave_base) {
+    const unsigned m0v = __builtin_amdgcn_readfirstlane((unsigned)(uintptr_t)(__attribute__((address_space(3))) void*)lds_wave_base);
+    unsigned keep;
+    asm volatile("s_mov_b32 %0, m0\n\ts_mov_b32 m0, %2\n\ts_nop 0\n\tglobal_load_lds_dwordx4 %1, off\n\ts_mov_b32 m0, %0" : "=&s"(keep) : "v"(g), "s"(m0v) : "memory");
+}
 #define SAT_WAIT_VMCNT(n) asm volatile("s_waitcnt vmcnt(%0)" ::"n"(n) : "memory")
 #define SAT_RAW_BARRIER() __builtin_amdgcn_s_barrier()
 #define SAT_WAIT_LGKM0() asm volatile("s_waitcnt lgkmcnt(0)" ::: "memory")
@@ -297,6 +303,28 @@
 SAT_DEVICE bool sat_wave_any(bool v) { return __builtin_amdgcn_ballot_w64(v) != 0; }
 #endif
 
+typedef short bf16x4 __attribute__((ext_vector_type(4)));
+#if defined(SAT_HIPEMU)
+static inline bf16x4 sat_lds_read_tr16_b64(const void* lane_addr) {
+    const void* mine = lane_addr;
+    const char* all = hipemu::wave_exchange(&mine, (int)sizeof(mine));
+    const int l = hipemu::lane_id(), g0 = l & ~15, i = l & 15;
+    bf16x4 r;
+    for (int q = 0; q < 4; ++q) {
+        const char* src;
+        memcpy(&src, all + (size_t)(g0 + 4 * q + (i >> 2)) * hipemu::kSlotBytes, sizeof(src));
+        short v;
+        memcpy(&v, src + 2 * (i & 3), 2);
+        r[q] = v;
+    }
+    return r;
+}
+#else
+SAT_DEVICE bf16x4 sat_lds_read_tr16_b64(const void* lane_addr) {
+    return __builtin_amdgcn_ds_read_tr16_b64_v4i16((__attribute__((address_space(3))) bf16x4*)lane_addr);
+}
+#endif
+
 #if defined(SAT_WITH_MFMA_PRIO)
 #define SAT_MFMA_PRIO(x) SAT_SETPRIO(x)
 #else
diff --git a/stable_audio_tools_amd/functional.py b/stable_audio_tools_amd/functional.py
--- a/stable_audio_tools_amd/functional.py
+++ b/stable_audio_tools_amd/functional.py
@@ -1,5 +1,6 @@
 import torch
 
+from . import _caches
 from . import ops as _ops_mod
 from .ops import PACK_CONV_DGRAD, PACK_CONV_FWD, PACK_POLYPHASE
 
@@ -109,7 +110,8 @@
     return (out[0], out[1].view(g_shape)) + tuple(out[2:])
 
 
-def _conv_fwd(ops, x, w, stride, dil, pad, bias=None, snake=None, res=None, tanh_out=False, dsnake=None, tout=None, cache=None, emit=None):
+def _conv_fwd(ops, x, w, stride, dil, pad, bias=None, snake=None, res=None, tanh_out=False, dsnake=None, tout=None, cache=None, emit=None,
+              keep_planes=None):
     cout, cin, k = w.shape
     if (res is None and ops.edge_ok(cin, cout, k, stride, dil, pad) and (tout is None or tout == x.shape[2])
             and (snake is None or cout <= 2) and (dsnake is None or cin <= 2) and (emit is None or cin <= 2)):
@@ -119,7 +121,7 @@
         planes = _cached(cache, "pack_fwd_q" if q else "pack_fwd", (w,), lambda: ops.pack_bf16x3(w, stride=stride, q=q))
         sconsts = _cached(cache, "snake", snake, lambda: ops.snake_consts(snake[0], snake[1])) if snake is not None else None
         return ops.conv1d_bf16x3(x, planes, cout, k, stride, dil, pad, tout=tout, bias=bias,
-                                 snake=snake, res=res, tanh_out=tanh_out, dsnake=dsnake, sconsts=sconsts, emit=emit)
+                                 snake=snake, res=res, tanh_out=tanh_out, dsnake=dsnake, sconsts=sconsts, emit=emit, keep_planes=keep_planes)
     return ops.conv1d(x, _cached(cache, "pack_fwd32", (w,), lambda: ops.pack(w, PACK_CONV_FWD)), cout, k, stride, dil, pad, tout=tout,
                       bias=bias, snake=snake, res=res, tanh_out=tanh_out, dsnake=dsnake)
 
@@ -262,7 +264,10 @@
             h, y = ops.residual_unit_fwd(x, (a1, b1), w7q, bias1, (a2, b2), w1q, bias2, k1, dil, keep_h=ctx is not None and not recompute and fuse != "nokeep",
                                          emit=emit, sconsts=sc)
         else:
-            h = _conv_fwd(ops, x, w1, 1, dil, pad, bias=bias1, snake=(a1, b1), cache=c1)
+            keep = {} if (ops.wgrad7_planes and not recompute and ctx is not None and any(ctx.needs_input_grad)) else None
+            h = _conv_fwd(ops, x, w1, 1, dil, pad, bias=bias1, snake=(a1, b1), cache=c1, keep_planes=keep)
+            if ctx is not None:
+                ctx.k7_planes = keep.get("kept") if keep is not None else None
             y = _conv_fwd(ops, h, w2, 1, 1, 0, bias=bias2, snake=(a2, b2), res=x, cache=c2, emit=emit)
         ctx.ops = ops
         ctx.dil = dil
@@ -288,13 +293,35 @@
         if ctx.recompute:
             h = _conv_fwd(ops, x, w1, 1, dil, pad1, bias=bias1, snake=(a1, b1))
         want_emit = ops.emit_ok(w1.shape[0], k2, 1, t, dil) and ops.k7q_applicable(w1.shape[0], k1, 1, dil, pad1, c)
+        kp = getattr(ctx, "k7_planes", None)
+        bsz = dy.shape[0]
+        skip_dh = False
+        if kp is not None and not (ops.wgrad7_planes and not ctx.recompute and want_emit and k1 == 7 and w1.shape[0] == c
+                                   and kp["gen"] == kp["buf"]["gen"] and kp["ptr"] == x.data_ptr() and kp["shape"] == tuple(x.shape)
+                                   and kp["ver"] == _caches.version_of(x) and kp["snake"] == ops._snake_key((a1, b1))
+                                   and ops.conv_wgrad7_planes_ok(bsz, c, c, t, dil, pad1, kp["buf"]["rows"], kp["buf"]["rows"])):
+            kp = None
+
+        def wgrad1(dh, bias_grad):
+            em = ops._peek_emitted(dh, None) if kp is not None else None
+            if em is None or not ops.conv_wgrad7_planes_ok(bsz, c, c, t, dil, pad1, em["rows"], kp["buf"]["rows"]):
+                return _conv_wgrad(ops, dh, x, k1, 1, dil, pad1, (a1, b1), bias_grad=bias_grad, raw=bool(wn1))
+            dw = ops.conv_wgrad7_planes((em["hi"], em["lo"], em["rows"]), (kp["buf"]["hi"], kp["buf"]["lo"], kp["buf"]["rows"]),
+                                        bsz, c, c, t, dil, pad1, raw=bool(wn1))
+            return (dw, ops.rowsum(dh, partial=bool(wn1))) if bias_grad else dw
         if k2 == 1 and w2.shape[0] == c and w1.shape[0] == c and ops.ru_k1_bwd_ok(dy.shape[0], c, t):
-            dh, da2, db2, dw2, dbias2, dbias1 = ops.ru_k1_bwd(dy, h, w2, (a2, b2), emit=want_emit, raw=bool(wn2))
-            dw1 = _conv_wgrad(ops, dh, x, k1, 1, dil, pad1, (a1, b1), bias_grad=False, raw=bool(wn1))
+            skip_dh = bool(kp is not None and ops.ru_k1_bwd_skip_dh)
+            dh, da2, db2, dw2, dbias2, dbias1 = ops.ru_k1_bwd(dy, h, w2, (a2, b2), emit=want_emit, raw=bool(wn2), skip_dh=skip_dh)
+            try:
+                dw1 = wgrad1(dh, False)
+                if skip_dh:
+                    dx, da1, db1 = _conv_dgrad(ops, dh, w1, k1, 1, dil, pad1, c, t, (x, a1, b1), res=dy)
+            finally:
+                ops.dh_written()
         else:
             dw2, dbias2 = ops.conv_wgrad(dy, h, k2, 1, 1, 0, snake=(a2, b2), snake_on=2, lo_rowsum=True, raw=bool(wn2))
             dh, da2, db2 = _conv_dgrad(ops, dy, w2, k2, 1, 1, 0, c, t, (h, a2, b2), emit={"snake": None} if want_emit else None)
-            dw1, dbias1 = _conv_wgrad(ops, dh, x, k1, 1, dil, pad1, (a1, b1), bias_grad=True, raw=bool(wn1))
+            dw1, dbias1 = wgrad1(dh, True)
         dg1 = dg2 = None
         if wn1:
             if dbias1.dim() == 2:
@@ -306,7 +333,8 @@
                 dw2, dg2, dbias2 = _wn_backward(ops, dw2, wn2, gs2, bias_partial=dbias2)
             else:
                 dw2, dg2 = _wn_backward(ops, dw2, wn2, gs2)
-        dx, da1, db1 = _conv_dgrad(ops, dh, w1, k1, 1, dil, pad1, c, t, (x, a1, b1), res=dy)
+        if not skip_dh:
+            dx, da1, db1 = _conv_dgrad(ops, dh, w1, k1, 1, dil, pad1, c, t, (x, a1, b1), res=dy)
         return dx, da1, db1, dw1, dbias1, da2, db2, dw2, dbias2, None, None, None, None, None, None, dg1, dg2
 
 
diff --git a/stable_audio_tools_amd/ops.py b/stable_audio_tools_amd/ops.py
--- a/stable_audio_tools_amd/ops.py
+++ b/stable_audio_tools_amd/ops.py
@@ -179,7 +179,7 @@
             if esnake is not None:
                 ela, elb = esnake
                 self._f32(ela, elb)
-            ehi, elo, erows = self._emit_planes(b, cout, t, x.device, self._stream(x))
+            ehi, elo, erows = self._emit_planes(b, cout, t, x.device, self._stream(x), owner=esnake)
         self._chk(self.lib.sat_edge_conv(_ptr(x), _ptr(w), _ptr(bias), _ptr(alpha), _ptr(beta), _ptr(y), _ptr(x2), _ptr(a2), _ptr(b2),
                                          _ptr(pda), _ptr(pdb), _ptr(ehi), _ptr(elo), _ptr(ela), _ptr(elb), erows, b, cin, cout, t, k, pad, mode,
                                          int(tanh_out), self._stream(x)))
@@ -278,7 +278,7 @@
             ea = eib = None
             if esnake is not None:
                 ea, eib = self.snake_consts(esnake[0], esnake[1])
-            ehi, elo, erows = self._emit_planes(b, cout, tout, x.device, self._stream(x))
+            ehi, elo, erows = self._emit_planes(b, cout, tout, x.device, self._stream(x), owner=esnake)
             self._chk(self.lib.sat_conv1d_bf16x3_emit(_ptr(x), _ptr(w_planes[0]), _ptr(w_planes[1]), _ptr(bias), _ptr(sa), _ptr(sib),
                                                       _ptr(res), _ptr(y), _ptr(x2), _ptr(a2), _ptr(b2), _ptr(pda), _ptr(pdb),
                                                       b, cin, cout, tin, tout, *dims, int(tanh_out), _ptr(ehi), _ptr(elo), _ptr(ea), _ptr(eib),
@@ -373,7 +373,37 @@
         return (self.k7_emit and self.use_bf16x3 and cin <= 2 and self.edge_ok(cin, cout, k, stride, dil, pad)
                 and self.k7q_applicable(cout, 7, 1, consumer_dil, 3 * consumer_dil, cout))
 
-    def _emit_planes(self, b, c, t, device, st, alt=False):
+    wgrad7_planes = True
+    wgrad7_planes_budget_gib = 16.0
+    ru_k1_bwd_skip_dh = True
+
+    def _owned_planes(self, snake, b, c, t, device, st, create=False):
+        if snake is None or not self.wgrad7_planes:
+            return None
+        key = (snake[0].data_ptr(), snake[1].data_ptr(), b, c, t, device)
+        cache = self.__dict__.setdefault("_own_planes", {})
+        own = cache.get(key)
+        capturing = device.type == "cuda" and torch.cuda.is_current_stream_capturing()
+        sv = st.value if st is not None else 0
+        if own is not None and own["stream"] != sv and not capturing:
+            return None
+        if own is None and create:
+            if capturing:
+                return None
+            rows = self.lib.sat_conv1d_k7_plane_rows(t, t, 0)
+            n = b * ((c + 7) // 8) * rows * 8
+            held = sum(4 * o["hi"].numel() for o in cache.values())
+            if held + 4 * n > self.wgrad7_planes_budget_gib * 2 ** 30:
+                return None
+            own = {"hi": _keep_zeros(n, torch.int16, device), "lo": _keep_zeros(n, torch.int16, device), "rows": rows, "gen": 0, "stream": sv}
+            cache[key] = own
+        return own
+
+    def _emit_planes(self, b, c, t, device, st, alt=False, owner=None):
+        own = self._owned_planes(owner, b, c, t, device, st)
+        if own is not None:
+            own["gen"] += 1
+            return own["hi"], own["lo"], own["rows"]
         rows = self.lib.sat_conv1d_k7_plane_rows(t, t, 0)
         key = ("emit", b, c, t, device, st.value if st is not None else 0, alt)
         cache = self.__dict__.setdefault("_planes", {})
@@ -394,8 +424,15 @@
             return e
         return None
 
+    def _peek_emitted(self, x, snake):
+        e = self.__dict__.get("_emitted")
+        if (e is not None and e["ptr"] == x.data_ptr() and e["shape"] == tuple(x.shape) and _caches.trackable(x)
+                and e["ver"] == _caches.version_of(x) and e["snake"] == self._snake_key(snake)):
+            return e
+        return None
+
     def conv1d_bf16x3(self, x, w_planes, cout, k, stride=1, dil=1, pad=0, tout=None, bias=None, snake=None, res=None,
-                      tanh_out=False, dsnake=None, out=None, sconsts=None, emit=None):
+                      tanh_out=False, dsnake=None, out=None, sconsts=None, emit=None, keep_planes=None):
         b, cin, tin = x.shape
         if tout is None:
             tout = (tin + 2 * pad - dil * (k - 1) - 1) // stride + 1
@@ -403,11 +440,12 @@
         if len(w_planes) == 3:
             if not (stride == 1 and 5 <= k <= 7 and 0 <= pad <= 32 and (k - 1) * dil <= 62):
                 raise ValueError("conv1d_bf16x3: q-packed weights need stride 1, 5 <= K <= 7, pad <= 32, (K-1)*dil <= 62")
-            return self._k7_planes_call(rows, x, w_planes, cout, tout, k, dil, pad, bias, snake, res, tanh_out, dsnake, out, sconsts)
+            return self._k7_planes_call(rows, x, w_planes, cout, tout, k, dil, pad, bias, snake, res, tanh_out, dsnake, out, sconsts, keep_planes)
         return self._bf16x3_call(self.lib.sat_conv1d_bf16x3, rows, x, w_planes, cout, tout, (k, stride, dil, pad),
                                  bias, snake, res, tanh_out, dsnake, out, sconsts, emit)
 
-    def _k7_planes_call(self, prows, x, w_planes, cout, tout, k, dil, pad, bias, snake, res, tanh_out, dsnake, out=None, sconsts=None):
+    def _k7_planes_call(self, prows, x, w_planes, cout, tout, k, dil, pad, bias, snake, res, tanh_out, dsnake, out=None, sconsts=None,
+                        keep_planes=None):
         b, cin, tin = x.shape
         self._f32(x, bias, res)
         sa = sib = None
@@ -415,8 +453,21 @@
             sa, sib = sconsts if sconsts is not None else self.snake_consts(snake[0], snake[1])
         st = self._stream(x)
         em = self._take_emitted(x, snake)
+        keep = keep_planes is not None
+        if em is None:
+            self._check_written(x)
+        own = self._owned_planes(snake, b, cin, tin, x.device, st, create=True) if keep and tin == tout and _caches.trackable(x) else None
+        if own is not None and em is None:
+            hi, lo, rows = own["hi"], own["lo"], own["rows"]
+            own["gen"] += 1
+            self._chk(self.lib.sat_conv1d_k7_planes(_ptr(x), _ptr(sa), _ptr(sib), _ptr(hi), _ptr(lo), b, cin, tin, rows, st))
+        if own is not None and (em is None or em["hi"].data_ptr() == own["hi"].data_ptr()):
+            keep_planes["kept"] = {"buf": own, "gen": own["gen"], "ptr": x.data_ptr(), "shape": tuple(x.shape), "ver": _caches.version_of(x),
+                             "snake": self._snake_key(snake)}
         if em is not None:
             hi, lo, rows = em["hi"], em["lo"], em["rows"]
+        elif own is not None:
+            pass
         else:
             rows = self.lib.sat_conv1d_k7_plane_rows(tin, tout, pad)
             c8 = (cin + 7) // 8
@@ -519,7 +570,7 @@
         self._chk(self.lib.sat_ru_k1_pack(_ptr(w2), _ptr(planes[0]), _ptr(planes[1]), c, self._stream(w2)))
         return planes[0], planes[1]
 
-    def ru_k1_bwd(self, dy, h, w2, snake2, emit=False, wt=None, raw=False):
+    def ru_k1_bwd(self, dy, h, w2, snake2, emit=False, wt=None, raw=False, skip_dh=False):
         b, c, t = dy.shape
         a2, b2 = snake2
         self._f32(dy, h, w2, a2, b2)
@@ -535,10 +586,15 @@
         erows = 0
         if emit:
             ehi, elo, erows = self._emit_planes(b, c, t, dy.device, st)
-        self._chk(self.lib.sat_ru_k1_bwd(_ptr(dy), _ptr(h), _ptr(wt_hi), _ptr(wt_lo), _ptr(a2), _ptr(b2), _ptr(dh), _ptr(ehi), _ptr(elo), erows,
-                                         _ptr(slabs), _ptr(part), b, c, t, st))
+        if skip_dh and not emit:
+            raise ValueError("ru_k1_bwd: skip_dh needs emit=True")
+        self._dh_unwritten = dh.data_ptr() if skip_dh else None
+        self._chk(self.lib.sat_ru_k1_bwd(_ptr(dy), _ptr(h), _ptr(wt_hi), _ptr(wt_lo), _ptr(a2), _ptr(b2), None if skip_dh else _ptr(dh),
+                                         _ptr(ehi), _ptr(elo), erows, _ptr(slabs), _ptr(part), b, c, t, st))
         if emit:
             self._note_emitted(dh, None, ehi, elo, erows)
+            if skip_dh and self._emitted is None:
+                raise RuntimeError("ru_k1_bwd: dh was skipped but its planes cannot be tracked")
         dw2 = WgradSlabs(slabs, ns, (c, c, 1), (c, 1, 1))
         if not raw:
             dw2 = dw2.reduce(self)
@@ -553,6 +609,7 @@
         n = x.shape[1]
         alpha, beta = snake if snake is not None else (None, None)
         self._f32(dy, x, alpha, beta)
+        self._check_written(dy)
         nsplit = self.lib.sat_conv_wgrad7_bf16x3_nsplit(b, m, n, t)
         partial = torch.empty(nsplit, m * n * 7, dtype=torch.float32, device=dy.device)
         fused = dy_rowsum and self.lib.sat_conv_wgrad7_bf16x3_fuses_rowsum(b, m, n, t) == 1
@@ -567,8 +624,34 @@
             return dw, (rs if fused else self.rowsum(dy, partial=True))
         return dw, (self._sum_last(rs) if fused else self.rowsum(dy))
 
+    def _check_written(self, t):
+        if t is not None and self.__dict__.get("_dh_unwritten") is not None and t.data_ptr() == self._dh_unwritten:
+            raise RuntimeError("this tensor is a dh that sat_ru_k1_bwd did not write (skip_dh): only its planes exist")
+
+    def dh_written(self):
+        self._dh_unwritten = None
+
+    def release_owned_planes(self):
+        self.__dict__.pop("_own_planes", None)
+
+    def conv_wgrad7_planes_ok(self, b, m, n, t, dil, pad, rows_dy, rows_act):
+        return self.use_bf16x3 and self.wgrad7_planes and self.lib.sat_conv_wgrad7_planes_ok(b, m, n, t, dil, pad, rows_dy, rows_act) == 1
+
+    def conv_wgrad7_planes(self, dy_planes, act_planes, b, m, n, t, dil, pad, raw=False):
+        dhi, dlo, drows = dy_planes
+        ahi, alo, arows = act_planes
+        if self.lib.sat_conv_wgrad7_planes_ok(b, m, n, t, dil, pad, drows, arows) != 1:
+            raise RuntimeError("conv_wgrad7_planes: shape not served by the planes kernel (conv_wgrad7_planes_ok)")
+        nsplit = self.lib.sat_conv_wgrad7_planes_nsplit(b, m, n, t)
+        partial = torch.empty(nsplit, m * n * 7, dtype=torch.float32, device=dhi.device)
+        self._chk(self.lib.sat_conv_wgrad7_planes(_ptr(dhi), _ptr(dlo), drows, _ptr(ahi), _ptr(alo), arows, _ptr(partial), n, 1, m * n,
+                                                  b, m, n, t, dil, pad, self._stream(dhi)))
+        slabs = WgradSlabs(partial, nsplit, (m, n, 7), (n, 1, m * n))
+        return slabs if raw else slabs.reduce(self)
+
     def rowsum(self, x, partial=False):
         self._f32(x)
+        self._check_written(x)
         b, c, t = x.shape
         while True:
             ns = self.lib.sat_rowsum_nsplit(t)
@@ -656,7 +739,7 @@
         return dx
 
     def release_workspaces(self):
-        for name in ("_planes", "_disc_pool", "_disc_gen", "_disc_geoms"):
+        for name in ("_planes", "_own_planes", "_disc_pool", "_disc_gen", "_disc_geoms"):
             d = self.__dict__.get(name)
             if d is not None:
                 d.clear()
```

Result: faster. 8.043, median of 6 (+3.5%).
